# Li-Qingyun/RSCoTr

Measured on AMD Instinct MI355X. Metric: images/sec MTL train step (Swin-T 512^2, bs=2/GPU), higher is better.
Workload: dtype f32 (large products as three fp16 MFMAs on two-plane power-of-two-scaled splits of the fp32 operands, fp32 accumulate: fp32-FMA-class error; six bf16 MFMAs on three-plane splits where an operand has no range word)

## Files before the change

include/rscotr.h:

```cpp
#ifndef RSCOTR_H
#define RSCOTR_H
#include <stdint.h>
#ifdef __cplusplus
extern "C" {
#endif

#define RSCOTR_OK 0
#define RSCOTR_E_SHAPE (-1)
#define RSCOTR_E_ALIGN (-2)
#define RSCOTR_E_ARCH (-3)
#define RSCOTR_E_LAUNCH (-4)
#define RSCOTR_E_ARG (-5)

#define RSCOTR_ABI_VERSION 11
int rscotr_version(void);
const char* rscotr_last_error(void);
int rscotr_device_count(void);

int rscotr_prof_enable(int every_gemm, int every_msda_fwd, int every_msda_bwd, int max_records);
int rscotr_prof_pause(void);
int rscotr_prof_empty(int n, void* stream);
int rscotr_prof_get(int i, int* kind, double* work, float* ms, char* name, int name_len);
int rscotr_prof_disable(void);

int rscotr_msda_fwd(const float* value, const int64_t* spatial_shapes,
                    const int64_t* level_start_index, const float* loc, const float* attn,
                    float* out, int B, int Nk, int Nq, int H, int D, int L, int P, void* stream);
int rscotr_msda_bwd(const float* value, const int64_t* spatial_shapes,
                    const int64_t* level_start_index, const float* loc, const float* attn,
                    const float* grad_out, float* grad_value, float* grad_loc, float* grad_attn,
                    int B, int Nk, int Nq, int H, int D, int L, int P, const int64_t* shapes_host,
                    void* workspace, int64_t workspace_bytes, uint32_t* amax_grad_value,
                    void* stream);
int64_t rscotr_msda_bwd_workspace(int B, int Nk, int Nq, int H, int L, int P);
int64_t rscotr_msda_bwd_tiled_workspace(const int64_t* shapes_host, int B, int Nk, int Nq, int H, int D, int L, int P);
int rscotr_msda_prep_fwd(const float* off, const float* logit, const float* ref, const float* norm, float* loc,
                         float* attn, int B, int Nq, int H, int L, int P, int refdim, int ld_off, int ld_logit,
                         int ref_levels, void* stream);
int rscotr_msda_prep_bwd(const float* grad_loc, const float* grad_attn, const float* attn, const float* ref,
                         const float* norm, float* grad_off, float* grad_logit, int B, int Nq, int H, int L, int P,
                         int refdim, int ld_off, int ld_logit, int ref_levels, uint32_t* amax_out, void* stream);
int rscotr_msda_fused_ok(int Nk, int H, int D, int L, int P);
int rscotr_msda_fwd_prep(const float* value, const int64_t* spatial_shapes, const int64_t* level_start_index,
                         const float* off, const float* logit, int ld_off, int ld_logit, const float* ref,
                         const float* norm, int refdim, int ref_levels, float* loc, float* attn, float* out, int B,
                         int Nk, int Nq, int H, int D, int L, int P, void* stream);

int rscotr_gemm_split_weights(const int64_t* table, int n, int total_blocks, void* stream);
int64_t rscotr_gemm_f32_wplanes_workspace(int M, int N, int K);
int rscotr_gemm_f32_wplanes_ok(int M, int N, int K, int act_is_gelu);
int rscotr_gemm_f32_wplanes(const float* A, const void* planes, int npad, float* C, int M, int N, int K, int lda, int ldc,
                            const float* bias, int act, const float* aux, float* pre, const float* resid, int accumulate,
                            const float* rowscale, int rows_per_scale, float* out2, float* workspace,
                            int64_t workspace_bytes, void* stream);
int rscotr_gemm_set_precision(int prec);
int rscotr_gemm_get_precision(void);
int64_t rscotr_gemm_f32_workspace(int M, int N, int K);
int rscotr_gemm_f32(const float* A, const float* B, float* C, int M, int N, int K, int lda, int ldb,
                    int ldc, int a_kmajor, int b_kmajor, const float* bias, int act, const float* aux,
                    float* pre, const float* resid, int accumulate, float* rowsum, int rowsum_accumulate,
                    const float* rowscale, int rows_per_scale, const float* kscale, int krows_per_scale,
                    float* out2, float* workspace, int64_t workspace_bytes, void* stream);
#define RSCOTR_RANGE_EXP_LO 80
#define RSCOTR_RANGE_PLANES 32
#define RSCOTR_RANGE_STRIDE 16384
int rscotr_gemm_f32_r(const float* A, const float* B, float* C, int M, int N, int K, int lda, int ldb,
                      int ldc, int a_kmajor, int b_kmajor, const float* bias, int act, const float* aux,
                      float* pre, const float* resid, int accumulate, float* rowsum, int rowsum_accumulate,
                      const float* rowscale, int rows_per_scale, const float* kscale, int krows_per_scale,
                      float* out2, float* workspace, int64_t workspace_bytes, const uint32_t* amax_a,
                      const uint32_t* amax_b, uint32_t* amax_out, void* stream);
int rscotr_gemm_set_h3(int on);
int rscotr_gemm_relu_bits_ok(int M, int N, int K, int lda, int ldb, int a_kmajor, int b_kmajor);
int rscotr_gemm_split_weights_h3(const int64_t* table, int n, int total_blocks, void* stream);
int rscotr_gemm_f32_rb(const float* A, const float* B, float* C, int M, int N, int K, int lda, int ldb,
                       int ldc, int a_kmajor, int b_kmajor, const float* bias, int act, const float* aux,
                       float* pre, const float* resid, int accumulate, float* rowsum, int rowsum_accumulate,
                       const float* rowscale, int rows_per_scale, const float* kscale, int krows_per_scale,
                       float* out2, float* workspace, int64_t workspace_bytes, const uint32_t* amax_a,
                       const uint32_t* amax_b, uint32_t* amax_out, const void* b_planes, int b_rpad, void* stream);
int rscotr_ffn_h3_ok(int M, int C, int H);
int rscotr_ffn_h3_splits(int M, int C, int H);
int64_t rscotr_ffn_h3_bits_words(int M, int C, int H);
int rscotr_gemm_split_weights_frag(const int64_t* table, int n, int total_blocks, void* stream);
int rscotr_lin_h3_ok(int M, int N, int K);
int rscotr_lin_h3(const float* X, int M, int N, int K, const void* Wf, const float* bias, const float* resid, float* Y,
                  const float* xscale, const float* yscale, int rows_per, const uint32_t* amax_x, const uint32_t* amax_w,
                  uint32_t* amax_y, void* stream);
int rscotr_lin_h3_ln(const float* X, int M, int N, int K, const float* ln_weight, const float* ln_bias, float ln_eps, float* ln_out,
                     float* ln_mean, float* ln_rstd, const void* Wf, const float* bias, const float* resid, float* Y,
                     const float* yscale, int rows_per, const uint32_t* amax_ln_weight, const uint32_t* amax_ln_bias,
                     const uint32_t* amax_w, uint32_t* amax_ln_out, uint32_t* amax_y, void* stream);
int rscotr_ffn_h3_ln(const float* X, int M, int C, int H, const float* ln_weight, const float* ln_bias, float ln_eps, float* ln_out,
                     float* ln_mean, float* ln_rstd, const void* W1f, const float* b1, const void* W2f, const float* b2, float* Pre,
                     float* Hid, const float* resid, float* Y, const float* yscale, int rows_per, const uint32_t* amax_ln_weight,
                     const uint32_t* amax_ln_bias, const uint32_t* amax_w1, const uint32_t* amax_w2, const uint32_t* amax_b1,
                     uint32_t* amax_ln_out, uint32_t* amax_hid, uint32_t* amax_y, float* workspace, int64_t workspace_bytes,
                     void* stream);
int rscotr_ffn_h3(const float* X, int M, int C, int H, const void* W1f, const float* b1, const void* W2f, const float* b2,
                  int mode, void* bits, float* Pre, float* Hid, const float* resid, float* Y, const float* xscale,
                  const float* yscale, int rows_per, const uint32_t* amax_x, const uint32_t* amax_w1,
                  const uint32_t* amax_w2, const uint32_t* amax_b1, uint32_t* amax_hid, uint32_t* amax_y, float* workspace,
                  int64_t workspace_bytes, void* stream);
int rscotr_gemm_f32_split_route(int M, int N, int K, int lda, int ldb, int a_kmajor, int b_kmajor, int act, int has_pre,
                                int has_rowscale, int has_kscale, int64_t workspace_bytes);
int rscotr_amax_f32(const float* X, int64_t rows, int cols, int ld, uint32_t* slot, void* stream);
int rscotr_amax_group(const int64_t* table, int n, int total_blocks, void* stream);
int rscotr_gemm_f32_dw_slabs(const float* A, const float* B, float* C, int M, int N, int K, int lda, int ldb, int ldc,
                             float* rowsum, const float* kscale, int krows_per_scale, float* slab_region,
                             int64_t slab_bytes, int32_t* splits_out, void* stream);
int rscotr_gemm_f32_dw_slabs_r(const float* A, const float* B, float* C, int M, int N, int K, int lda, int ldb, int ldc,
                               float* rowsum, const float* kscale, int krows_per_scale, float* slab_region,
                               int64_t slab_bytes, int32_t* splits_out, const uint32_t* amax_a, const uint32_t* amax_b,
                               void* stream);
int rscotr_splitk_flush(const int64_t* table, const int32_t* wgmap, int nwg, double bytes, void* stream);
int rscotr_gemm_dw_group(const int64_t* table, int n, int total_wgs, int variant, double flops,
                         const uint32_t* amax_base, void* stream);

int rscotr_gemm_f32_batched(const float* A, const float* B, float* C, int M, int N, int K, int lda, int ldb,
                            int ldc, int a_kmajor, int b_kmajor, int nb0, int nb1, int64_t sA0, int64_t sA1,
                            int64_t sB0, int64_t sB1, int64_t sC0, int64_t sC1, int accumulate, int ksplits,
                            float* workspace, int64_t c_elems, void* stream);
int rscotr_softmax_mask_fwd(float* S, const unsigned char* mask, int mask_mode, int B, int heads, int Lq, int Lk,
                            float scale, void* stream);
int rscotr_softmax_bwd(const float* P, float* dP, int64_t rows, int Lk, float scale, void* stream);
int64_t rscotr_attn_core_workspace(int B, int heads, int Lq, int Lk);
int rscotr_attn_core_fwd(const float* q, const float* k, const float* v, const unsigned char* mask, int mask_mode, float* out,
                         float* lse, int B, int heads, int Lq, int Lk, int hd, int ldq, int ldk, int ldv, int ldo, float scale,
                         void* workspace, int64_t workspace_bytes, void* stream);
int rscotr_attn_core_bwd(const float* q, const float* k, const float* v, const unsigned char* mask, int mask_mode, const float* out,
                         const float* dout, const float* lse, float* dq, float* dk, float* dv, int B, int heads, int Lq, int Lk,
                         int hd, int ldq, int ldk, int ldv, int ldo, int lddq, int lddk, int lddv, float scale, void* workspace,
                         int64_t workspace_bytes, void* stream);
int64_t rscotr_colsum_f32_workspace(int M, int N);
int rscotr_colsum_f32(const float* X, float* out, int M, int N, int ld, int accumulate, float* workspace,
                      int64_t workspace_bytes, void* stream);

int rscotr_layernorm_fwd(const float* x, const float* weight, const float* bias, float* y, float* mean,
                         float* rstd, int M, int C, float eps, uint32_t* amax_out, void* stream);
int rscotr_det_proposals(const float* enc_cls, const float* enc_reg, const float* proposals, int proposals_batched,
                         int64_t* topk_idx, float* topk_score, float* topk_unact, float* topk_anchor, int32_t* inv, int B, int N,
                         int C, int K, void* stream);
int rscotr_det_proposals_bwd(const float* d_score, const float* d_anchor, const float* topk_anchor, const int32_t* inv,
                             float* d_cls, float* d_reg, int B, int N, int C, int K, void* stream);

int rscotr_det_targets(const int32_t* q_for_gt, const int64_t* gt_lab, const float* gt_boxn, int64_t* labels, float* bbox_targets,
                       float* bbox_weights, int S, int B, int Q, int G, int num_classes, void* stream);

int rscotr_layernorm_fwd_sum(const float* x, const float* weight, const float* bias, float* y, float* mean, float* rstd,
                             const float* add, int add_rows, float* y2, int M, int C, float eps, uint32_t* amax_out,
                             void* stream);
int64_t rscotr_layernorm_bwd_workspace(int M, int C);
int rscotr_layernorm_bwd(const float* dy, const float* x, const float* weight, const float* mean,
                         const float* rstd, float* dx, const float* dx_add, float* dweight, float* dbias, int M, int C,
                         float* workspace, int64_t workspace_bytes, uint32_t* amax_out, void* stream);

int rscotr_patch_merge_norm_fwd(const float* x, const float* weight, const float* bias, float* y, float* mean, float* rstd,
                                int B, int H, int W, int Cin, float eps, uint32_t* amax_out, void* stream);
int64_t rscotr_patch_merge_norm_bwd_workspace(int B, int H, int W, int Cin);
int rscotr_patch_merge_norm_bwd(const float* dy, const float* x, const float* weight, const float* mean, const float* rstd,
                                float* dx, float* dweight, float* dbias, int B, int H, int W, int Cin, float* workspace,
                                int64_t workspace_bytes, int fold, uint32_t* amax_out, void* stream);

int rscotr_layernorm_bwd_partials(const float* dy, const float* x, const float* weight, const float* mean,
                                  const float* rstd, float* dx, const float* dx_add, int M, int C, float* part, int64_t part_bytes,
                                  uint32_t* amax_out, void* stream);
int rscotr_layernorm_flush(const int64_t* table, const int32_t* wgmap, int nwg, void* stream);


int rscotr_swin_wattn_fwd(const float* qkv, const float* qkv_bias, const float* bias_table, float* out,
                          int B, int H, int W, int C, int heads, int ws, int shift, uint32_t* amax_out,
                         void* stream);
int64_t rscotr_swin_wattn_bwd_workspace(int B, int H, int W, int C, int heads);
int rscotr_swin_wattn_bwd(const float* qkv, const float* qkv_bias, const float* bias_table, const float* dout,
                          float* dqkv, float* dqkv_bias, float* dbias_table, int B, int H, int W, int C,
                          int heads, int ws, int shift, const float* out, float* workspace,
                          int64_t workspace_bytes, uint32_t* amax_out, void* stream);
int rscotr_swin_wattn_flush(const int64_t* table, int n, int total_heads, void* stream);

int64_t rscotr_groupnorm_tokens_workspace(int B, int L, int C, int G);
int rscotr_groupnorm_tokens_fwd(const float* x, const float* weight, const float* bias, float* y,
                                float* mean_rstd, int B, int L, int C, int G, float eps, float* workspace,
                                int64_t workspace_bytes, void* stream);
int rscotr_groupnorm_tokens_bwd(const float* dy, const float* x, const float* weight, const float* mean_rstd,
                                float* dx, float* dweight, float* dbias, float* proj_ws, int B, int L, int C,
                                int G, int64_t dy_batch_stride, float* workspace, int64_t workspace_bytes, void* stream);
int rscotr_im2col3x3s2_tokens(const float* x, float* col, int B, int H, int W, int C, void* stream);
int rscotr_col2im3x3s2_tokens(const float* dcol, float* dx, int B, int H, int W, int C, void* stream);

int64_t rscotr_upsample_ce_workspace(void);
int rscotr_upsample_ce_fwd(const float* logit, const int64_t* label, float* lse, float* sums, int B, int C,
                           int h, int w, int H, int W, int ignore_index, float* workspace, int64_t workspace_bytes,
                           void* stream);
int rscotr_upsample_ce_bwd(const float* logit, const int64_t* label, const float* lse, const float* grad_scale,
                           float* dlogit, int B, int C, int h, int w, int H, int W, int ignore_index, void* stream);
int64_t rscotr_upsample_ce_w_workspace(void);
int rscotr_upsample_ce_w_fwd(const float* logit, const int64_t* label, const float* class_weight, float* lse, float* nll,
                             float* pix_weight, float* sums, int B, int C, int h, int w, int H, int W, int ignore_index,
                             float* workspace, int64_t workspace_bytes, void* stream);
int rscotr_upsample_ce_ohem(const int64_t* label, const float* class_weight, const float* nll, float* pix_weight,
                            float* sum_out, int64_t npix, int C, int ignore_index, int64_t kept, float nll_thresh,
                            float* workspace, int64_t workspace_bytes, void* stream);
int rscotr_upsample_ce_w_bwd(const float* logit, const int64_t* label, const float* lse, const float* pix_weight,
                             const float* grad_scale, float* dlogit, int B, int C, int h, int w, int H, int W,
                             int ignore_index, void* stream);

int64_t rscotr_upsample_dice_workspace(int B, int C);
int rscotr_upsample_dice_fwd(const float* logit, const int64_t* label, const float* class_weight, float* lse, float* coef,
                             float* loss, int B, int C, int h, int w, int H, int W, int ignore_index, float smooth,
                             float loss_weight, float* workspace, int64_t workspace_bytes, void* stream);
int rscotr_upsample_dice_bwd(const float* logit, const int64_t* label, const float* lse, const float* coef,
                             const float* grad_scale, float* pix_s, float* dlogit, int B, int C, int h, int w, int H, int W,
                             int ignore_index, void* stream);

int64_t rscotr_upsample_tversky_workspace(int B, int C);
int rscotr_upsample_tversky_fwd(const float* logit, const int64_t* label, const float* class_weight, float* lse, float* coef,
                                float* loss, int B, int C, int h, int w, int H, int W, int ignore_index, float alpha, float beta,
                                float smooth, float loss_weight, float* workspace, int64_t workspace_bytes, void* stream);
int rscotr_upsample_tversky_bwd(const float* logit, const int64_t* label, const float* lse, const float* coef,
                                const float* grad_scale, float* pix_s, float* dlogit, int B, int C, int h, int w, int H, int W,
                                int ignore_index, void* stream);

int64_t rscotr_upsample_focal_workspace(void);
int rscotr_upsample_focal_fwd(const float* logit, const int64_t* label, const float* alpha_per_class, const float* class_weight,
                              float* loss, int B, int C, int h, int w, int H, int W, int ignore_index, float gamma, float alpha,
                              float loss_scale, float* workspace, int64_t workspace_bytes, void* stream);
int rscotr_upsample_focal_bwd(const float* logit, const int64_t* label, const float* alpha_per_class, const float* class_weight,
                              const float* grad_scale, float* dlogit, int B, int C, int h, int w, int H, int W, int ignore_index,
                              float gamma, float alpha, void* stream);

int64_t rscotr_upsample_lovasz_workspace(int B, int C, int nslots, int H, int W, int per_image);
int rscotr_upsample_lovasz_sort_tile(void);
int rscotr_upsample_lovasz_sort_workgroup(void);
int rscotr_upsample_lovasz_fwd(const float* logit, const int64_t* label, const int* slots, const float* class_weight, float* lse,
                               float* dplane, int* meta, float* loss, int B, int C, int nslots, int h, int w, int H, int W,
                               int ignore_index, int present, int per_image, int image_mean, float loss_weight, float* workspace,
                               int64_t workspace_bytes, void* stream);
int rscotr_upsample_lovasz_bwd(const float* logit, const int64_t* label, const int* slots, const float* lse, const float* dplane,
                               const int* meta, const float* grad_scale, float* pix_s, float* dlogit, int B, int C, int nslots,
                               int h, int w, int H, int W, int ignore_index, int per_image, void* stream);

int rscotr_sine_embed4(const float* pos, float* out, int64_t rows, void* stream);

int rscotr_level_embed_fwd(const float* x, int64_t x_bstride, const float* cst, int cst_batched, const float* w,
                           float* out, const int* sizes, int L, int B, int N, int C, void* stream);
int rscotr_cdn_queries(const int64_t* gt_lab, const float* gt_boxn, const int64_t* slot_src, const float* slot_valid,
                       const float* slot_neg, const float* u, int uniform, const float* embed, float label_thr,
                       float box_scale, int num_classes, int64_t* kl_out, float* q_label, float* q_bbox, int n_slots, int C,
                       void* stream);
int rscotr_cdn_embed_grad(const float* g, const int64_t* kl, const float* slot_valid, float* dw, int rows, int n_slots,
                          int C, int accumulate, void* stream);
int rscotr_gap_tokens_fwd(const float* x, float* out, int B, int T, int C, void* stream);
int rscotr_gap_tokens_bwd(const float* g, float* dx, int B, int T, int C, void* stream);
int rscotr_soft_ce(const float* score, const float* label, float* loss, float* dscore, int B, int C, float smooth,
                   float avg_factor, void* stream);
int rscotr_sum8(const float* p0, const float* p1, const float* p2, const float* p3, const float* p4, const float* p5,
                const float* p6, const float* p7, int n, float* out, int64_t count, void* stream);
int rscotr_pack4(const float* a, int64_t na, const float* b, int64_t nb, const float* c, int64_t nc, const float* d,
                 int64_t nd, float* out, uint32_t* amax_out, void* stream);
int64_t rscotr_level_embed_bwd_workspace(int L, int C);
int rscotr_level_embed_bwd(const float* g, float* dw, const int* sizes, int L, int B, int N, int C, int accumulate,
                           float* workspace, int* counters, void* stream);

int rscotr_seg_attn_mask(const float* mask_pred, unsigned char* out, int rows, int h, int w, int th, int tw,
                         void* stream);

int64_t rscotr_seg_mix_workspace(void);
int rscotr_seg_mix_fwd(const float* cls, const float* e, const float* mf, float* mix, float* seg, int B, int Q, int K, int D,
                       int P, void* stream);
int rscotr_seg_mix_bwd(const float* g, const float* cls, const float* e, const float* mf, const float* mix, float* dmf,
                       float* de, float* dcls, float* dmix, int B, int Q, int K, int D, int P, float* workspace,
                       int64_t workspace_bytes, void* stream);

int rscotr_refine_box_fwd(const float* delta, const float* ref, float* out, int64_t n, float eps, void* stream);
int rscotr_refine_box_bwd(const float* grad_out, const float* out, const float* ref, float* d_delta, float* d_ref,
                          int64_t n, float eps, void* stream);
int rscotr_match_cost(const float* cls, const float* box, const float* gt_box, const int64_t* gt_lab,
                      const float* factors, float* cost, int S, int B, int Q, int C, int G, float w_cls, float w_l1,
                      float w_iou, float alpha, float gamma, float eps, void* stream);
int rscotr_focal_sum(const float* pred, const int64_t* target, const float* weight, float* sums, float* dpred, int S,
                     int N, int C, float gamma, float alpha, void* stream);
int rscotr_box_loss(const float* pred, const float* target, const float* weight, const float* factors, float* sums,
                    float* d_l1, float* d_giou, int S, int B, int Q, float eps, void* stream);
int rscotr_match_cost_kind(const float* cls, const float* box, const float* gt_box, const int64_t* gt_lab,
                           const float* factors, float* cost, int S, int B, int Q, int C, int G, float w_cls, float w_l1,
                           float w_iou, float alpha, float gamma, float eps, int iou_mode, void* stream);
int rscotr_box_loss_kind(const float* pred, const float* target, const float* weight, const float* factors, float* sums,
                         float* d_l1, float* d_iou, int S, int B, int Q, float eps, int kind, int mode, void* stream);
int rscotr_qfl_sum(const float* pred, const int64_t* target, const float* weight, const float* box, const float* box_target,
                   float* sums, float* dpred, int S, int N, int C, float beta, void* stream);

int rscotr_lsap_f64(const double* cost, int nr, int nc, int64_t* row_ind, int64_t* col_ind);
int rscotr_lsap_dev_f32(const float* cost, const int32_t* gcount, int P, int Q, int ld, int32_t* q_for_gt,
                        void* stream);
int rscotr_lsap_batch_f32(const float* cost, const int64_t* offsets, const int* rows, const int* cols,
                          int n, const int64_t* out_offsets, int64_t* row_ind, int64_t* col_ind);

int rscotr_grad_sumsq(const float* grad, const int32_t* chunk_seg, const int64_t* chunk_off,
                      const int32_t* chunk_len, const float* seg_dyn, int nchunks, float* sumsq,
                      void* stream);
int rscotr_adamw_clip_step(float* param, const float* grad, float* exp_avg, float* exp_avg_sq,
                           const int32_t* chunk_seg, const int64_t* chunk_off, const int32_t* chunk_len,
                           const float* seg_dyn, int nchunks, const float* sumsq, float max_norm,
                           float beta1, float beta2, float eps, void* stream);
int rscotr_adamw_clip_step_r(float* param, const float* grad, float* exp_avg, float* exp_avg_sq,
                             const int32_t* chunk_seg, const int64_t* chunk_off, const int32_t* chunk_len,
                             const float* seg_dyn, int nchunks, const float* sumsq, float max_norm,
                             float beta1, float beta2, float eps, uint32_t* seg_amax, int nseg, uint32_t* chunk_amax,
                             void* stream);
int rscotr_param_amax(const float* param, const int32_t* chunk_seg, const int64_t* chunk_off,
                      const int32_t* chunk_len, int nchunks, uint32_t* seg_amax, int nseg, uint32_t* chunk_amax,
                      void* stream);

int rscotr_comm_available(void);
int rscotr_comm_unique_id(void* id128);
int rscotr_comm_init(const void* id128, int rank, int nranks, void** comm_out);
int rscotr_comm_allreduce_avg(void* comm, float* buf, int64_t count, void* stream);
int rscotr_comm_destroy(void* comm);

int rscotr_img_prep_u8(const uint8_t* src, const int64_t* meta, float* out, int B, int Hout, int Wout,
                       const float* mean3, const float* std3, int to_rgb, void* stream);
int rscotr_seg_label_prep_u8(const uint8_t* src, const int64_t* meta, int64_t* out, int B, int Hout, int Wout,
                             int reduce_zero_label, int pad_val, void* stream);

int rscotr_img_aug_u8(const uint8_t* src, const int64_t* meta, const int32_t* tables, const float* params, float* out,
                      int B, int Hout, int Wout, const float* mean3, const float* std3, int to_rgb, void* stream);
int rscotr_seg_label_aug_u8(const uint8_t* src, const int64_t* meta, const int32_t* tables, int64_t* out, int B, int Hout,
                            int Wout, int reduce_zero_label, int pad_val, void* stream);

int rscotr_img_aug_chain_u8(const uint8_t* src, const int64_t* meta, const int32_t* tables, float* out, int B, int Hout,
                            int Wout, const float* mean3, const float* std3, int to_rgb, void* stream);

int rscotr_img_aug_rot_u8(const uint8_t* src, const int64_t* meta, const int32_t* tables, const float* params,
                          const int32_t* rot, const int32_t* warp, float* out, int B, int Hout, int Wout, const float* mean3,
                          const float* std3, int to_rgb, void* stream);
int rscotr_seg_label_rot_u8(const uint8_t* src, const int64_t* meta, const int32_t* tables, const int32_t* rot,
                            const int32_t* warp, int64_t* out, int B, int Hout, int Wout, int reduce_zero_label, int pad_val,
                            void* stream);

int rscotr_img_frames_u8(const uint8_t* src, const int64_t* meta, const int32_t* tables, uint8_t* frames, int B, int H, int W,
                         void* stream);
int rscotr_randaug_u8(const uint8_t* in, uint8_t* out, const int32_t* meta, const int32_t* warp, const int16_t* wtab,
                      uint32_t* stats, int need_stats, int B, int H, int W, void* stream);

int rscotr_seg_predict_u8(const float* logit, uint8_t* out, int B, int C, int h, int w, int H, int W, int rescale, int hs,
                          int ws, int Ho, int Wo, int flip, void* stream);
int rscotr_seg_areas_u8(const uint8_t* pred, const uint8_t* gt, int64_t* out, int B, int Hp, int Wp, int C, int ignore_index,
                        int reduce_zero_label, void* stream);

int rscotr_seg_predict_tta_u8(const int64_t* views, uint8_t* out, int V, int B, int C, int Ho, int Wo, void* stream);

int rscotr_seg_predict_slide_u8(const float* logit, uint8_t* out, int B, int C, int h, int w, int H, int W, int ch, int cw, int sy,
                                int sx, int rescale, int hs, int ws, int Ho, int Wo, int flip, void* stream);

int rscotr_det_decode_f32(const float* cls, const float* box, const float* meta, float* dets, int64_t* labels, int B, int Q,
                          int C, int K, int rescale, void* stream);
int rscotr_det_match(const float* dets, const int64_t* labels, const int32_t* n_det, const float* gt_boxes,
                     const int64_t* gt_labels, const int64_t* gt_offsets, const double* area_ranges, const double* iou_thrs,
                     int32_t* flags, int32_t* npig, int B, int K, int64_t G, int C, int A, int T, int max_det, void* stream);

#ifdef __cplusplus
}
#endif
#endif
```

rscotr_amd/csrc/common.h:

```cpp
#pragma once
#include <hip/hip_runtime.h>
#include <stdint.h>
#include <stdio.h>
#include <stdarg.h>

#define RSCOTR_OK 0
#define RSCOTR_E_SHAPE (-1)
#define RSCOTR_E_ALIGN (-2)
#define RSCOTR_E_ARCH (-3)
#define RSCOTR_E_LAUNCH (-4)
#define RSCOTR_E_ARG (-5)

namespace rscotr {

char* err_buf();

inline int fail(int code, const char* fmt, ...) {
  va_list ap;
  va_start(ap, fmt);
  vsnprintf(err_buf(), 512, fmt, ap);
  va_end(ap);
  return code;
}

inline int check_launch(const char* what) {
  hipError_t e = hipGetLastError();
  if (e != hipSuccess) return fail(RSCOTR_E_LAUNCH, "%s: %s", what, hipGetErrorString(e));
  return RSCOTR_OK;
}

inline bool aligned16(const void* p) { return (reinterpret_cast<uintptr_t>(p) & 15u) == 0; }

constexpr int kWave = 64;

enum { PROF_GEMM = 0, PROF_MSDA_FWD = 1, PROF_MSDA_BWD = 2, PROF_HBM = 3, PROF_MFMA = 4, PROF_KINDS = 5 };
struct ProfScope {
  int slot;
  hipStream_t stream;
  ProfScope(int kind, double work, hipStream_t s, const char* fmt, ...);
  ~ProfScope();
};

template <int G>
__device__ __forceinline__ float group_sum(float v) {
#pragma unroll
  for (int o = G / 2; o > 0; o >>= 1) v += __shfl_xor(v, o, 64);
  return v;
}

template <int G>
__device__ __forceinline__ float group_max(float v) {
#pragma unroll
  for (int o = G / 2; o > 0; o >>= 1) v = fmaxf(v, __shfl_xor(v, o, 64));
  return v;
}

__device__ __forceinline__ float wave_sum(float v) { return group_sum<64>(v); }
__device__ __forceinline__ float wave_max(float v) { return group_max<64>(v); }

constexpr int kAmaxPlanes = 32;
constexpr int kAmaxStride = 16384;
constexpr int kRangeExpLo = 80;

__device__ __forceinline__ int range_byte(unsigned bits) {
  return min(max((int)((bits >> 23) & 0xffu), kRangeExpLo), kRangeExpLo + 4 * kAmaxPlanes - 1) - kRangeExpLo;
}
__device__ __forceinline__ void range_mark(unsigned* slot, int i) {
  reinterpret_cast<unsigned char*>(slot + (long)(i >> 2) * kAmaxStride)[i & 3] = 1;
}

__device__ __forceinline__ int amax_fold_code(unsigned v, int sub) { return v ? 4 * sub + ((31 - __clz((int)v)) >> 3) + 1 : 0; }
__device__ __forceinline__ unsigned amax_fold_bits(int c) { return c ? (unsigned)(kRangeExpLo + c - 1) << 23 : 0u; }
__device__ __forceinline__ unsigned amax_fold(unsigned v) {
  int c = amax_fold_code(v, (int)(threadIdx.x & (kAmaxPlanes - 1)));
#pragma unroll
  for (int o = kAmaxPlanes / 2; o > 0; o >>= 1) c = max(c, __shfl_xor(c, o, 64));
  return amax_fold_bits(__builtin_amdgcn_readfirstlane(c));
}
__device__ __forceinline__ unsigned amax_fold_lane(unsigned v, int lane) {
  int c = amax_fold_code(v, lane & (kAmaxPlanes - 1));
#pragma unroll
  for (int o = kAmaxPlanes / 2; o > 0; o >>= 1) c = max(c, __builtin_amdgcn_ds_bpermute((lane ^ o) << 2, c));
  return amax_fold_bits(__builtin_amdgcn_readfirstlane(c));
}
__device__ __forceinline__ unsigned amax_read(const unsigned* word) {
  return amax_fold(word[(long)(threadIdx.x & (kAmaxPlanes - 1)) * kAmaxStride]);
}
__device__ __forceinline__ float amax_hi(unsigned folded) { return folded ? __uint_as_float(folded + (1u << 23)) : 0.f; }

__device__ __forceinline__ void amax_commit(unsigned* slot, float amx) {
  if (!slot) return;
#pragma unroll
  for (int o = 32; o > 0; o >>= 1) amx = fmaxf(amx, __shfl_xor(amx, o, 64));
  if ((threadIdx.x & 63) == 0) {
    const unsigned b = __float_as_uint(amx) & 0x7fffffffu;
    if (b) range_mark(slot, range_byte(b));
  }
}

__device__ __forceinline__ float2 msda_location(const float* __restrict__ r, float2 o, const float* __restrict__ norm, int l, int P,
                                                int refdim) {
  float2 out;
  if (refdim == 2) {
    out.x = r[0] + o.x / norm[2 * l];
    out.y = r[1] + o.y / norm[2 * l + 1];
  } else {
    out.x = r[0] + o.x / (float)P * r[2] * 0.5f;
    out.y = r[1] + o.y / (float)P * r[3] * 0.5f;
  }
  return out;
}

__device__ __forceinline__ float amax4(float a, const float4& v) {
  return fmaxf(fmaxf(a, fmaxf(fabsf(v.x), fabsf(v.y))), fmaxf(fabsf(v.z), fabsf(v.w)));
}

}
```

rscotr_amd/csrc/ffn.hip:

```cpp
#include "gemm_common.h"
#include "rscotr.h"
#include <type_traits>

namespace rscotr {

typedef float f32x4_t __attribute__((ext_vector_type(4)));

constexpr int FFN_HC = 128;
constexpr int FFN_LDRB = 160;
constexpr int FFN_DB = 1;

enum { FFN_RELU = 0,
       FFN_RELU_GATE = 1,
       FFN_GELU = 2,
       FFN_GELU_GRAD = 3 };

struct FfnParams {
  const float* X;
  int M, H;
  const uint4* W1f;
  const float* b1;
  const uint4* W2f;
  const float* b2;
  unsigned* bits;
  float* Pre;
  float* Hid;
  const float* resid;
  float* Y;
  const float* xscale;
  const float* yscale;
  int rows_per;
  const unsigned *amax_x, *amax_w1, *amax_w2, *amax_b1;
  unsigned *amax_hid, *amax_y;
  int splits;
  float* slabs;
  const float *ln_g, *ln_b;
  float ln_eps;
  float *ln_out, *ln_mean, *ln_rstd;
  const unsigned *amax_g, *amax_bt;
  unsigned* amax_ln;
  int by_xcd;
  int tpx;
};

template <int C, int NT>
constexpr size_t ffn_lds_bytes() { return (size_t)(C / 32 + 2 * (FFN_HC / 32)) * (16 * NT) * FFN_LDRB; }

__device__ __forceinline__ void store_b128(float4 v, __amdgpu_buffer_rsrc_t r, int voff, int soff) {
  __builtin_amdgcn_raw_buffer_store_b128(__builtin_bit_cast(__attribute__((__vector_size__(4 * sizeof(unsigned)))) unsigned, v), r, voff, soff, 0);
  __builtin_amdgcn_sched_barrier(0);
  asm volatile("s_nop 1");
  __builtin_amdgcn_sched_barrier(0);
}

constexpr int FFN_STAG_MINC = 192;
constexpr int FFN_PHASES = 4;
__device__ __forceinline__ int ffn_phase(int j, int n) {
  const int ph = n < FFN_PHASES ? n : FFN_PHASES;
  return (int)((unsigned)j % (unsigned)ph) * n / ph;
}

__device__ __forceinline__ f32x4_t mfma16(uint4 a, uint4 b, f32x4_t c) {
  return __builtin_amdgcn_mfma_f32_16x16x32_f16(__builtin_bit_cast(f16x8, a), __builtin_bit_cast(f16x8, b), c, 0, 0, 0);
}

constexpr int FFN_SWIN_WAVES = 4;
template <int C, int NT, int MODE, bool LN = false>
__global__ __launch_bounds__(512) __attribute__((amdgpu_waves_per_eu(C == 96 ? FFN_SWIN_WAVES : 2, C == 96 ? FFN_SWIN_WAVES : 2))) void ffn_h3_kernel(FfnParams p) {
  extern __shared__ __attribute__((aligned(16))) unsigned char ffn_lds[];
  constexpr bool GATE = MODE == FFN_RELU_GATE, GELU = MODE == FFN_GELU, GGRAD = MODE == FFN_GELU_GRAD;
  constexpr bool FWD = MODE == FFN_RELU || MODE == FFN_GELU;
  constexpr int BM = 16 * NT, STG = BM * FFN_LDRB;
  constexpr int KS1 = C / 32, HST = FFN_HC / 32;
  constexpr int DA = KS1 % 2 == 0 ? 2 : 1;
  constexpr int TPB = C == 96 ? 2 : C / 64;
  constexpr int NB = C / 16 / TPB;
  constexpr int RING = 4 * DA > 2 * TPB * FFN_DB ? 4 * DA : 2 * TPB * FFN_DB;
  constexpr int SPK = (2 * NT + KS1 - 1) / KS1;
  static_assert(C % 32 == 0 && (C / 16) % TPB == 0 && NB <= 4, "column tiles split evenly over the B wavefronts");
  unsigned char* xs = ffn_lds;
  unsigned char* hs = ffn_lds + KS1 * STG;
  const int tid = threadIdx.x, lane = tid & 63, li = lane & 15, kg = lane >> 4;
  const int wv = __builtin_amdgcn_readfirstlane(tid >> 6);
  const bool role_a = wv < 4;
  const int wr = wv & 3;
  int bx = blockIdx.x, by = blockIdx.y, jx = blockIdx.x >> 3;
  if (p.by_xcd) {
    const int xcd = (int)(blockIdx.x & 7);
    jx = (int)(blockIdx.x >> 3);
    by = xcd % p.splits;
    bx = xcd / p.splits + (8 / p.splits) * jx;
    if (bx * BM >= p.M) return;
  }
  const int m0 = bx * BM;
  const int nch = p.H / FFN_HC;
  const int nloc = nch / p.splits;
  const int cbase = by * nloc;

  const long sub = (long)(lane & (kAmaxPlanes - 1)) * kAmaxStride;
  const unsigned rx = LN ? 0u : p.amax_x[sub], r1 = p.amax_w1[sub], r2 = p.amax_w2[sub], rb = p.amax_b1 ? p.amax_b1[sub] : 0u;
  const unsigned rg = LN ? p.amax_g[sub] : 0u, rbt = (LN && p.amax_bt) ? p.amax_bt[sub] : 0u;

  const int wbytes = p.H * C * 4;
  const __amdgpu_buffer_rsrc_t rW = __builtin_amdgcn_make_buffer_rsrc(const_cast<uint4*>(role_a ? p.W1f : p.W2f), 0, wbytes, 0x00020000);
  const int nks2 = p.H / 32;
  const int vW = lane * 16 + (role_a ? wr * 2 * KS1 * 2048 : wr * TPB * nks2 * 2048);
  auto ld_a = [&](int c, int ks, int it, int pl) {
    return __builtin_bit_cast(uint4, __builtin_amdgcn_raw_buffer_load_b128(rW, vW, c * (8 * KS1 * 2048) + it * (KS1 * 2048) + ks * 2048 + pl * 1024, 0));
  };
  auto ld_b = [&](int t, int it, int pl) {
    return __builtin_bit_cast(uint4, __builtin_amdgcn_raw_buffer_load_b128(rW, vW, it * nks2 * 2048 + t * 2048 + pl * 1024, 0));
  };
  const int c0r = cbase + (C >= FFN_STAG_MINC ? ffn_phase(jx, nloc) : 0);
  uint4 ring[RING];
  if (role_a) {
#pragma unroll
    for (int q = 0; q < 4 * DA; ++q) ring[q] = ld_a(c0r, q >> 2, (q >> 1) & 1, q & 1);
  } else if (wr < NB) {
#pragma unroll
    for (int q = 0; q < 2 * TPB * FFN_DB; ++q) ring[q] = ld_b(c0r * HST + min(q / (2 * TPB), HST - 1), (q >> 1) % TPB, q & 1);
  }

  const int rows_ok = min(BM, p.M - m0);
  const __amdgpu_buffer_rsrc_t rX = __builtin_amdgcn_make_buffer_rsrc(const_cast<float*>(p.X + (long)m0 * C), 0, rows_ok * C * 4, 0x00020000);
  const __amdgpu_buffer_rsrc_t rH = __builtin_amdgcn_make_buffer_rsrc(p.Hid + (long)m0 * p.H, 0, rows_ok * p.H * 4, 0x00020000);
  const __amdgpu_buffer_rsrc_t rP = __builtin_amdgcn_make_buffer_rsrc((GELU || GGRAD) ? p.Pre + (long)m0 * p.H : p.Hid, 0, rows_ok * p.H * 4, 0x00020000);
  float* const ybase = p.splits > 1 ? p.slabs + (long)by * p.M * C : p.Y;
  const __amdgpu_buffer_rsrc_t rY = __builtin_amdgcn_make_buffer_rsrc(ybase + (long)m0 * C, 0, rows_ok * C * 4, 0x00020000);
  const __amdgpu_buffer_rsrc_t rR = __builtin_amdgcn_make_buffer_rsrc(const_cast<float*>(p.resid ? p.resid + (long)m0 * C : p.X), 0, rows_ok * C * 4, 0x00020000);

  const unsigned fx = LN ? 0u : amax_fold(rx);
  const float xbound = LN ? sqrtf((float)C) * amax_hi(amax_fold(rg)) + amax_hi(amax_fold(rbt)) : amax_hi(fx);
  const unsigned ux = LN ? __float_as_uint(xbound) : fx;
  if constexpr (!LN) {
    constexpr int TOT = BM * (C / 4), NV = (TOT + 511) / 512;
    float4 v[NV];
#pragma unroll
    for (int i = 0; i < NV; ++i) v[i] = __builtin_bit_cast(float4, __builtin_amdgcn_raw_buffer_load_b128(rX, (tid + i * 512) * 16, 0, 0));
    const int ex0 = h3_scale_exp(ux);
    const H3Scale hx{__uint_as_float((unsigned)ex0 << 23), __uint_as_float((unsigned)(ex0 + 11) << 23)};
#pragma unroll
    for (int i = 0; i < NV; ++i) {
      const int idx = tid + i * 512;
      if (TOT % 512 == 0 || idx < TOT) {
        const int row = idx / (C / 4), kq = (idx % (C / 4)) * 4;
        if (p.xscale) {
          const float f = p.xscale[min(m0 + row, p.M - 1) / p.rows_per];
          v[i].x *= f; v[i].y *= f; v[i].z *= f; v[i].w *= f;
        }
        unsigned ab[3], cd[3];
        split_pair_h(v[i].x, v[i].y, hx, ab);
        split_pair_h(v[i].z, v[i].w, hx, cd);
        unsigned char* dst = xs + (kq / 32) * STG + row * FFN_LDRB + (kq % 32) * 2;
        *reinterpret_cast<uint2*>(dst) = make_uint2(ab[0], cd[0]);
        *reinterpret_cast<uint2*>(dst + 64) = make_uint2(ab[1], cd[1]);
      }
    }
  } else {
    static_assert(C % 48 == 0 && (C / 12 == 8 || C / 12 == 16 || C / 12 == 32), "LN rows: 8 / 16 / 32 lanes x 3 float4");
    constexpr int G = C / 12, RPP = 512 / G, NP = (BM + RPP - 1) / RPP;
    const int sub = tid % G, rr = tid / G;
    const __amdgpu_buffer_rsrc_t rL = __builtin_amdgcn_make_buffer_rsrc(p.ln_out + (long)m0 * C, 0, (by == 0 ? rows_ok : 0) * C * 4, 0x00020000);
    const int ex0 = h3_scale_exp(ux);
    const H3Scale hx{__uint_as_float((unsigned)ex0 << 23), __uint_as_float((unsigned)(ex0 + 11) << 23)};
    float amx = 0.f;
    if (RPP <= BM || wv < 8 * BM / RPP) {
      float4 gw[3], gb[3];
#pragma unroll
      for (int j = 0; j < 3; ++j) {
        gw[j] = reinterpret_cast<const float4*>(p.ln_g)[sub + j * G];
        gb[j] = p.ln_b ? reinterpret_cast<const float4*>(p.ln_b)[sub + j * G] : make_float4(0.f, 0.f, 0.f, 0.f);
      }
#pragma unroll
      for (int ps = 0; ps < NP; ++ps) {
        const int row = ps * RPP + rr;
        float4 v[3];
        float sm = 0.f;
#pragma unroll
        for (int j = 0; j < 3; ++j) {
          v[j] = __builtin_bit_cast(float4, __builtin_amdgcn_raw_buffer_load_b128(rX, (row * C + 4 * (sub + j * G)) * 4, 0, 0));
          sm += v[j].x + v[j].y + v[j].z + v[j].w;
        }
#pragma unroll
        for (int o = G / 2; o > 0; o >>= 1) sm += __shfl_xor(sm, o, 64);
        const float mu = sm * (1.f / (float)C);
        float q = 0.f;
#pragma unroll
        for (int j = 0; j < 3; ++j) {
          v[j].x -= mu; v[j].y -= mu; v[j].z -= mu; v[j].w -= mu;
          q += v[j].x * v[j].x + v[j].y * v[j].y + v[j].z * v[j].z + v[j].w * v[j].w;
        }
#pragma unroll
        for (int o = G / 2; o > 0; o >>= 1) q += __shfl_xor(q, o, 64);
        const float rs = rsqrtf(q * (1.f / (float)C) + p.ln_eps);
        if (sub == 0 && by == 0 && row < rows_ok) { p.ln_mean[m0 + row] = mu; p.ln_rstd[m0 + row] = rs; }
#pragma unroll
        for (int j = 0; j < 3; ++j) {
          float4 o;
          o.x = v[j].x * rs * gw[j].x + gb[j].x; o.y = v[j].y * rs * gw[j].y + gb[j].y;
          o.z = v[j].z * rs * gw[j].z + gb[j].z; o.w = v[j].w * rs * gw[j].w + gb[j].w;
          if (row >= rows_ok) o = make_float4(0.f, 0.f, 0.f, 0.f);
          const int kq = 4 * (sub + j * G);
          store_b128(o, rL, (row * C + kq) * 4, 0);
          amx = amax4(amx, o);
          unsigned ab[3], cd[3];
          split_pair_h(o.x, o.y, hx, ab);
          split_pair_h(o.z, o.w, hx, cd);
          unsigned char* dst = xs + (kq / 32) * STG + row * FFN_LDRB + (kq % 32) * 2;
          *reinterpret_cast<uint2*>(dst) = make_uint2(ab[0], cd[0]);
          *reinterpret_cast<uint2*>(dst + 64) = make_uint2(ab[1], cd[1]);
        }
      }
    }
    if (by == 0) amax_commit(p.amax_ln, amx);
  }
  const unsigned u1 = amax_fold(r1), u2 = amax_fold(r2), ub = amax_fold(rb);
  const int ex = h3_scale_exp(ux), e1 = h3_scale_exp(u1), e2 = h3_scale_exp(u2);
  const float bound = ((float)C * xbound * amax_hi(u1) + amax_hi(ub)) * (GGRAD ? 1.25f : 1.f);
  const int eh = h3_scale_exp(__float_as_uint(bound));
  const H3Scale hh{__uint_as_float((unsigned)eh << 23), __uint_as_float((unsigned)(eh + 11) << 23)};
  const float invx = __uint_as_float((unsigned)(254 - ex) << 23), inv1 = __uint_as_float((unsigned)(254 - e1) << 23);
  const float invh = __uint_as_float((unsigned)(254 - eh) << 23), inv2 = __uint_as_float((unsigned)(254 - e2) << 23);

  const int fo = li * FFN_LDRB + kg * 16;
  const int c0 = C >= FFN_STAG_MINC ? ffn_phase(jx, nloc) : 0;
  auto chunk_of = [&](int c) {
    if constexpr (C < FFN_STAG_MINC) return cbase + c;
    const int v = c + c0;
    return cbase + (v >= nloc ? v - nloc : v);
  };
  __syncthreads();

  if (role_a) {
    unsigned amxu = 0u;
    const int vH = (li * p.H + wr * 32 + 4 * kg) * 4;
    float4 pv[2][NT];
    float4 bvs[2];
    float4 pres[GGRAD ? 2 : 1][GGRAD ? NT : 1];
    unsigned bits = 0u;
    auto slice = [&](int cl, int it, int n) {
      const int cp = chunk_of(cl);
      float v[4] = {pv[it][n].x, pv[it][n].y, pv[it][n].z, pv[it][n].w};
      const int soff = (n * 16 * p.H + cp * FFN_HC + it * 16) * 4;
      if constexpr (MODE == FFN_RELU) {
        const float t[4] = {v[0] + bvs[it].x, v[1] + bvs[it].y, v[2] + bvs[it].z, v[3] + bvs[it].w};
#pragma unroll
        for (int r = 0; r < 4; ++r) {
          const bool pos = t[r] > 0.f;
          v[r] = pos ? t[r] : 0.f;
          bits |= (unsigned)pos << ((it * NT + n) * 4 + r);
        }
      } else if constexpr (GATE) {
#pragma unroll
        for (int r = 0; r < 4; ++r)
          v[r] = __uint_as_float(__float_as_uint(v[r]) & (unsigned)__builtin_amdgcn_sbfe((int)bits, (it * NT + n) * 4 + r, 1));
      } else if constexpr (GELU) {
        const float4 t = make_float4(v[0] + bvs[it].x, v[1] + bvs[it].y, v[2] + bvs[it].z, v[3] + bvs[it].w);
        store_b128(t, rP, vH, soff);
        v[0] = gelu_f(t.x); v[1] = gelu_f(t.y); v[2] = gelu_f(t.z); v[3] = gelu_f(t.w);
      } else {
        const float4 t = pres[GGRAD ? it : 0][GGRAD ? n : 0];
        v[0] *= gelu_grad_f(t.x); v[1] *= gelu_grad_f(t.y); v[2] *= gelu_grad_f(t.z); v[3] *= gelu_grad_f(t.w);
      }
#pragma unroll
      for (int r = 0; r < 4; ++r) amxu = max(amxu, __float_as_uint(v[r]) & 0x7fffffffu);
      unsigned ab[3], cd[3];
      split_pair_h(v[0], v[1], hh, ab);
      split_pair_h(v[2], v[3], hh, cd);
      unsigned char* dst = hs + (cl & 1) * (HST * STG) + wr * STG + li * FFN_LDRB + kg * 8 + n * 16 * FFN_LDRB + it * 32;
      *reinterpret_cast<uint2*>(dst) = make_uint2(ab[0], cd[0]);
      *reinterpret_cast<uint2*>(dst + 64) = make_uint2(ab[1], cd[1]);
      store_b128(make_float4(v[0], v[1], v[2], v[3]), rH, vH, soff);
    };
    auto pre_epi = [&](int cl) {
      const int cp = chunk_of(cl);
#pragma unroll
      for (int it = 0; it < 2; ++it)
        bvs[it] = (FWD && p.b1) ? *reinterpret_cast<const float4*>(p.b1 + cp * FFN_HC + wr * 32 + it * 16 + 4 * kg) : make_float4(0.f, 0.f, 0.f, 0.f);
      if constexpr (GATE) bits = p.bits[(((long)bx * nch + cp) * 4 + wr) * 64 + lane];
      else bits = 0u;
      if constexpr (GGRAD) {
#pragma unroll
        for (int it = 0; it < 2; ++it)
#pragma unroll
          for (int n = 0; n < NT; ++n)
            pres[it][n] = __builtin_bit_cast(float4, __builtin_amdgcn_raw_buffer_load_b128(rP, vH, (n * 16 * p.H + cp * FFN_HC + it * 16) * 4, 0));
      }
    };
    auto kloop = [&](int c, auto with_epi) {
      constexpr bool EPI = decltype(with_epi)::value;
      f32x4_t ha[2][NT], hb[2][NT];
#pragma unroll
      for (int it = 0; it < 2; ++it)
#pragma unroll
        for (int n = 0; n < NT; ++n) { ha[it][n] = f32x4_t{0.f, 0.f, 0.f, 0.f}; hb[it][n] = f32x4_t{0.f, 0.f, 0.f, 0.f}; }
      const int cw = chunk_of(c), cn = chunk_of(min(c + 1, nloc - 1));
#pragma unroll
      for (int ks = 0; ks < KS1; ++ks) {
        uint4 xh[NT], xl[NT];
#pragma unroll
        for (int n = 0; n < NT; ++n) {
          const unsigned char* q = xs + ks * STG + n * 16 * FFN_LDRB + fo;
          xh[n] = *reinterpret_cast<const uint4*>(q);
          xl[n] = *reinterpret_cast<const uint4*>(q + 64);
        }
#pragma unroll
        for (int it = 0; it < 2; ++it) {
          const int slot = (ks % DA) * 4 + it * 2;
          const uint4 wh = ring[slot], wl = ring[slot + 1];
#pragma unroll
          for (int n = 0; n < NT; ++n) hb[it][n] = mfma16(wh, xl[n], hb[it][n]);
#pragma unroll
          for (int n = 0; n < NT; ++n) hb[it][n] = mfma16(wl, xh[n], hb[it][n]);
#pragma unroll
          for (int n = 0; n < NT; ++n) ha[it][n] = mfma16(wh, xh[n], ha[it][n]);
          if (ks + DA < KS1) { ring[slot] = ld_a(cw, ks + DA, it, 0); ring[slot + 1] = ld_a(cw, ks + DA, it, 1); }
          else { ring[slot] = ld_a(cn, ks + DA - KS1, it, 0); ring[slot + 1] = ld_a(cn, ks + DA - KS1, it, 1); }
        }
        if constexpr (EPI) {
#pragma unroll
          for (int t = ks * SPK; t < (ks + 1) * SPK; ++t)
            if (t < 2 * NT) slice(c - 1, t / NT, t % NT);
        }
        __builtin_amdgcn_sched_barrier(0);
      }
      if constexpr (EPI && MODE == FFN_RELU) p.bits[(((long)bx * nch + chunk_of(c - 1)) * 4 + wr) * 64 + lane] = bits;
      pre_epi(c);
#pragma unroll
      for (int it = 0; it < 2; ++it)
#pragma unroll
        for (int n = 0; n < NT; ++n) {
          pv[it][n].x = fmaf(hb[it][n][0], 0x1p-11f, ha[it][n][0]) * invx * inv1;
          pv[it][n].y = fmaf(hb[it][n][1], 0x1p-11f, ha[it][n][1]) * invx * inv1;
          pv[it][n].z = fmaf(hb[it][n][2], 0x1p-11f, ha[it][n][2]) * invx * inv1;
          pv[it][n].w = fmaf(hb[it][n][3], 0x1p-11f, ha[it][n][3]) * invx * inv1;
        }
    };
    kloop(0, std::false_type{});
    __syncthreads();
#pragma unroll 1
    for (int c = 1; c < nloc; ++c) {
      kloop(c, std::true_type{});
      __syncthreads();
    }
#pragma unroll
    for (int t = 0; t < 2 * NT; ++t) slice(nloc - 1, t / NT, t % NT);
    if constexpr (MODE == FFN_RELU) p.bits[(((long)bx * nch + chunk_of(nloc - 1)) * 4 + wr) * 64 + lane] = bits;
    __syncthreads();
    __syncthreads();
    amax_commit(p.amax_hid, __uint_as_float(amxu));
  } else {
    f32x4_t ya[TPB][NT], yb[TPB][NT];
#pragma unroll
    for (int it = 0; it < TPB; ++it)
#pragma unroll
      for (int n = 0; n < NT; ++n) { ya[it][n] = f32x4_t{0.f, 0.f, 0.f, 0.f}; yb[it][n] = f32x4_t{0.f, 0.f, 0.f, 0.f}; }
    const bool active = wr < NB;
    __syncthreads();
    __syncthreads();
#pragma unroll 1
    for (int c = 0; c < nloc; ++c) {
      const unsigned char* img = hs + (c & 1) * (HST * STG) + fo;
      const int cb = chunk_of(c);
      if (active) {
#pragma unroll 1
        for (int kq = 0; kq < HST / FFN_DB; ++kq)
#pragma unroll
          for (int u = 0; u < FFN_DB; ++u) {
            const int ks = kq * FFN_DB + u;
            uint4 gh[NT], gl[NT];
#pragma unroll
            for (int n = 0; n < NT; ++n) {
              const unsigned char* q = img + ks * STG + n * 16 * FFN_LDRB;
              gh[n] = *reinterpret_cast<const uint4*>(q);
              gl[n] = *reinterpret_cast<const uint4*>(q + 64);
            }
            int tn;
            if constexpr (C < FFN_STAG_MINC) tn = cbase * HST + min(c * HST + ks + FFN_DB, nloc * HST - 1);
            else tn = ks + FFN_DB < HST ? cb * HST + ks + FFN_DB : chunk_of(min(c + 1, nloc - 1)) * HST + (ks + FFN_DB - HST);
#pragma unroll
            for (int it = 0; it < TPB; ++it) {
              const int slot = u * 2 * TPB + it * 2;
              const uint4 wh = ring[slot], wl = ring[slot + 1];
#pragma unroll
              for (int n = 0; n < NT; ++n) yb[it][n] = mfma16(wh, gl[n], yb[it][n]);
#pragma unroll
              for (int n = 0; n < NT; ++n) yb[it][n] = mfma16(wl, gh[n], yb[it][n]);
#pragma unroll
              for (int n = 0; n < NT; ++n) ya[it][n] = mfma16(wh, gh[n], ya[it][n]);
              ring[slot] = ld_b(tn, it, 0);
              ring[slot + 1] = ld_b(tn, it, 1);
            }
          }
      }
      __syncthreads();
    }
    if (active) {
      const int vY = (li * C + wr * TPB * 16 + 4 * kg) * 4;
      float amy = 0.f;
#pragma unroll
      for (int it = 0; it < TPB; ++it) {
        float4 bv = make_float4(0.f, 0.f, 0.f, 0.f);
        if (p.b2) bv = *reinterpret_cast<const float4*>(p.b2 + wr * TPB * 16 + it * 16 + 4 * kg);
        float4 e[NT];
        float ysc[NT];
#pragma unroll
        for (int n = 0; n < NT; ++n) {
          e[n] = p.resid ? __builtin_bit_cast(float4, __builtin_amdgcn_raw_buffer_load_b128(rR, vY, (n * 16 * C + it * 16) * 4, 0)) : make_float4(0.f, 0.f, 0.f, 0.f);
          ysc[n] = p.yscale ? p.yscale[min(m0 + n * 16 + li, p.M - 1) / p.rows_per] : 1.f;
        }
#pragma unroll
        for (int n = 0; n < NT; ++n) {
          float4 v;
          v.x = fmaf(fmaf(yb[it][n][0], 0x1p-11f, ya[it][n][0]) * invh * inv2 + bv.x, ysc[n], e[n].x);
          v.y = fmaf(fmaf(yb[it][n][1], 0x1p-11f, ya[it][n][1]) * invh * inv2 + bv.y, ysc[n], e[n].y);
          v.z = fmaf(fmaf(yb[it][n][2], 0x1p-11f, ya[it][n][2]) * invh * inv2 + bv.z, ysc[n], e[n].z);
          v.w = fmaf(fmaf(yb[it][n][3], 0x1p-11f, ya[it][n][3]) * invh * inv2 + bv.w, ysc[n], e[n].w);
          store_b128(v, rY, vY, (n * 16 * C + it * 16) * 4);
          amy = amax4(amy, v);
        }
      }
      amax_commit(p.amax_y, amy);
    }
  }
}

struct LinParams {
  const float* X;
  int M, N;
  const uint4* Wf;
  const float* bias;
  const float* resid;
  float* Y;
  const float* xscale;
  const float* yscale;
  int rows_per;
  const unsigned *amax_x, *amax_w;
  unsigned* amax_y;
  int col_groups;
  const float *ln_g, *ln_b;
  float ln_eps;
  float *ln_out, *ln_mean, *ln_rstd;
  const unsigned *amax_g, *amax_bt;
  unsigned* amax_ln;
};

template <int C, bool LN, int NT = 2>
__global__ __launch_bounds__(512) void lin_h3_kernel(LinParams p) {
  extern __shared__ __attribute__((aligned(16))) unsigned char ffn_lds[];
  constexpr int BM = 16 * NT, STG = BM * FFN_LDRB, KS1 = C / 32;
  constexpr int DA = KS1 % 2 == 0 ? 2 : KS1 % 3 == 0 ? 3 : 1;
  static_assert(C % 32 == 0 && KS1 % DA == 0, "reduction in whole 32-k steps");
  unsigned char* xs = ffn_lds;
  const int tid = threadIdx.x, lane = tid & 63, li = lane & 15, kg = lane >> 4;
  const int wv = __builtin_amdgcn_readfirstlane(tid >> 6);
  const int m0 = blockIdx.x * BM;
  const long sub = (long)(lane & (kAmaxPlanes - 1)) * kAmaxStride;
  const unsigned rx = LN ? 0u : p.amax_x[sub], rw = p.amax_w[sub];
  const unsigned rg = LN ? p.amax_g[sub] : 0u, rbt = (LN && p.amax_bt) ? p.amax_bt[sub] : 0u;
  const __amdgpu_buffer_rsrc_t rW = __builtin_amdgcn_make_buffer_rsrc(const_cast<uint4*>(p.Wf), 0, p.N * C * 4, 0x00020000);
  auto ld_w = [&](int col0, int ks, int it, int pl) {
    return __builtin_bit_cast(uint4, __builtin_amdgcn_raw_buffer_load_b128(rW, lane * 16, ((col0 >> 4) + it) * (KS1 * 2048) + ks * 2048 + pl * 1024, 0));
  };
  const int c_first = (int)blockIdx.y * 256 + wv * 32;
  const int c_step = 256 * (int)gridDim.y;
  uint4 ring[4 * DA];
  if (c_first < p.N) {
#pragma unroll
    for (int q = 0; q < 4 * DA; ++q) ring[q] = ld_w(c_first, q >> 2, (q >> 1) & 1, q & 1);
  }
  const int rows_ok = min(BM, p.M - m0);
  const __amdgpu_buffer_rsrc_t rX = __builtin_amdgcn_make_buffer_rsrc(const_cast<float*>(p.X + (long)m0 * C), 0, rows_ok * C * 4, 0x00020000);
  const __amdgpu_buffer_rsrc_t rY = __builtin_amdgcn_make_buffer_rsrc(p.Y + (long)m0 * p.N, 0, rows_ok * p.N * 4, 0x00020000);
  const __amdgpu_buffer_rsrc_t rR = __builtin_amdgcn_make_buffer_rsrc(const_cast<float*>(p.resid ? p.resid + (long)m0 * p.N : p.X), 0, rows_ok * p.N * 4, 0x00020000);
  const unsigned fx = LN ? 0u : amax_fold(rx);
  const float xbound = LN ? sqrtf((float)C) * amax_hi(amax_fold(rg)) + amax_hi(amax_fold(rbt)) : amax_hi(fx);
  const unsigned ux = LN ? __float_as_uint(xbound) : fx;
  const int ex = h3_scale_exp(ux);
  const H3Scale hx{__uint_as_float((unsigned)ex << 23), __uint_as_float((unsigned)(ex + 11) << 23)};
  if constexpr (!LN) {
    constexpr int TOT = BM * (C / 4), NV = (TOT + 511) / 512;
    float4 v[NV];
#pragma unroll
    for (int i = 0; i < NV; ++i) v[i] = __builtin_bit_cast(float4, __builtin_amdgcn_raw_buffer_load_b128(rX, (tid + i * 512) * 16, 0, 0));
#pragma unroll
    for (int i = 0; i < NV; ++i) {
      const int idx = tid + i * 512;
      if (TOT % 512 == 0 || idx < TOT) {
        const int row = idx / (C / 4), kq = (idx % (C / 4)) * 4;
        if (p.xscale) {
          const float f = p.xscale[min(m0 + row, p.M - 1) / p.rows_per];
          v[i].x *= f; v[i].y *= f; v[i].z *= f; v[i].w *= f;
        }
        unsigned ab[3], cd[3];
        split_pair_h(v[i].x, v[i].y, hx, ab);
        split_pair_h(v[i].z, v[i].w, hx, cd);
        unsigned char* dst = xs + (kq / 32) * STG + row * FFN_LDRB + (kq % 32) * 2;
        *reinterpret_cast<uint2*>(dst) = make_uint2(ab[0], cd[0]);
        *reinterpret_cast<uint2*>(dst + 64) = make_uint2(ab[1], cd[1]);
      }
    }
  } else {
    static_assert(!LN || (C % 48 == 0 && (C / 12 == 8 || C / 12 == 16 || C / 12 == 32)), "LN rows: 8 / 16 / 32 lanes x 3 float4");
    constexpr int G = C / 12, RPP = 512 / G, NP = (BM + RPP - 1) / RPP;
    const int sb = tid % G, rr = tid / G;
    const bool own = blockIdx.y == 0;
    const __amdgpu_buffer_rsrc_t rL = __builtin_amdgcn_make_buffer_rsrc(p.ln_out + (long)m0 * C, 0, (own ? rows_ok : 0) * C * 4, 0x00020000);
    float amx = 0.f;
    if (RPP <= BM || wv < 8 * BM / RPP) {
      float4 gw[3], gb[3];
#pragma unroll
      for (int j = 0; j < 3; ++j) {
        gw[j] = reinterpret_cast<const float4*>(p.ln_g)[sb + j * G];
        gb[j] = p.ln_b ? reinterpret_cast<const float4*>(p.ln_b)[sb + j * G] : make_float4(0.f, 0.f, 0.f, 0.f);
      }
#pragma unroll
      for (int ps = 0; ps < NP; ++ps) {
        const int row = ps * RPP + rr;
        float4 v[3];
        float sm = 0.f;
#pragma unroll
        for (int j = 0; j < 3; ++j) {
          v[j] = __builtin_bit_cast(float4, __builtin_amdgcn_raw_buffer_load_b128(rX, (row * C + 4 * (sb + j * G)) * 4, 0, 0));
          sm += v[j].x + v[j].y + v[j].z + v[j].w;
        }
#pragma unroll
        for (int o = G / 2; o > 0; o >>= 1) sm += __shfl_xor(sm, o, 64);
        const float mu = sm * (1.f / (float)C);
        float q = 0.f;
#pragma unroll
        for (int j = 0; j < 3; ++j) {
          v[j].x -= mu; v[j].y -= mu; v[j].z -= mu; v[j].w -= mu;
          q += v[j].x * v[j].x + v[j].y * v[j].y + v[j].z * v[j].z + v[j].w * v[j].w;
        }
#pragma unroll
        for (int o = G / 2; o > 0; o >>= 1) q += __shfl_xor(q, o, 64);
        const float rs = rsqrtf(q * (1.f / (float)C) + p.ln_eps);
        if (sb == 0 && own && row < rows_ok) { p.ln_mean[m0 + row] = mu; p.ln_rstd[m0 + row] = rs; }
#pragma unroll
        for (int j = 0; j < 3; ++j) {
          float4 o;
          o.x = v[j].x * rs * gw[j].x + gb[j].x; o.y = v[j].y * rs * gw[j].y + gb[j].y;
          o.z = v[j].z * rs * gw[j].z + gb[j].z; o.w = v[j].w * rs * gw[j].w + gb[j].w;
          if (row >= rows_ok) o = make_float4(0.f, 0.f, 0.f, 0.f);
          const int kq = 4 * (sb + j * G);
          store_b128(o, rL, (row * C + kq) * 4, 0);
          amx = amax4(amx, o);
          unsigned ab[3], cd[3];
          split_pair_h(o.x, o.y, hx, ab);
          split_pair_h(o.z, o.w, hx, cd);
          unsigned char* dst = xs + (kq / 32) * STG + row * FFN_LDRB + (kq % 32) * 2;
          *reinterpret_cast<uint2*>(dst) = make_uint2(ab[0], cd[0]);
          *reinterpret_cast<uint2*>(dst + 64) = make_uint2(ab[1], cd[1]);
        }
      }
    }
    if (own) amax_commit(p.amax_ln, amx);
  }
  const int ew = h3_scale_exp(amax_fold(rw));
  const float inv = __uint_as_float((unsigned)(254 - ex) << 23) * __uint_as_float((unsigned)(254 - ew) << 23);
  const int fo = li * FFN_LDRB + kg * 16;
  __syncthreads();

  float amy = 0.f;
#pragma unroll 1
  for (int col0 = c_first; col0 < p.N; col0 += c_step) {
    f32x4_t ha[2][NT], hb[2][NT];
#pragma unroll
    for (int it = 0; it < 2; ++it)
#pragma unroll
      for (int n = 0; n < NT; ++n) { ha[it][n] = f32x4_t{0.f, 0.f, 0.f, 0.f}; hb[it][n] = f32x4_t{0.f, 0.f, 0.f, 0.f}; }
    const int cnext = col0 + c_step < p.N ? col0 + c_step : col0;
#pragma unroll
    for (int ks = 0; ks < KS1; ++ks) {
      uint4 xh[NT], xl[NT];
#pragma unroll
      for (int n = 0; n < NT; ++n) {
        const unsigned char* q = xs + ks * STG + n * 16 * FFN_LDRB + fo;
        xh[n] = *reinterpret_cast<const uint4*>(q);
        xl[n] = *reinterpret_cast<const uint4*>(q + 64);
      }
#pragma unroll
      for (int it = 0; it < 2; ++it) {
        const int slot = (ks % DA) * 4 + it * 2;
        const uint4 wh = ring[slot], wl = ring[slot + 1];
#pragma unroll
        for (int n = 0; n < NT; ++n) hb[it][n] = mfma16(wh, xl[n], hb[it][n]);
#pragma unroll
        for (int n = 0; n < NT; ++n) hb[it][n] = mfma16(wl, xh[n], hb[it][n]);
#pragma unroll
        for (int n = 0; n < NT; ++n) ha[it][n] = mfma16(wh, xh[n], ha[it][n]);
        if (ks + DA < KS1) { ring[slot] = ld_w(col0, ks + DA, it, 0); ring[slot + 1] = ld_w(col0, ks + DA, it, 1); }
        else { ring[slot] = ld_w(cnext, ks + DA - KS1, it, 0); ring[slot + 1] = ld_w(cnext, ks + DA - KS1, it, 1); }
      }
      __builtin_amdgcn_sched_barrier(0);
    }
    const int vY = (li * p.N + col0 + 4 * kg) * 4;
#pragma unroll
    for (int it = 0; it < 2; ++it) {
      float4 bv = make_float4(0.f, 0.f, 0.f, 0.f);
      if (p.bias) bv = *reinterpret_cast<const float4*>(p.bias + col0 + it * 16 + 4 * kg);
      float4 e[NT];
      float ysc[NT];
#pragma unroll
      for (int n = 0; n < NT; ++n) {
        e[n] = p.resid ? __builtin_bit_cast(float4, __builtin_amdgcn_raw_buffer_load_b128(rR, vY, (n * 16 * p.N + it * 16) * 4, 0)) : make_float4(0.f, 0.f, 0.f, 0.f);
        ysc[n] = p.yscale ? p.yscale[min(m0 + n * 16 + li, p.M - 1) / p.rows_per] : 1.f;
      }
#pragma unroll
      for (int n = 0; n < NT; ++n) {
        float4 v;
        v.x = fmaf(fmaf(hb[it][n][0], 0x1p-11f, ha[it][n][0]) * inv + bv.x, ysc[n], e[n].x);
        v.y = fmaf(fmaf(hb[it][n][1], 0x1p-11f, ha[it][n][1]) * inv + bv.y, ysc[n], e[n].y);
        v.z = fmaf(fmaf(hb[it][n][2], 0x1p-11f, ha[it][n][2]) * inv + bv.z, ysc[n], e[n].z);
        v.w = fmaf(fmaf(hb[it][n][3], 0x1p-11f, ha[it][n][3]) * inv + bv.w, ysc[n], e[n].w);
        store_b128(v, rY, vY, (n * 16 * p.N + it * 16) * 4);
        amy = amax4(amy, v);
      }
    }
  }
  amax_commit(p.amax_y, amy);
}



__global__ __launch_bounds__(256) void split_weights_frag_kernel(const int64_t* __restrict__ table, int n_entries) {
  int e = 0;
  while (e + 1 < n_entries && (long)table[(long)(e + 1) * 9 + 6] <= (long)blockIdx.x) ++e;
  const int64_t* t = table + (long)e * 9;
  const float* W = reinterpret_cast<const float*>(t[0]);
  uint4* planes = reinterpret_cast<uint4*>(t[1]);
  const int wrows = (int)t[2], wcols = (int)t[3], ldw = (int)t[4], tr = (int)t[7];
  const int rows = tr ? wcols : wrows, red = tr ? wrows : wcols;
  const int se = h3_scale_exp(amax_read(reinterpret_cast<const unsigned*>(t[8])));
  const H3Scale hs{__uint_as_float((unsigned)se << 23), __uint_as_float((unsigned)(se + 11) << 23)};
  const long idx = ((long)blockIdx.x - t[6]) * 256 + threadIdx.x;
  const int nks = red / 32;
  const int lane = (int)(idx & 63);
  const long rest = idx >> 6;
  const int ks = (int)(rest % nks), nt = (int)(rest / nks);
  if (nt >= rows / 16) return;
  const int n = nt * 16 + (lane & 15), k0 = ks * 32 + 8 * (lane >> 4);
  float v[8];
  if (!tr) {
    const float4* src = reinterpret_cast<const float4*>(W + (long)n * ldw + k0);
    const float4 a = src[0], b = src[1];
    v[0] = a.x; v[1] = a.y; v[2] = a.z; v[3] = a.w; v[4] = b.x; v[5] = b.y; v[6] = b.z; v[7] = b.w;
  } else {
#pragma unroll
    for (int j = 0; j < 8; ++j) v[j] = W[(long)(k0 + j) * ldw + n];
  }
  unsigned h[4], l[4];
#pragma unroll
  for (int q = 0; q < 4; ++q) {
    unsigned o[3];
    split_pair_h(v[2 * q], v[2 * q + 1], hs, o);
    h[q] = o[0]; l[q] = o[1];
  }
  uint4* dst = planes + ((long)nt * nks + ks) * 128 + lane;
  dst[0] = make_uint4(h[0], h[1], h[2], h[3]);
  dst[64] = make_uint4(l[0], l[1], l[2], l[3]);
}

}

using namespace rscotr;

extern "C" int rscotr_gemm_split_weights_frag(const int64_t* table, int n, int total_blocks, void* stream) {
  if (!table || n <= 0 || total_blocks <= 0) return fail(RSCOTR_E_ARG, "split_weights_frag: empty table");
  hipLaunchKernelGGL(split_weights_frag_kernel, dim3((unsigned)total_blocks), dim3(256), 0, static_cast<hipStream_t>(stream), table, n);
  return check_launch("split_weights_frag");
}

static int ffn_rows(int M, int C) {
  if (C != 256) return 32;
  const long c48 = ((long)((M + 47) / 48) + 255) / 256 * 48, c32 = ((long)((M + 31) / 32) + 255) / 256 * 32;
  return c32 < c48 ? 32 : 48;
}

extern "C" int rscotr_ffn_h3_splits(int M, int C, int H) {
  if (H < FFN_HC || H % FFN_HC) return 1;
  const int bm = ffn_rows(M, C), tiles = (M + bm - 1) / bm, nch = H / FFN_HC;
  if (tiles >= 200) return 1;
  for (int d = 2; d <= nch / 2; ++d)
    if (nch % d == 0 && tiles * d >= 200) return d;
  return 1;
}

extern "C" int rscotr_ffn_h3_ok(int M, int C, int H) {
  return ((C == 384 || C == 256 || C == 192 || C == 128 || C == 96) && H >= FFN_HC && H % FFN_HC == 0 && M >= 1) ? 1 : 0;
}

extern "C" int64_t rscotr_ffn_h3_bits_words(int M, int C, int H) {
  const int bm = ffn_rows(M, C);
  return (int64_t)((M + bm - 1) / bm) * (H / FFN_HC) * 256;
}

template <int C, int NT, int MODE, bool LN = false>
static void ffn_launch1(const FfnParams& p, hipStream_t s) {
  constexpr size_t lds = ffn_lds_bytes<C, NT>();
  static bool attr_set = [] {
    (void)hipFuncSetAttribute(reinterpret_cast<const void*>(ffn_h3_kernel<C, NT, MODE, LN>), hipFuncAttributeMaxDynamicSharedMemorySize, (int)lds);
    return true;
  }();
  (void)attr_set;
  const unsigned tiles = (unsigned)((p.M + 16 * NT - 1) / (16 * NT));
  const dim3 grid = p.by_xcd ? dim3(8u * (unsigned)p.tpx) : dim3(tiles, (unsigned)p.splits);
  hipLaunchKernelGGL((ffn_h3_kernel<C, NT, MODE, LN>), grid, dim3(512), lds, s, p);
}

template <int C, int NT>
static void ffn_launch(const FfnParams& p, int mode, hipStream_t s) {
  switch (mode) {
    case FFN_RELU: ffn_launch1<C, NT, FFN_RELU>(p, s); break;
    case FFN_RELU_GATE: ffn_launch1<C, NT, FFN_RELU_GATE>(p, s); break;
    case FFN_GELU: ffn_launch1<C, NT, FFN_GELU>(p, s); break;
    default: ffn_launch1<C, NT, FFN_GELU_GRAD>(p, s); break;
  }
}

struct FfnNorm {
  const float *g, *b;
  float eps;
  float *out, *mean, *rstd;
  const uint32_t *amax_g, *amax_b;
  uint32_t* amax_out;
};

static int ffn_h3_run(const float* X, int M, int C, int H, const void* W1f, const float* b1, const void* W2f, const float* b2,
                      int mode, void* bits, float* Pre, float* Hid, const float* resid, float* Y, const float* xscale,
                      const float* yscale, int rows_per, const uint32_t* amax_x, const uint32_t* amax_w1,
                      const uint32_t* amax_w2, const uint32_t* amax_b1, uint32_t* amax_hid, uint32_t* amax_y, float* workspace,
                      int64_t workspace_bytes, const FfnNorm& ln, void* stream) {
  if (!rscotr_ffn_h3_ok(M, C, H)) return fail(RSCOTR_E_SHAPE, "ffn_h3: M=%d C=%d H=%d (C in {96, 128, 192, 256, 384}, H %% 128 == 0)", M, C, H);
  const int splits = rscotr_ffn_h3_splits(M, C, H);
  if (splits > 1 && (!workspace || workspace_bytes < (int64_t)splits * M * C * 4 || ((uintptr_t)workspace & 15)))
    return fail(RSCOTR_E_ARG, "ffn_h3: M=%d C=%d H=%d runs as %d partial sums: workspace of %lld bytes (16-byte aligned), got %lld", M, C, H,
                splits, (long long)splits * M * C * 4, (long long)workspace_bytes);
  if (mode < 0 || mode > 3) return fail(RSCOTR_E_ARG, "ffn_h3: mode %d", mode);
  if (!X || !W1f || !W2f || !Hid || !Y || (!amax_x && !ln.g) || !amax_w1 || !amax_w2) return fail(RSCOTR_E_ARG, "ffn_h3: null argument");
  if (ln.g) {
    if (mode != FFN_GELU || !(C == 96 || C == 192 || C == 384))
      return fail(RSCOTR_E_SHAPE, "ffn_h3_ln: the norm prologue exists for mode 2 (GELU forward) at C in {96, 192, 384} (mode %d, C=%d)", mode, C);
    if (!ln.out || !ln.mean || !ln.rstd || !ln.amax_g || xscale) return fail(RSCOTR_E_ARG, "ffn_h3_ln: null argument (or a row scale on X)");
    if (((uintptr_t)ln.g | (uintptr_t)ln.b | (uintptr_t)ln.out) & 15) return fail(RSCOTR_E_ALIGN, "ffn_h3_ln: operands must be 16-byte aligned");
  }
  if (mode <= FFN_RELU_GATE ? !bits : !Pre) return fail(RSCOTR_E_ARG, "ffn_h3: mode %d needs %s", mode, mode <= FFN_RELU_GATE ? "bits" : "Pre");
  if ((xscale || yscale) && rows_per <= 0) return fail(RSCOTR_E_ARG, "ffn_h3: rows_per with a row scale");
  if (((uintptr_t)X | (uintptr_t)W1f | (uintptr_t)W2f | (uintptr_t)Hid | (uintptr_t)Y | (uintptr_t)resid | (uintptr_t)b1 | (uintptr_t)b2 |
       (uintptr_t)Pre) & 15)
    return fail(RSCOTR_E_ALIGN, "ffn_h3: operands must be 16-byte aligned");
  if ((long)M * H * 4 >= (1l << 32)) return fail(RSCOTR_E_SHAPE, "ffn_h3: M * H too large for 32-bit buffer offsets");
  const bool fwd = mode == FFN_RELU || mode == FFN_GELU;
  FfnParams p{};
  p.X = X; p.M = M; p.H = H;
  p.W1f = static_cast<const uint4*>(W1f); p.b1 = fwd ? b1 : nullptr;
  p.W2f = static_cast<const uint4*>(W2f); p.b2 = b2;
  p.bits = static_cast<unsigned*>(bits); p.Pre = Pre; p.Hid = Hid; p.resid = resid; p.Y = Y;
  p.xscale = xscale; p.yscale = yscale; p.rows_per = rows_per > 0 ? rows_per : 1;
  p.amax_x = amax_x; p.amax_w1 = amax_w1; p.amax_w2 = amax_w2; p.amax_b1 = fwd ? amax_b1 : nullptr;
  p.amax_hid = amax_hid; p.amax_y = amax_y;
  p.splits = splits; p.slabs = workspace;
  p.ln_g = ln.g; p.ln_b = ln.b; p.ln_eps = ln.eps; p.ln_out = ln.out; p.ln_mean = ln.mean; p.ln_rstd = ln.rstd;
  p.amax_g = ln.amax_g; p.amax_bt = ln.amax_b; p.amax_ln = ln.amax_out;
  if (splits > 1 && 8 % splits == 0) {
    const int bm0 = ffn_rows(M, C), tiles = (M + bm0 - 1) / bm0, per = 8 / splits;
    p.by_xcd = 1; p.tpx = (tiles + per - 1) / per;
  }
  if (splits > 1) { p.b2 = nullptr; p.resid = nullptr; p.yscale = nullptr; p.amax_y = nullptr; }
  hipStream_t s = static_cast<hipStream_t>(stream);
  const int bm = ffn_rows(M, C);
  {
    ProfScope prof(PROF_GEMM, 4.0 * M * (double)C * H, s, "rscotr::ffn_h3_kernel<%d, %d, %d>", C, bm / 16, mode);
    if (ln.g) {
      if (C == 384) ffn_launch1<384, 2, FFN_GELU, true>(p, s);
      else if (C == 192) ffn_launch1<192, 2, FFN_GELU, true>(p, s);
      else ffn_launch1<96, 2, FFN_GELU, true>(p, s);
    } else if (C == 384) ffn_launch<384, 2>(p, mode, s);
    else if (C == 256) { if (bm == 32) ffn_launch<256, 2>(p, mode, s); else ffn_launch<256, 3>(p, mode, s); }
    else if (C == 192) ffn_launch<192, 2>(p, mode, s);
    else if (C == 128) ffn_launch<128, 2>(p, mode, s);
    else ffn_launch<96, 2>(p, mode, s);
  }
  if (int rc = check_launch("ffn_h3")) return rc;
  if (splits > 1) {
    GemmParams q{};
    q.C = Y; q.M = M; q.N = C; q.ldc = C; q.vecC = 1;
    q.bias = b2; q.resid = resid; q.rowscale = yscale; q.rows_per = p.rows_per;
    q.slabs = workspace; q.splits = splits; q.amax_out = amax_y;
    splitk_reduce_launch(q, workspace, s);
    return check_launch("ffn_h3 combine");
  }
  return 0;
}


extern "C" int rscotr_ffn_h3(const float* X, int M, int C, int H, const void* W1f, const float* b1, const void* W2f, const float* b2,
                             int mode, void* bits, float* Pre, float* Hid, const float* resid, float* Y, const float* xscale,
                             const float* yscale, int rows_per, const uint32_t* amax_x, const uint32_t* amax_w1,
                             const uint32_t* amax_w2, const uint32_t* amax_b1, uint32_t* amax_hid, uint32_t* amax_y, float* workspace,
                             int64_t workspace_bytes, void* stream) {
  return ffn_h3_run(X, M, C, H, W1f, b1, W2f, b2, mode, bits, Pre, Hid, resid, Y, xscale, yscale, rows_per, amax_x, amax_w1, amax_w2, amax_b1,
                    amax_hid, amax_y, workspace, workspace_bytes, FfnNorm{}, stream);
}

extern "C" int rscotr_ffn_h3_ln(const float* X, int M, int C, int H, const float* ln_weight, const float* ln_bias, float ln_eps,
                                float* ln_out, float* ln_mean, float* ln_rstd, const void* W1f, const float* b1, const void* W2f,
                                const float* b2, float* Pre, float* Hid, const float* resid, float* Y, const float* yscale, int rows_per,
                                const uint32_t* amax_ln_weight, const uint32_t* amax_ln_bias, const uint32_t* amax_w1,
                                const uint32_t* amax_w2, const uint32_t* amax_b1, uint32_t* amax_ln_out, uint32_t* amax_hid,
                                uint32_t* amax_y, float* workspace, int64_t workspace_bytes, void* stream) {
  if (!ln_weight) return fail(RSCOTR_E_ARG, "ffn_h3_ln: null LayerNorm weight");
  const FfnNorm ln{ln_weight, ln_bias, ln_eps, ln_out, ln_mean, ln_rstd, amax_ln_weight, amax_ln_bias, amax_ln_out};
  return ffn_h3_run(X, M, C, H, W1f, b1, W2f, b2, FFN_GELU, nullptr, Pre, Hid, resid, Y, nullptr, yscale, rows_per, nullptr, amax_w1, amax_w2,
                    amax_b1, amax_hid, amax_y, workspace, workspace_bytes, ln, stream);
}

template <int C, bool LN, int NT = 2>
static void lin_launch(const LinParams& p, hipStream_t s) {
  constexpr size_t lds = (size_t)(C / 32) * (16 * NT) * FFN_LDRB;
  static bool attr_set = [] {
    (void)hipFuncSetAttribute(reinterpret_cast<const void*>(lin_h3_kernel<C, LN, NT>), hipFuncAttributeMaxDynamicSharedMemorySize, (int)lds);
    return true;
  }();
  (void)attr_set;
  hipLaunchKernelGGL((lin_h3_kernel<C, LN, NT>), dim3((unsigned)((p.M + 16 * NT - 1) / (16 * NT)), (unsigned)p.col_groups), dim3(512), lds, s, p);
}

extern "C" int rscotr_lin_h3_ok(int M, int N, int K) {
  const bool k_ok = K == 96 || K == 128 || K == 192 || K == 256 || K == 288 || K == 384 || K == 576 || K == 768 || K == 1152;
  return (k_ok && N >= 32 && N % 32 == 0 && M >= 1 && (long)M * N * 4 < (1l << 32) && (long)M * K * 4 < (1l << 32)) ? 1 : 0;
}

static int lin_h3_run(const float* X, int M, int N, int K, const void* Wf, const float* bias, const float* resid, float* Y,
                      const float* xscale, const float* yscale, int rows_per, const uint32_t* amax_x, const uint32_t* amax_w,
                      uint32_t* amax_y, const FfnNorm& ln, void* stream) {
  if (!rscotr_lin_h3_ok(M, N, K)) return fail(RSCOTR_E_SHAPE, "lin_h3: M=%d N=%d K=%d (K in {96, 128, 192, 256, 288, 384, 576, 768, 1152}, N %% 32 == 0)", M, N, K);
  if (!X || !Wf || !Y || (!amax_x && !ln.g) || !amax_w) return fail(RSCOTR_E_ARG, "lin_h3: null argument");
  if ((xscale || yscale) && rows_per <= 0) return fail(RSCOTR_E_ARG, "lin_h3: rows_per with a row scale");
  if (((uintptr_t)X | (uintptr_t)Wf | (uintptr_t)Y | (uintptr_t)resid | (uintptr_t)bias) & 15)
    return fail(RSCOTR_E_ALIGN, "lin_h3: operands must be 16-byte aligned");
  if (ln.g) {
    if (!(K == 96 || K == 192 || K == 384)) return fail(RSCOTR_E_SHAPE, "lin_h3_ln: the norm prologue exists at K in {96, 192, 384} (K=%d)", K);
    if (!ln.out || !ln.mean || !ln.rstd || !ln.amax_g || xscale) return fail(RSCOTR_E_ARG, "lin_h3_ln: null argument (or a row scale on X)");
    if (((uintptr_t)ln.g | (uintptr_t)ln.b | (uintptr_t)ln.out) & 15) return fail(RSCOTR_E_ALIGN, "lin_h3_ln: operands must be 16-byte aligned");
  }
  LinParams p{};
  p.X = X; p.M = M; p.N = N; p.Wf = static_cast<const uint4*>(Wf); p.bias = bias; p.resid = resid; p.Y = Y;
  p.xscale = xscale; p.yscale = yscale; p.rows_per = rows_per > 0 ? rows_per : 1;
  p.amax_x = amax_x; p.amax_w = amax_w; p.amax_y = amax_y;
  p.ln_g = ln.g; p.ln_b = ln.b; p.ln_eps = ln.eps; p.ln_out = ln.out; p.ln_mean = ln.mean; p.ln_rstd = ln.rstd;
  p.amax_g = ln.amax_g; p.amax_bt = ln.amax_b; p.amax_ln = ln.amax_out;
  p.col_groups = (M + 31) / 32 >= 200 ? 1 : (N + 255) / 256;
  if (K == 1152 && M >= 8192) return fail(RSCOTR_E_SHAPE, "lin_h3: K = 1152 is a few-row width (M=%d)", M);
  hipStream_t s = static_cast<hipStream_t>(stream);
  ProfScope prof(PROF_GEMM, 2.0 * M * (double)N * K, s, "rscotr::lin_h3_kernel<%d, %s>", K, ln.g ? "true" : "false");
  if (ln.g) {
    if (K == 96) lin_launch<96, true>(p, s);
    else if (K == 192) lin_launch<192, true>(p, s);
    else lin_launch<384, true>(p, s);
  } else switch (K) {
    case 96: lin_launch<96, false>(p, s); break;
    case 128: lin_launch<128, false>(p, s); break;
    case 192: lin_launch<192, false>(p, s); break;
    case 256: lin_launch<256, false>(p, s); break;
    case 288: lin_launch<288, false>(p, s); break;
    case 384: lin_launch<384, false>(p, s); break;
    case 576: lin_launch<576, false>(p, s); break;
    case 768: lin_launch<768, false>(p, s); break;
    default: lin_launch<1152, false, 1>(p, s); break;
  }
  return check_launch("lin_h3");
}

extern "C" int rscotr_lin_h3(const float* X, int M, int N, int K, const void* Wf, const float* bias, const float* resid, float* Y,
                             const float* xscale, const float* yscale, int rows_per, const uint32_t* amax_x, const uint32_t* amax_w,
                             uint32_t* amax_y, void* stream) {
  return lin_h3_run(X, M, N, K, Wf, bias, resid, Y, xscale, yscale, rows_per, amax_x, amax_w, amax_y, FfnNorm{}, stream);
}

extern "C" int rscotr_lin_h3_ln(const float* X, int M, int N, int K, const float* ln_weight, const float* ln_bias, float ln_eps,
                                float* ln_out, float* ln_mean, float* ln_rstd, const void* Wf, const float* bias, const float* resid,
                                float* Y, const float* yscale, int rows_per, const uint32_t* amax_ln_weight, const uint32_t* amax_ln_bias,
                                const uint32_t* amax_w, uint32_t* amax_ln_out, uint32_t* amax_y, void* stream) {
  if (!ln_weight) return fail(RSCOTR_E_ARG, "lin_h3_ln: null LayerNorm weight");
  const FfnNorm ln{ln_weight, ln_bias, ln_eps, ln_out, ln_mean, ln_rstd, amax_ln_weight, amax_ln_bias, amax_ln_out};
  return lin_h3_run(X, M, N, K, Wf, bias, resid, Y, nullptr, yscale, rows_per, nullptr, amax_w, amax_y, ln, stream);
}
```

rscotr_amd/csrc/gemm_planes.hip:

```cpp
#include "gemm_plan.h"

namespace rscotr {
constexpr int WPL_LDR = 56;

struct WplRegs {
  float4 a;
  uint4 b[3];
  __device__ __forceinline__ void load(const float* a_src, const unsigned short* b_src, long a_off, long b_off, bool b_active) {
    a = *reinterpret_cast<const float4*>(a_src + a_off);
    if (b_active) {
      const uint4* s = reinterpret_cast<const uint4*>(b_src + b_off);
      b[0] = s[0]; b[1] = s[1]; b[2] = s[2];
    }
  }
  __device__ __forceinline__ void store(unsigned* a_s, unsigned* b_s, int tid, bool b_active) const {
    __bf16 x[3], y[3], z[3], w[3];
    split_planes<3>(a.x, x); split_planes<3>(a.y, y); split_planes<3>(a.z, z); split_planes<3>(a.w, w);
    unsigned* dst = a_s + ((tid >> 2) * WPL_LDR + (tid & 3) * 4) / 2;
#pragma unroll
    for (int p = 0; p < 3; ++p) *reinterpret_cast<uint2*>(dst + p * 8) = make_uint2(pack_bf16(x[p], y[p]), pack_bf16(z[p], w[p]));
    if (b_active) {
      uint4* d4 = reinterpret_cast<uint4*>(b_s + ((tid >> 1) * WPL_LDR + (tid & 1) * 24) / 2);
      d4[0] = b[0]; d4[1] = b[1]; d4[2] = b[2];
    }
  }
};

template <int BN> constexpr size_t wplanes_lds_bytes() { return 2 * (size_t)(128 + BN) * WPL_LDR * 2; }

template <int BN>
__global__ __launch_bounds__(512) __attribute__((amdgpu_waves_per_eu(2, 2))) void gemm_wplanes_kernel(
    GemmParams p, const unsigned short* __restrict__ planes, int npad) {
  constexpr int BM = 128, DEPTH = 3;
  constexpr int WNW = BN / 64, WMW = 8 / WNW, MT = BM / WMW / 32, NT = 2;
  constexpr int A_WORDS = BM * WPL_LDR / 2, B_WORDS = BN * WPL_LDR / 2;
  extern __shared__ __attribute__((aligned(16))) unsigned wpl_lds[];
  unsigned* sA[2] = {wpl_lds, wpl_lds + A_WORDS};
  unsigned* sB[2] = {wpl_lds + 2 * A_WORDS, wpl_lds + 2 * A_WORDS + B_WORDS};
  const int tid = threadIdx.x, lane = tid & 63, wave = tid >> 6;
  const int wm = wave / WNW, wn = wave % WNW;
  const int tiles_n = (p.N + BN - 1) / BN;
  const int idx = xcd_swizzle(blockIdx.x, gridDim.x);
  const int split = idx / p.tiles, tile = idx - split * p.tiles;
  const int m0 = (tile / tiles_n) * BM, n0 = (tile % tiles_n) * BN;
  const int nk_all = p.K / 16;
  const int kt0 = (int)((long)split * nk_all / p.splits), kt1 = (int)((long)(split + 1) * nk_all / p.splits);
  const int nk = kt1 - kt0;

  f32x16 acc[MT][NT];
#pragma unroll
  for (int i = 0; i < MT; ++i)
#pragma unroll
    for (int j = 0; j < NT; ++j)
#pragma unroll
      for (int r = 0; r < 16; ++r) acc[i][j][r] = 0.f;

  WplRegs sets[DEPTH];
  const float* a_src = p.A + (long)min(m0 + (tid >> 2), p.M - 1) * p.lda + (tid & 3) * 4;
  const bool b_active = BN == 256 || tid < 256;
  const unsigned short* b_src = planes + ((long)n0 + (tid >> 1)) * 48 + (tid & 1) * 24;
  const long b_step = (long)npad * 48;
  const int fr = lane & 31, g = lane >> 5;
  auto mma = [&](const unsigned* a_s, const unsigned* b_s) {
    bf16x8 af[MT][3], bf[NT][3];
#pragma unroll
    for (int i = 0; i < MT; ++i) {
      const unsigned* q = a_s + ((wm * (BM / WMW) + i * 32 + fr) * WPL_LDR + 8 * g) / 2;
#pragma unroll
      for (int pl = 0; pl < 3; ++pl) af[i][pl] = __builtin_bit_cast(bf16x8, *reinterpret_cast<const uint4*>(q + pl * 8));
    }
#pragma unroll
    for (int j = 0; j < NT; ++j) {
      const unsigned* q = b_s + ((wn * 64 + j * 32 + fr) * WPL_LDR + 8 * g) / 2;
#pragma unroll
      for (int pl = 0; pl < 3; ++pl) bf[j][pl] = __builtin_bit_cast(bf16x8, *reinterpret_cast<const uint4*>(q + pl * 8));
    }
#pragma unroll
    for (int i = 0; i < MT; ++i)
#pragma unroll
      for (int j = 0; j < NT; ++j) {
        acc[i][j] = __builtin_amdgcn_mfma_f32_32x32x16_bf16(af[i][2], bf[j][0], acc[i][j], 0, 0, 0);
        acc[i][j] = __builtin_amdgcn_mfma_f32_32x32x16_bf16(af[i][0], bf[j][2], acc[i][j], 0, 0, 0);
        acc[i][j] = __builtin_amdgcn_mfma_f32_32x32x16_bf16(af[i][1], bf[j][1], acc[i][j], 0, 0, 0);
        acc[i][j] = __builtin_amdgcn_mfma_f32_32x32x16_bf16(af[i][1], bf[j][0], acc[i][j], 0, 0, 0);
        acc[i][j] = __builtin_amdgcn_mfma_f32_32x32x16_bf16(af[i][0], bf[j][1], acc[i][j], 0, 0, 0);
        acc[i][j] = __builtin_amdgcn_mfma_f32_32x32x16_bf16(af[i][0], bf[j][0], acc[i][j], 0, 0, 0);
      }
  };
  constexpr int U = 2 * DEPTH;
  constexpr int NMFMA = MT * NT * 6;
#pragma unroll
  for (int d = 0; d < DEPTH; ++d) {
    const int kt = kt0 + min(d, nk - 1);
    sets[d].load(a_src, b_src, (long)kt * 16, kt * b_step, b_active);
  }
  sets[0].store(sA[0], sB[0], tid, b_active);
  __syncthreads();
  for (int t0 = 0; t0 < nk; t0 += U) {
#pragma unroll
    for (int s = 0; s < U; ++s) {
      const int t = t0 + s;
      if (t < nk) {
        {
          const int kt = kt0 + min(t + DEPTH, nk - 1);
          sets[s % DEPTH].load(a_src, b_src, (long)kt * 16, kt * b_step, b_active);
        }
        mma(sA[s & 1], sB[s & 1]);
        sets[(s + 1) % DEPTH].store(sA[(s + 1) & 1], sB[(s + 1) & 1], tid, b_active);
#pragma unroll
        for (int i = 0; i < NMFMA; ++i) {
          __builtin_amdgcn_sched_group_barrier(0x008, 1, 0);
          __builtin_amdgcn_sched_group_barrier(0x002, 2, 0);
          __builtin_amdgcn_sched_group_barrier(0x200, 1, 0);
        }
        __syncthreads();
      }
    }
  }

  if (p.splits > 1) {
    float* slab = p.slabs + (long)split * p.M * p.N;
#pragma unroll
    for (int i = 0; i < MT; ++i)
#pragma unroll
      for (int j = 0; j < NT; ++j) {
        const int n = n0 + wn * 64 + j * 32 + fr;
        if (n >= p.N) continue;
#pragma unroll
        for (int r = 0; r < 16; ++r) {
          const int m = m0 + wm * (BM / WMW) + i * 32 + (r & 3) + 8 * (r >> 2) + 4 * g;
          if (m < p.M) slab[(long)m * p.N + n] = acc[i][j][r];
        }
      }
    return;
  }
  float amx = 0.f;
#pragma unroll
  for (int i = 0; i < MT; ++i)
#pragma unroll
    for (int j = 0; j < NT; ++j) {
      const int n = n0 + wn * 64 + j * 32 + fr;
      if (n >= p.N) continue;
      const float bv = p.bias ? p.bias[n] : 0.f;
      const int mb = m0 + wm * (BM / WMW) + i * 32 + 4 * g;
#pragma unroll
      for (int g4 = 0; g4 < 4; ++g4) {
        float v[4];
#pragma unroll
        for (int u = 0; u < 4; ++u) v[u] = acc[i][j][4 * g4 + u] + bv;
        epilogue_rows4<true>(p, v, mb + 8 * g4, n, amx);
        __builtin_amdgcn_sched_barrier(0);
      }
    }
}

__global__ __launch_bounds__(256) void split_weights_kernel(const int64_t* __restrict__ table, int n_entries) {
  int e = 0;
  while (e + 1 < n_entries && (long)table[(long)(e + 1) * 8 + 6] <= (long)blockIdx.x) ++e;
  const int64_t* t = table + (long)e * 8;
  const float* W = reinterpret_cast<const float*>(t[0]);
  unsigned short* planes = reinterpret_cast<unsigned short*>(t[1]);
  const int N = (int)t[2], K = (int)t[3], ldw = (int)t[4], npad = (int)t[5], tr = (int)t[7];
  const int rows = tr ? K : N, red = tr ? N : K;
  const long idx = ((long)blockIdx.x - t[6]) * 256 + threadIdx.x;
  const int nkt = red / 16;
  const int row = tr ? (int)(idx % npad) : (int)(idx / nkt);
  const int kt = tr ? (int)(idx / npad) : (int)(idx % nkt);
  if (kt >= nkt || row >= npad) return;
  float v[16];
  if (row >= rows) {
#pragma unroll
    for (int i = 0; i < 16; ++i) v[i] = 0.f;
  } else if (!tr) {
    const float4* src = reinterpret_cast<const float4*>(W + (long)row * ldw + kt * 16);
#pragma unroll
    for (int q = 0; q < 4; ++q) { const float4 x = src[q]; v[4 * q] = x.x; v[4 * q + 1] = x.y; v[4 * q + 2] = x.z; v[4 * q + 3] = x.w; }
  } else {
#pragma unroll
    for (int i = 0; i < 16; ++i) v[i] = W[(long)(kt * 16 + i) * ldw + row];
  }
  unsigned out[3][8];
#pragma unroll
  for (int q = 0; q < 8; ++q) {
    __bf16 a[3], b[3];
    split_planes<3>(v[2 * q], a);
    split_planes<3>(v[2 * q + 1], b);
#pragma unroll
    for (int pl = 0; pl < 3; ++pl) out[pl][q] = pack_bf16(a[pl], b[pl]);
  }
  uint4* dst = reinterpret_cast<uint4*>(planes + ((long)kt * npad + row) * 48);
#pragma unroll
  for (int pl = 0; pl < 3; ++pl) {
    dst[pl * 2] = make_uint4(out[pl][0], out[pl][1], out[pl][2], out[pl][3]);
    dst[pl * 2 + 1] = make_uint4(out[pl][4], out[pl][5], out[pl][6], out[pl][7]);
  }
}

__global__ __launch_bounds__(256) void split_weights_h3_kernel(const int64_t* __restrict__ table, int n_entries) {
  int e = 0;
  while (e + 1 < n_entries && (long)table[(long)(e + 1) * 9 + 6] <= (long)blockIdx.x) ++e;
  const int64_t* t = table + (long)e * 9;
  const float* W = reinterpret_cast<const float*>(t[0]);
  uint4* planes = reinterpret_cast<uint4*>(t[1]);
  const int wrows = (int)t[2], wcols = (int)t[3], ldw = (int)t[4], rpad = (int)t[5], tr = (int)t[7];
  const int rows = tr ? wcols : wrows, red = tr ? wrows : wcols;
  const int se = h3_scale_exp(amax_read(reinterpret_cast<const unsigned*>(t[8])));
  const H3Scale hs{__uint_as_float((unsigned)se << 23), __uint_as_float((unsigned)(se + 11) << 23)};
  const long idx = ((long)blockIdx.x - t[6]) * 256 + threadIdx.x;
  const int nkt = red / 32;
  const int kt = (int)(idx / rpad), row = (int)(idx % rpad);
  if (kt >= nkt) return;
  float v[32];
  if (row >= rows) {
#pragma unroll
    for (int i = 0; i < 32; ++i) v[i] = 0.f;
  } else if (!tr) {
    const float4* src = reinterpret_cast<const float4*>(W + (long)row * ldw + kt * 32);
#pragma unroll
    for (int q = 0; q < 8; ++q) { const float4 x = src[q]; v[4 * q] = x.x; v[4 * q + 1] = x.y; v[4 * q + 2] = x.z; v[4 * q + 3] = x.w; }
  } else {
#pragma unroll
    for (int i = 0; i < 32; ++i) v[i] = W[(long)(kt * 32 + i) * ldw + row];
  }
  unsigned h[16], l[16];
#pragma unroll
  for (int q = 0; q < 16; ++q) {
    unsigned o[3];
    split_pair_h(v[2 * q], v[2 * q + 1], hs, o);
    h[q] = o[0]; l[q] = o[1];
  }
  uint4* dst = planes + ((long)kt * rpad + row) * 8;
#pragma unroll
  for (int q = 0; q < 4; ++q) {
    dst[q] = make_uint4(h[4 * q], h[4 * q + 1], h[4 * q + 2], h[4 * q + 3]);
    dst[4 + q] = make_uint4(l[4 * q], l[4 * q + 1], l[4 * q + 2], l[4 * q + 3]);
  }
}

void launch_wplanes(const GemmParams& p, const GemmPlan& pl, const unsigned short* planes, int npad, hipStream_t s) {
  static const bool attr_set = [] {
    hipFuncSetAttribute(reinterpret_cast<const void*>(gemm_wplanes_kernel<256>), hipFuncAttributeMaxDynamicSharedMemorySize,
                        (int)wplanes_lds_bytes<256>());
    hipFuncSetAttribute(reinterpret_cast<const void*>(gemm_wplanes_kernel<128>), hipFuncAttributeMaxDynamicSharedMemorySize,
                        (int)wplanes_lds_bytes<128>());
    return true;
  }();
  (void)attr_set;
  if (pl.bn == 256) gemm_wplanes_kernel<256><<<dim3(pl.nwg), 512, wplanes_lds_bytes<256>(), s>>>(p, planes, npad);
  else gemm_wplanes_kernel<128><<<dim3(pl.nwg), 512, wplanes_lds_bytes<128>(), s>>>(p, planes, npad);
}
}
using namespace rscotr;

extern "C" int rscotr_gemm_split_weights(const int64_t* table, int n, int total_blocks, void* stream) {
  if (n < 0 || total_blocks < 0) return fail(RSCOTR_E_SHAPE, "rscotr_gemm_split_weights: negative count");
  if (n == 0 || total_blocks == 0) return RSCOTR_OK;
  if (!table) return fail(RSCOTR_E_ARG, "rscotr_gemm_split_weights: null table");
  split_weights_kernel<<<dim3((unsigned)total_blocks), 256, 0, (hipStream_t)stream>>>(table, n);
  return check_launch("rscotr_gemm_split_weights");
}

extern "C" int rscotr_gemm_split_weights_h3(const int64_t* table, int n, int total_blocks, void* stream) {
  if (n < 0 || total_blocks < 0) return fail(RSCOTR_E_SHAPE, "rscotr_gemm_split_weights_h3: negative count");
  if (n == 0 || total_blocks == 0) return RSCOTR_OK;
  if (!table) return fail(RSCOTR_E_ARG, "rscotr_gemm_split_weights_h3: null table");
  split_weights_h3_kernel<<<dim3((unsigned)total_blocks), 256, 0, (hipStream_t)stream>>>(table, n);
  return check_launch("rscotr_gemm_split_weights_h3");
}
```

rscotr_amd/csrc/neck.hip:

```cpp
#include "common.h"

namespace rscotr {

template <int MODE>
__global__ __launch_bounds__(256) void gn_stats_kernel(const float* __restrict__ x, const float* __restrict__ dy,
                                                       const float* __restrict__ gamma,
                                                       const float* __restrict__ mean_rstd, float* __restrict__ part,
                                                       int L, int C, int G, int tokens_per_block, long dy_bstride = 0) {
  const int LT = C >> 2;
  const int TPW = kWave / LT;
  const int gs4 = (C / G) >> 2;
  const int lane = threadIdx.x & 63, wave = threadIdx.x >> 6;
  const int sub = lane % LT, slot = lane / LT;
  const int b = blockIdx.y;
  const int t0 = blockIdx.x * tokens_per_block, t1 = min(L, t0 + tokens_per_block);
  const int g = sub / gs4;
  float4 gm = make_float4(1.f, 1.f, 1.f, 1.f);
  float mu = 0.f, rs = 0.f;
  if (MODE == 1) {
    if (gamma) gm = reinterpret_cast<const float4*>(gamma)[sub];
    mu = mean_rstd[((long)b * G + g) * 2];
    rs = mean_rstd[((long)b * G + g) * 2 + 1];
  }
  float s1 = 0.f, s2 = 0.f;
  float4 ag = make_float4(0.f, 0.f, 0.f, 0.f), ab = make_float4(0.f, 0.f, 0.f, 0.f);
  for (int t = t0 + wave * TPW + slot; t < t1; t += 4 * TPW) {
    const long off = ((long)b * L + t) * C;
    const float4 xv = reinterpret_cast<const float4*>(x + off)[sub];
    if (MODE == 0) {
      s1 += xv.x + xv.y + xv.z + xv.w;
      s2 += xv.x * xv.x + xv.y * xv.y + xv.z * xv.z + xv.w * xv.w;
    } else {
      const float4 d = reinterpret_cast<const float4*>(dy + (long)b * dy_bstride + (long)t * C)[sub];
      const float4 xh = make_float4((xv.x - mu) * rs, (xv.y - mu) * rs, (xv.z - mu) * rs, (xv.w - mu) * rs);
      s1 += gm.x * d.x + gm.y * d.y + gm.z * d.z + gm.w * d.w;
      s2 += gm.x * d.x * xh.x + gm.y * d.y * xh.y + gm.z * d.z * xh.z + gm.w * d.w * xh.w;
      ag.x += d.x * xh.x; ag.y += d.y * xh.y; ag.z += d.z * xh.z; ag.w += d.w * xh.w;
      ab.x += d.x; ab.y += d.y; ab.z += d.z; ab.w += d.w;
    }
  }
  for (int o = 1; o < gs4; o <<= 1) {
    s1 += __shfl_xor(s1, o, 64);
    s2 += __shfl_xor(s2, o, 64);
  }
  for (int o = LT; o < kWave; o <<= 1) {
    s1 += __shfl_xor(s1, o, 64);
    s2 += __shfl_xor(s2, o, 64);
    if (MODE == 1) {
      ag.x += __shfl_xor(ag.x, o, 64); ag.y += __shfl_xor(ag.y, o, 64);
      ag.z += __shfl_xor(ag.z, o, 64); ag.w += __shfl_xor(ag.w, o, 64);
      ab.x += __shfl_xor(ab.x, o, 64); ab.y += __shfl_xor(ab.y, o, 64);
      ab.z += __shfl_xor(ab.z, o, 64); ab.w += __shfl_xor(ab.w, o, 64);
    }
  }
  __shared__ float red[4][64][10];
  if (slot == 0) {
    float* r = red[wave][sub];
    r[0] = s1; r[1] = s2;
    r[2] = ag.x; r[3] = ag.y; r[4] = ag.z; r[5] = ag.w;
    r[6] = ab.x; r[7] = ab.y; r[8] = ab.z; r[9] = ab.w;
  }
  __syncthreads();
  if (wave == 0 && slot == 0) {
    float v[10];
#pragma unroll
    for (int k = 0; k < 10; ++k) v[k] = red[0][sub][k] + red[1][sub][k] + red[2][sub][k] + red[3][sub][k];
    float* row = part + ((long)b * gridDim.x + blockIdx.x) * (2 * G + 2 * C);
    if (sub % gs4 == 0) {
      row[2 * g] = v[0];
      row[2 * g + 1] = v[1];
    }
    if (MODE == 1) {
      for (int k = 0; k < 4; ++k) row[2 * G + sub * 4 + k] = v[2 + k];
      for (int k = 0; k < 4; ++k) row[2 * G + C + sub * 4 + k] = v[6 + k];
    }
  }
}

__global__ void gn_finalize_kernel(const float* __restrict__ part, float* __restrict__ mean_rstd, int B, int G, int C,
                                   int chunks, float inv_count, float eps) {
  const int i = blockIdx.x * blockDim.x + threadIdx.x;
  if (i >= B * G) return;
  const int b = i / G, g = i - b * G;
  float s1 = 0.f, s2 = 0.f;
#pragma unroll 8
  for (int c = 0; c < chunks; ++c) {
    const float* row = part + ((long)b * chunks + c) * (2 * G + 2 * C);
    s1 += row[2 * g];
    s2 += row[2 * g + 1];
  }
  const float mu = s1 * inv_count;
  const float var = fmaxf(s2 * inv_count - mu * mu, 0.f);
  mean_rstd[2 * i] = mu;
  mean_rstd[2 * i + 1] = rsqrtf(var + eps);
}

__global__ void gn_finalize_bwd_kernel(const float* __restrict__ part, float* __restrict__ proj, float* __restrict__ dgamma,
                                       float* __restrict__ dbeta, int B, int G, int C, int chunks) {
  const int i = blockIdx.x * blockDim.x + threadIdx.x;
  if (i < B * G) {
    const int b = i / G, g = i - b * G;
    float s1 = 0.f, s2 = 0.f;
#pragma unroll 8
    for (int c = 0; c < chunks; ++c) {
      const float* row = part + ((long)b * chunks + c) * (2 * G + 2 * C);
      s1 += row[2 * g];
      s2 += row[2 * g + 1];
    }
    proj[2 * i] = s1;
    proj[2 * i + 1] = s2;
  }
  if (i < 2 * C) {
    float* dst = i < C ? dgamma : dbeta;
    if (dst) {
      float s = 0.f;
#pragma unroll 8
      for (int r = 0; r < B * chunks; ++r) s += part[(long)r * (2 * G + 2 * C) + 2 * G + i];
      dst[i < C ? i : i - C] += s;
    }
  }
}

template <int MODE>
__global__ __launch_bounds__(256) void gn_apply_kernel(const float* __restrict__ x, const float* __restrict__ dy,
                                                       const float* __restrict__ gamma, const float* __restrict__ beta,
                                                       const float* __restrict__ mean_rstd,
                                                       const float* __restrict__ proj, float* __restrict__ out, int L,
                                                       int C, int G, float inv_count, long dy_bstride4 = 0) {
  const int C4 = C >> 2, gs4 = (C / G) >> 2;
  const long total = (long)gridDim.y * L * C4;
  for (long i = (long)blockIdx.x * 256 + threadIdx.x; i < (long)L * C4; i += (long)gridDim.x * 256) {
    const int b = blockIdx.y;
    const int c4 = (int)(i % C4);
    const int g = c4 / gs4;
    const long off = (long)b * L * C4 + i;
    const float mu = mean_rstd[((long)b * G + g) * 2], rs = mean_rstd[((long)b * G + g) * 2 + 1];
    const float4 xv = reinterpret_cast<const float4*>(x)[off];
    const float4 gm = gamma ? reinterpret_cast<const float4*>(gamma)[c4] : make_float4(1.f, 1.f, 1.f, 1.f);
    float4 o;
    if (MODE == 0) {
      const float4 bt = beta ? reinterpret_cast<const float4*>(beta)[c4] : make_float4(0.f, 0.f, 0.f, 0.f);
      o.x = (xv.x - mu) * rs * gm.x + bt.x; o.y = (xv.y - mu) * rs * gm.y + bt.y;
      o.z = (xv.z - mu) * rs * gm.z + bt.z; o.w = (xv.w - mu) * rs * gm.w + bt.w;
    } else {
      const float4 d = reinterpret_cast<const float4*>(dy)[(long)b * dy_bstride4 + i];
      const float p1 = proj[((long)b * G + g) * 2] * inv_count, p2 = proj[((long)b * G + g) * 2 + 1] * inv_count;
      o.x = rs * (gm.x * d.x - p1 - (xv.x - mu) * rs * p2); o.y = rs * (gm.y * d.y - p1 - (xv.y - mu) * rs * p2);
      o.z = rs * (gm.z * d.z - p1 - (xv.z - mu) * rs * p2); o.w = rs * (gm.w * d.w - p1 - (xv.w - mu) * rs * p2);
    }
    reinterpret_cast<float4*>(out)[off] = o;
  }
  (void)total;
}

__global__ __launch_bounds__(256) void im2col3x3s2_kernel(const float* __restrict__ x, float* __restrict__ col, int B,
                                                          int H, int W, int C, int Ho, int Wo) {
  const long total = (long)B * Ho * Wo * C * 9;
  for (long i = (long)blockIdx.x * 256 + threadIdx.x; i < total; i += (long)gridDim.x * 256) {
    const int k = (int)(i % 9);
    long r = i / 9;
    const int c = (int)(r % C);
    r /= C;
    const int ox = (int)(r % Wo), oy = (int)((r / Wo) % Ho), b = (int)(r / ((long)Wo * Ho));
    const int y = 2 * oy - 1 + k / 3, xx = 2 * ox - 1 + k % 3;
    col[i] = (y >= 0 && y < H && xx >= 0 && xx < W) ? x[(((long)b * H + y) * W + xx) * C + c] : 0.f;
  }
}

__global__ __launch_bounds__(256) void col2im3x3s2_kernel(const float* __restrict__ dcol, float* __restrict__ dx, int B,
                                                          int H, int W, int C, int Ho, int Wo) {
  const long total = (long)B * H * W * C;
  for (long i = (long)blockIdx.x * 256 + threadIdx.x; i < total; i += (long)gridDim.x * 256) {
    const int c = (int)(i % C);
    long r = i / C;
    const int xx = (int)(r % W), y = (int)((r / W) % H), b = (int)(r / ((long)W * H));
    float acc = 0.f;
    for (int ky = 0; ky < 3; ++ky) {
      const int ty = y + 1 - ky;
      if (ty < 0 || (ty & 1)) continue;
      const int oy = ty >> 1;
      if (oy >= Ho) continue;
      for (int kx = 0; kx < 3; ++kx) {
        const int tx = xx + 1 - kx;
        if (tx < 0 || (tx & 1)) continue;
        const int ox = tx >> 1;
        if (ox >= Wo) continue;
        acc += dcol[((((long)b * Ho + oy) * Wo + ox) * C + c) * 9 + ky * 3 + kx];
      }
    }
    dx[i] = acc;
  }
}

static int gn_check(const char* fn, int B, int L, int C, int G) {
  if (B < 0 || L < 0 || C <= 0 || G <= 0 || C % G != 0)
    return fail(RSCOTR_E_SHAPE, "%s: bad shape B=%d L=%d C=%d G=%d", fn, B, L, C, G);
  const int lt = C / 4, gs = C / G;
  if (C % 4 != 0 || (lt != 16 && lt != 32 && lt != 64) || gs % 4 != 0 || ((gs / 4) & (gs / 4 - 1)) != 0)
    return fail(RSCOTR_E_SHAPE, "%s: C=%d must be 64, 128 or 256 with a power-of-two multiple of 4 channels per group", fn, C);
  return RSCOTR_OK;
}

static dim3 gn_stats_grid(int B, int L, int* tpb) {
  int chunks = std::max(1, std::min((L + 31) / 32, 128));
  *tpb = (L + chunks - 1) / chunks;
  chunks = (L + *tpb - 1) / *tpb;
  return dim3(chunks, B);
}

}

using namespace rscotr;

extern "C" int64_t rscotr_groupnorm_tokens_workspace(int B, int L, int C, int G) {
  if (B <= 0 || L <= 0 || C <= 0 || G <= 0) return 0;
  int tpb;
  const dim3 grid = gn_stats_grid(B, L, &tpb);
  return (int64_t)B * grid.x * (2 * G + 2 * C) * 4;
}

extern "C" int rscotr_groupnorm_tokens_fwd(const float* x, const float* weight, const float* bias, float* y,
                                           float* mean_rstd, int B, int L, int C, int G, float eps, float* workspace,
                                           int64_t workspace_bytes, void* stream) {
  if (int e = gn_check("rscotr_groupnorm_tokens_fwd", B, L, C, G)) return e;
  if (B == 0 || L == 0) return RSCOTR_OK;
  if (!x || !y || !mean_rstd) return fail(RSCOTR_E_ARG, "rscotr_groupnorm_tokens_fwd: null pointer");
  if (!aligned16(x) || !aligned16(y) || (weight && !aligned16(weight)) || (bias && !aligned16(bias)))
    return fail(RSCOTR_E_ALIGN, "rscotr_groupnorm_tokens_fwd: pointers must be 16-byte aligned");
  if (!workspace || workspace_bytes < rscotr_groupnorm_tokens_workspace(B, L, C, G))
    return fail(RSCOTR_E_ARG, "rscotr_groupnorm_tokens_fwd: workspace of rscotr_groupnorm_tokens_workspace() bytes required");
  hipStream_t s = (hipStream_t)stream;
  int tpb;
  const dim3 grid = gn_stats_grid(B, L, &tpb);
  gn_stats_kernel<0><<<grid, 256, 0, s>>>(x, nullptr, nullptr, nullptr, workspace, L, C, G, tpb);
  const float inv = 1.f / ((float)L * (float)(C / G));
  gn_finalize_kernel<<<(B * G + 255) / 256, 256, 0, s>>>(workspace, mean_rstd, B, G, C, (int)grid.x, inv, eps);
  const int ax = (int)std::min<long>(((long)L * (C / 4) + 255) / 256, 1024);
  gn_apply_kernel<0><<<dim3(ax, B), 256, 0, s>>>(x, nullptr, weight, bias, mean_rstd, nullptr, y, L, C, G, inv);
  return check_launch("rscotr_groupnorm_tokens_fwd");
}

extern "C" int rscotr_groupnorm_tokens_bwd(const float* dy, const float* x, const float* weight,
                                           const float* mean_rstd, float* dx, float* dweight, float* dbias,
                                           float* proj_ws, int B, int L, int C, int G, int64_t dy_batch_stride,
                                           float* workspace, int64_t workspace_bytes, void* stream) {
  if (int e = gn_check("rscotr_groupnorm_tokens_bwd", B, L, C, G)) return e;
  if (B == 0 || L == 0) return RSCOTR_OK;
  if (dy_batch_stride < (int64_t)L * C || (dy_batch_stride & 3))
    return fail(RSCOTR_E_SHAPE, "rscotr_groupnorm_tokens_bwd: dy batch stride %lld must be >= L * C and a multiple of 4",
                (long long)dy_batch_stride);
  if (!dy || !x || !mean_rstd || !dx || !proj_ws) return fail(RSCOTR_E_ARG, "rscotr_groupnorm_tokens_bwd: null pointer");
  if (!aligned16(dy) || !aligned16(x) || !aligned16(dx) || (weight && !aligned16(weight)))
    return fail(RSCOTR_E_ALIGN, "rscotr_groupnorm_tokens_bwd: pointers must be 16-byte aligned");
  if (!workspace || workspace_bytes < rscotr_groupnorm_tokens_workspace(B, L, C, G))
    return fail(RSCOTR_E_ARG, "rscotr_groupnorm_tokens_bwd: workspace of rscotr_groupnorm_tokens_workspace() bytes required");
  hipStream_t s = (hipStream_t)stream;
  int tpb;
  const dim3 grid = gn_stats_grid(B, L, &tpb);
  gn_stats_kernel<1><<<grid, 256, 0, s>>>(x, dy, weight, mean_rstd, workspace, L, C, G, tpb, (long)dy_batch_stride);
  gn_finalize_bwd_kernel<<<(std::max(B * G, 2 * C) + 255) / 256, 256, 0, s>>>(workspace, proj_ws, dweight, dbias, B, G, C,
                                                                              (int)grid.x);
  const float inv = 1.f / ((float)L * (float)(C / G));
  const int ax = (int)std::min<long>(((long)L * (C / 4) + 255) / 256, 1024);
  gn_apply_kernel<1><<<dim3(ax, B), 256, 0, s>>>(x, dy, weight, nullptr, mean_rstd, proj_ws, dx, L, C, G, inv,
                                                 (long)(dy_batch_stride / 4));
  return check_launch("rscotr_groupnorm_tokens_bwd");
}

extern "C" int rscotr_im2col3x3s2_tokens(const float* x, float* col, int B, int H, int W, int C, void* stream) {
  if (B < 0 || H <= 0 || W <= 0 || C <= 0) return fail(RSCOTR_E_SHAPE, "rscotr_im2col3x3s2_tokens: bad shape");
  if (B == 0) return RSCOTR_OK;
  if (!x || !col) return fail(RSCOTR_E_ARG, "rscotr_im2col3x3s2_tokens: null pointer");
  const int Ho = (H + 1) / 2, Wo = (W + 1) / 2;
  const long total = (long)B * Ho * Wo * C * 9;
  im2col3x3s2_kernel<<<(int)std::min<long>((total + 255) / 256, 4096), 256, 0, (hipStream_t)stream>>>(x, col, B, H, W, C,
                                                                                                 Ho, Wo);
  return check_launch("rscotr_im2col3x3s2_tokens");
}

extern "C" int rscotr_col2im3x3s2_tokens(const float* dcol, float* dx, int B, int H, int W, int C, void* stream) {
  if (B < 0 || H <= 0 || W <= 0 || C <= 0) return fail(RSCOTR_E_SHAPE, "rscotr_col2im3x3s2_tokens: bad shape");
  if (B == 0) return RSCOTR_OK;
  if (!dcol || !dx) return fail(RSCOTR_E_ARG, "rscotr_col2im3x3s2_tokens: null pointer");
  const int Ho = (H + 1) / 2, Wo = (W + 1) / 2;
  const long total = (long)B * H * W * C;
  col2im3x3s2_kernel<<<(int)std::min<long>((total + 255) / 256, 4096), 256, 0, (hipStream_t)stream>>>(dcol, dx, B, H, W, C,
                                                                                                 Ho, Wo);
  return check_launch("rscotr_col2im3x3s2_tokens");
}
```

rscotr_amd/csrc/optim.hip:

```cpp
#include "common.h"

namespace rscotr {

constexpr int SEG_STRIDE = 8;

constexpr int SUMSQ_PARTS = 1024;
__global__ __launch_bounds__(256) void grad_sumsq_kernel(
    const float* __restrict__ grad, const int32_t* __restrict__ chunk_seg,
    const int64_t* __restrict__ chunk_off, const int32_t* __restrict__ chunk_len,
    const float* __restrict__ seg_dyn, float* __restrict__ sumsq, int nchunks) {
  float acc = 0.f;
  for (int c = blockIdx.x; c < nchunks; c += gridDim.x) {
    const int seg = chunk_seg[c];
    if (seg_dyn[seg * SEG_STRIDE + 4] == 0.f) continue;
    const float4* g = reinterpret_cast<const float4*>(grad + chunk_off[c]);
    const int n4 = chunk_len[c] >> 2;
    for (int i = threadIdx.x; i < n4; i += 256) {
      const float4 v = g[i];
      acc += v.x * v.x + v.y * v.y + v.z * v.z + v.w * v.w;
    }
  }
  acc = wave_sum(acc);
  __shared__ float part[4];
  if ((threadIdx.x & 63) == 0) part[threadIdx.x >> 6] = acc;
  __syncthreads();
  if (threadIdx.x == 0) sumsq[1 + blockIdx.x] = part[0] + part[1] + part[2] + part[3];
}

__global__ __launch_bounds__(256) void grad_sumsq_final_kernel(float* __restrict__ sumsq, int nparts) {
  float acc = 0.f;
  for (int i = threadIdx.x; i < nparts; i += 256) acc += sumsq[1 + i];
  acc = wave_sum(acc);
  __shared__ float part[4];
  if ((threadIdx.x & 63) == 0) part[threadIdx.x >> 6] = acc;
  __syncthreads();
  if (threadIdx.x == 0) sumsq[0] = part[0] + part[1] + part[2] + part[3];
}

__global__ __launch_bounds__(256) void seg_amax_reduce_kernel(const int32_t* __restrict__ chunk_seg, const unsigned* __restrict__ chunk_amax,
                                                              const float* __restrict__ seg_dyn, unsigned* __restrict__ seg_amax,
                                                              int nseg, int nchunks) {
  const int sgm = blockIdx.x * 4 + (threadIdx.x >> 6), lane = threadIdx.x & 63;
  if (sgm >= nseg || (seg_dyn && seg_dyn[sgm * SEG_STRIDE + 4] == 0.f)) return;
  int lo0 = 0, hi0 = nchunks, lo1 = 0, hi1 = nchunks;
  while (lo0 < hi0 || lo1 < hi1) {
    const int m0 = (lo0 + hi0) >> 1, m1 = (lo1 + hi1) >> 1;
    const int v0 = lo0 < hi0 ? chunk_seg[m0] : 0, v1 = lo1 < hi1 ? chunk_seg[m1] : 0;
    if (lo0 < hi0) { if (v0 < sgm) lo0 = m0 + 1; else hi0 = m0; }
    if (lo1 < hi1) { if (v1 < sgm + 1) lo1 = m1 + 1; else hi1 = m1; }
  }
  const int c0 = lo0, c1 = lo1;
  unsigned m = 0u;
  for (int c = c0 + lane; c < c1; c += 64) {
    const uint4 v = reinterpret_cast<const uint4*>(chunk_amax)[c];
    m = max(max(m, max(v.x, v.y)), max(v.z, v.w));
  }
#pragma unroll
  for (int o = 32; o > 0; o >>= 1) m = max(m, (unsigned)__shfl_xor((int)m, o, 64));
  if (lane < kAmaxPlanes) {
    const int i = m ? range_byte(m) : -1;
    seg_amax[sgm + (long)lane * kAmaxStride] = (i >= 0 && (i >> 2) == lane) ? (1u << (8 * (i & 3))) : 0u;
  }
}

__device__ __forceinline__ void chunk_amax_store(unsigned* __restrict__ chunk_amax, int c, float amx) {
  amx = wave_max(amx);
  if ((threadIdx.x & 63) == 0) chunk_amax[4 * c + (threadIdx.x >> 6)] = __float_as_uint(amx);
}

__global__ __launch_bounds__(256) void param_amax_kernel(const float* __restrict__ param, const int32_t* __restrict__ chunk_seg,
                                                         const int64_t* __restrict__ chunk_off,
                                                         const int32_t* __restrict__ chunk_len, unsigned* __restrict__ chunk_amax) {
  const int c = blockIdx.x;
  const float4* p4 = reinterpret_cast<const float4*>(param + chunk_off[c]);
  const int n4 = chunk_len[c] >> 2;
  float amx = 0.f;
  for (int i = threadIdx.x; i < n4; i += 256) {
    const float4 p = p4[i];
    amx = fmaxf(fmaxf(amx, fmaxf(fabsf(p.x), fabsf(p.y))), fmaxf(fabsf(p.z), fabsf(p.w)));
  }
  chunk_amax_store(chunk_amax, c, amx);
}

__global__ __launch_bounds__(256) void adamw_clip_kernel(
    float* __restrict__ param, const float* __restrict__ grad, float* __restrict__ exp_avg,
    float* __restrict__ exp_avg_sq, const int32_t* __restrict__ chunk_seg,
    const int64_t* __restrict__ chunk_off, const int32_t* __restrict__ chunk_len,
    const float* __restrict__ seg_dyn, const float* __restrict__ sumsq, float max_norm, float beta1,
    float beta2, float eps, unsigned* __restrict__ chunk_amax) {
  const int c = blockIdx.x;
  const float* d = seg_dyn + chunk_seg[c] * SEG_STRIDE;
  if (d[4] == 0.f) return;
  const float lr = d[0], wd = d[1], inv_bc1 = d[2], inv_sqrt_bc2 = d[3];
  float coef = 1.f;
  if (max_norm > 0.f) {
    coef = fminf(max_norm / (sqrtf(*sumsq) + 1e-6f), 1.f);
  }
  const int64_t off = chunk_off[c];
  float4* p4 = reinterpret_cast<float4*>(param + off);
  const float4* g4 = reinterpret_cast<const float4*>(grad + off);
  float4* m4 = reinterpret_cast<float4*>(exp_avg + off);
  float4* v4 = reinterpret_cast<float4*>(exp_avg_sq + off);
  const int n4 = chunk_len[c] >> 2;
  const float decay = 1.f - lr * wd;
  const float step_size = lr * inv_bc1;
  const float omb1 = 1.f - beta1, omb2 = 1.f - beta2;
  float amx = 0.f;
#define RSCOTR_ADAMW_1(X)                                   \
  {                                                         \
    const float gg = g.X * coef;                            \
    p.X *= decay;                                           \
    m.X = m.X * beta1 + omb1 * gg;                          \
    v.X = v.X * beta2 + omb2 * gg * gg;                     \
    const float denom = sqrtf(v.X) * inv_sqrt_bc2 + eps;    \
    p.X -= step_size * (m.X / denom);                       \
  }
  auto step4 = [&](int i, float4 p, const float4& g, float4 m, float4 v) {
    RSCOTR_ADAMW_1(x) RSCOTR_ADAMW_1(y) RSCOTR_ADAMW_1(z) RSCOTR_ADAMW_1(w)
    p4[i] = p;
    m4[i] = m;
    v4[i] = v;
    amx = fmaxf(fmaxf(amx, fmaxf(fabsf(p.x), fabsf(p.y))), fmaxf(fabsf(p.z), fabsf(p.w)));
  };
  int i = threadIdx.x;
  for (; i + 256 < n4; i += 512) {
    const int j = i + 256;
    const float4 p0 = p4[i], g0 = g4[i], m0 = m4[i], v0 = v4[i];
    const float4 p1 = p4[j], g1 = g4[j], m1 = m4[j], v1 = v4[j];
    asm volatile("" ::: "memory");
    step4(i, p0, g0, m0, v0);
    step4(j, p1, g1, m1, v1);
  }
  if (i < n4) step4(i, p4[i], g4[i], m4[i], v4[i]);
#undef RSCOTR_ADAMW_1
  if (chunk_amax) chunk_amax_store(chunk_amax, c, amx);
}

}

using namespace rscotr;

extern "C" int rscotr_grad_sumsq(const float* grad, const int32_t* chunk_seg, const int64_t* chunk_off,
                                 const int32_t* chunk_len, const float* seg_dyn, int nchunks,
                                 float* sumsq, void* stream) {
  if (nchunks < 0) return fail(RSCOTR_E_SHAPE, "rscotr_grad_sumsq: negative chunk count");
  if (nchunks == 0) return RSCOTR_OK;
  if (!grad || !chunk_seg || !chunk_off || !chunk_len || !seg_dyn || !sumsq)
    return fail(RSCOTR_E_ARG, "rscotr_grad_sumsq: null pointer");
  if (!aligned16(grad)) return fail(RSCOTR_E_ALIGN, "rscotr_grad_sumsq: grad must be 16-byte aligned");
  const int nparts = nchunks < SUMSQ_PARTS ? nchunks : SUMSQ_PARTS;
  grad_sumsq_kernel<<<dim3(nparts), dim3(256), 0, (hipStream_t)stream>>>(
      grad, chunk_seg, chunk_off, chunk_len, seg_dyn, sumsq, nchunks);
  grad_sumsq_final_kernel<<<1, 256, 0, (hipStream_t)stream>>>(sumsq, nparts);
  return check_launch("rscotr_grad_sumsq");
}

extern "C" int rscotr_adamw_clip_step_r(float* param, const float* grad, float* exp_avg, float* exp_avg_sq,
                                        const int32_t* chunk_seg, const int64_t* chunk_off,
                                        const int32_t* chunk_len, const float* seg_dyn, int nchunks,
                                        const float* sumsq, float max_norm, float beta1, float beta2,
                                        float eps, uint32_t* seg_amax, int nseg, uint32_t* chunk_amax, void* stream);

extern "C" int rscotr_adamw_clip_step(float* param, const float* grad, float* exp_avg, float* exp_avg_sq,
                                      const int32_t* chunk_seg, const int64_t* chunk_off,
                                      const int32_t* chunk_len, const float* seg_dyn, int nchunks,
                                      const float* sumsq, float max_norm, float beta1, float beta2,
                                      float eps, void* stream) {
  return rscotr_adamw_clip_step_r(param, grad, exp_avg, exp_avg_sq, chunk_seg, chunk_off, chunk_len, seg_dyn, nchunks, sumsq,
                                  max_norm, beta1, beta2, eps, nullptr, 0, nullptr, stream);
}

extern "C" int rscotr_param_amax(const float* param, const int32_t* chunk_seg, const int64_t* chunk_off,
                                 const int32_t* chunk_len, int nchunks, uint32_t* seg_amax, int nseg, uint32_t* chunk_amax,
                                 void* stream) {
  if (nchunks < 0 || nseg < 0) return fail(RSCOTR_E_SHAPE, "rscotr_param_amax: negative count");
  if (nchunks == 0 || nseg == 0) return RSCOTR_OK;
  if (!param || !chunk_seg || !chunk_off || !chunk_len || !seg_amax || !chunk_amax) return fail(RSCOTR_E_ARG, "rscotr_param_amax: null pointer");
  if (!aligned16(chunk_amax)) return fail(RSCOTR_E_ALIGN, "rscotr_param_amax: chunk_amax must be 16-byte aligned");
  param_amax_kernel<<<dim3(nchunks), dim3(256), 0, (hipStream_t)stream>>>(param, chunk_seg, chunk_off, chunk_len, chunk_amax);
  seg_amax_reduce_kernel<<<dim3((nseg + 3) / 4), dim3(256), 0, (hipStream_t)stream>>>(chunk_seg, chunk_amax, nullptr, seg_amax, nseg, nchunks);
  return check_launch("rscotr_param_amax");
}

extern "C" int rscotr_adamw_clip_step_r(float* param, const float* grad, float* exp_avg, float* exp_avg_sq,
                                        const int32_t* chunk_seg, const int64_t* chunk_off,
                                        const int32_t* chunk_len, const float* seg_dyn, int nchunks,
                                        const float* sumsq, float max_norm, float beta1, float beta2,
                                        float eps, uint32_t* seg_amax, int nseg, uint32_t* chunk_amax, void* stream) {
  if (nchunks < 0) return fail(RSCOTR_E_SHAPE, "rscotr_adamw_clip_step: negative chunk count");
  if (nchunks == 0) return RSCOTR_OK;
  if (!param || !grad || !exp_avg || !exp_avg_sq || !chunk_seg || !chunk_off || !chunk_len || !seg_dyn)
    return fail(RSCOTR_E_ARG, "rscotr_adamw_clip_step: null pointer");
  if (max_norm > 0.f && !sumsq) return fail(RSCOTR_E_ARG, "rscotr_adamw_clip_step: sumsq required when clipping");
  if (!aligned16(param) || !aligned16(grad) || !aligned16(exp_avg) || !aligned16(exp_avg_sq))
    return fail(RSCOTR_E_ALIGN, "rscotr_adamw_clip_step: arenas must be 16-byte aligned");
  const bool ranges = seg_amax && nseg > 0;
  if (ranges && !chunk_amax) return fail(RSCOTR_E_ARG, "rscotr_adamw_clip_step_r: chunk_amax (4 * nchunks words) required with seg_amax");
  if (ranges && !aligned16(chunk_amax)) return fail(RSCOTR_E_ALIGN, "rscotr_adamw_clip_step_r: chunk_amax must be 16-byte aligned");
  ProfScope prof(PROF_HBM, 0.0, (hipStream_t)stream, "rscotr::adamw_clip_kernel");
  adamw_clip_kernel<<<dim3(nchunks), dim3(256), 0, (hipStream_t)stream>>>(
      param, grad, exp_avg, exp_avg_sq, chunk_seg, chunk_off, chunk_len, seg_dyn, sumsq, max_norm, beta1,
      beta2, eps, ranges ? chunk_amax : nullptr);
  if (ranges)
    seg_amax_reduce_kernel<<<dim3((nseg + 3) / 4), dim3(256), 0, (hipStream_t)stream>>>(chunk_seg, chunk_amax, seg_dyn, seg_amax, nseg, nchunks);
  return check_launch("rscotr_adamw_clip_step");
}
```

rscotr_amd/csrc/ranges.hip:

```cpp
#include "common.h"
#include <algorithm>
namespace rscotr {
__device__ __forceinline__ unsigned amax_scan(const float* __restrict__ X, long rows, int cols, int ld, bool vec, long tid, long nth) {
  unsigned m = 0u;
  if (vec) {
    const int c4 = cols >> 2;
    const long n4 = rows * c4;
    for (long i = tid; i < n4; i += nth) {
      const long r = i / c4;
      const int c = (int)(i - r * c4) << 2;
      const uint4 v = *reinterpret_cast<const uint4*>(X + r * ld + c);
      m = max(max(m, v.x & 0x7fffffffu), max(max(v.y & 0x7fffffffu, v.z & 0x7fffffffu), v.w & 0x7fffffffu));
    }
  } else {
    const long n = rows * cols;
    for (long i = tid; i < n; i += nth) {
      const long r = i / cols;
      m = max(m, __float_as_uint(X[r * ld + (i - r * cols)]) & 0x7fffffffu);
    }
  }
  return m;
}

__device__ __forceinline__ void amax_mark(unsigned m, unsigned* sm, unsigned* __restrict__ slot) {
#pragma unroll
  for (int o = 32; o > 0; o >>= 1) m = max(m, (unsigned)__shfl_xor((int)m, o, 64));
  if ((threadIdx.x & 63) == 0) sm[threadIdx.x >> 6] = m;
  __syncthreads();
  if (threadIdx.x == 0) {
    m = max(max(sm[0], sm[1]), max(sm[2], sm[3]));
    if (m) range_mark(slot, range_byte(m));
  }
}

__global__ __launch_bounds__(256) void amax_kernel(const float* __restrict__ X, long rows, int cols, int ld, int vec,
                                                   unsigned* __restrict__ slot) {
  __shared__ unsigned sm[4];
  amax_mark(amax_scan(X, rows, cols, ld, vec, (long)blockIdx.x * 256 + threadIdx.x, (long)gridDim.x * 256), sm, slot);
}

__global__ __launch_bounds__(256) void amax_group_kernel(const int64_t* __restrict__ table, int n) {
  __shared__ unsigned sm[4];
  int lo = 0, hi = n - 1;
  while (lo < hi) {
    const int mid = (lo + hi + 1) >> 1;
    if ((int)table[(long)mid * 6 + 5] <= (int)blockIdx.x) lo = mid; else hi = mid - 1;
  }
  const int64_t* t = table + (long)lo * 6;
  const float* X = reinterpret_cast<const float*>(t[0]);
  const long rows = t[1];
  const int cols = (int)t[2], ld = (int)t[3];
  unsigned* slot = reinterpret_cast<unsigned*>(t[4]);
  const int first = (int)t[5], nb = (lo + 1 < n ? (int)table[(long)(lo + 1) * 6 + 5] : (int)gridDim.x) - first;
  const long tid = (long)(blockIdx.x - first) * 256 + threadIdx.x, nth = (long)nb * 256;
  amax_mark(amax_scan(X, rows, cols, ld, ((t[0] & 15) == 0) && cols % 4 == 0 && ld % 4 == 0, tid, nth), sm, slot);
}
}

extern "C" int rscotr_amax_group(const int64_t* table, int n, int total_blocks, void* stream) {
  if (n < 0 || total_blocks < 0) return rscotr::fail(RSCOTR_E_SHAPE, "rscotr_amax_group: negative count");
  if (n == 0 || total_blocks == 0) return RSCOTR_OK;
  if (!table) return rscotr::fail(RSCOTR_E_ARG, "rscotr_amax_group: null table");
  rscotr::amax_group_kernel<<<dim3((unsigned)total_blocks), 256, 0, (hipStream_t)stream>>>(table, n);
  return rscotr::check_launch("rscotr_amax_group");
}

extern "C" int rscotr_amax_f32(const float* X, int64_t rows, int cols, int ld, uint32_t* slot, void* stream) {
  if (rows < 0 || cols < 0 || ld < cols) return rscotr::fail(RSCOTR_E_SHAPE, "rscotr_amax_f32: bad shape");
  if (rows == 0 || cols == 0) return RSCOTR_OK;
  if (!X || !slot) return rscotr::fail(RSCOTR_E_ARG, "rscotr_amax_f32: null pointer");
  const int vec = rscotr::aligned16(X) && cols % 4 == 0 && ld % 4 == 0;
  const long n = rows * (long)cols;
  const unsigned grid = (unsigned)std::max<long>(1, std::min<long>(256, (n + 8191) / 8192));
  rscotr::amax_kernel<<<dim3(grid), 256, 0, (hipStream_t)stream>>>(X, rows, cols, ld, vec, slot);
  return rscotr::check_launch("rscotr_amax_f32");
}
```

rscotr_amd/ops/deform.py:

```python
import torch
from torch.autograd import Function

from .core import _WS, _Prof, _chk, _f32c, _ptr, _stream, lib
from .matmul import RANGE_OUT, _linear_param_grad, gemm
from .ranges import RANGES
from .state import STATE


_MSDA_HOST_SHAPES = {}


def msda_register_shapes(spatial_shapes, shapes):
    import weakref
    import numpy as np
    _MSDA_HOST_SHAPES[spatial_shapes.data_ptr()] = (
        weakref.ref(spatial_shapes), spatial_shapes._version,
        np.ascontiguousarray(np.asarray(shapes, dtype=np.int64).reshape(-1, 2)))
    if len(_MSDA_HOST_SHAPES) > 256:
        for k in [k for k, e in _MSDA_HOST_SHAPES.items() if e[0]() is None]:
            del _MSDA_HOST_SHAPES[k]


def _msda_host_shapes(spatial_shapes):
    e = _MSDA_HOST_SHAPES.get(spatial_shapes.data_ptr())
    if e is not None:
        owner = e[0]()
        if (owner is not None and owner._version == e[1] and spatial_shapes._version == e[1]
                and owner.shape == spatial_shapes.shape):
            return e[2]
    if torch.cuda.is_current_stream_capturing():
        raise RuntimeError('rscotr_msda_bwd (tiled): the level shapes of this spatial_shapes tensor are not known on the host; '
                           'register them (ops.msda_register_shapes) before the iteration is captured')
    import numpy as np
    return np.ascontiguousarray(spatial_shapes.detach().cpu().numpy().astype(np.int64).reshape(-1, 2))


def _msda_fwd_raw(value, spatial_shapes, level_start_index, loc, attn):
    B, Nk, H, D = value.shape
    _, Nq, _, L, P, _ = loc.shape
    out = torch.empty((B, Nq, H * D), dtype=torch.float32, device=value.device)
    nbytes = 4 * B * (Nk * H * D + Nq * H * L * P * 3 + Nq * H * D)
    with _Prof('msda_fwd', nbytes):
        lib.call('rscotr_msda_fwd', value.data_ptr(), spatial_shapes.data_ptr(),
                 level_start_index.data_ptr(), loc.data_ptr(), attn.data_ptr(), out.data_ptr(),
                 B, Nk, Nq, H, D, L, P, _stream())
    return out


def _msda_bwd_raw(value, spatial_shapes, level_start_index, loc, attn, grad_out):
    B, Nk, H, D = value.shape
    _, Nq, _, L, P, _ = loc.shape
    hs, hs_ptr, nws = None, 0, 0
    if STATE.msda_bwd != 'scatter':
        nws = lib.rscotr_msda_bwd_workspace(B, Nk, Nq, H, L, P)
        if STATE.msda_bwd == 'tiled':
            hs = _msda_host_shapes(spatial_shapes)
            hs_ptr = hs.ctypes.data
            nws = max(nws, lib.rscotr_msda_bwd_tiled_workspace(hs_ptr, B, Nk, Nq, H, D, L, P))
    ws = _WS.get(nws, value.device) if nws else None
    grad_value = torch.zeros_like(value) if ws is None else torch.empty_like(value)
    grad_loc = torch.empty_like(loc)
    grad_attn = torch.empty_like(attn)
    nbytes = 4 * B * (3 * Nk * H * D + Nq * H * L * P * 3 + Nq * H * D + Nq * H * L * P * 3)
    slot = RANGES.out_slot(value.device)
    with _Prof('msda_bwd', nbytes):
        lib.call('rscotr_msda_bwd', value.data_ptr(), spatial_shapes.data_ptr(),
                 level_start_index.data_ptr(), loc.data_ptr(), attn.data_ptr(), grad_out.data_ptr(),
                 grad_value.data_ptr(), grad_loc.data_ptr(), grad_attn.data_ptr(),
                 B, Nk, Nq, H, D, L, P, hs_ptr, 0 if ws is None else ws.data_ptr(), nws, slot, _stream())
    return RANGES.tag(grad_value, slot), grad_loc, grad_attn


class _MSDA(Function):
    @staticmethod
    def forward(ctx, value, spatial_shapes, level_start_index, loc, attn):
        value, loc, attn = _f32c(value), _f32c(loc), _f32c(attn)
        spatial_shapes = spatial_shapes.contiguous()
        level_start_index = level_start_index.contiguous()
        _chk(value, spatial_shapes, level_start_index, loc, attn)
        assert spatial_shapes.dtype == torch.int64 and level_start_index.dtype == torch.int64
        out = _msda_fwd_raw(value, spatial_shapes, level_start_index, loc, attn)
        ctx.save_for_backward(value, spatial_shapes, level_start_index, loc, attn)
        return out

    @staticmethod
    def backward(ctx, grad_out):
        value, spatial_shapes, level_start_index, loc, attn = ctx.saved_tensors
        grad_value, grad_loc, grad_attn = _msda_bwd_raw(value, spatial_shapes, level_start_index, loc, attn, _f32c(grad_out))
        return grad_value, None, None, grad_loc, grad_attn


def msda(value, spatial_shapes, level_start_index, loc, attn):
    return _MSDA.apply(value, spatial_shapes, level_start_index, loc, attn)


def _msda_fused_ok(Nk, H, D, L, P):
    return bool(lib.rscotr_msda_fused_ok(Nk, H, D, L, P))


def _msda_fwd_prep_raw(value, spatial_shapes, level_start_index, off, logit, ref, norm, L, P, ld_off, ld_logit):
    B, Nk, H, D = value.shape
    Nq = ref.shape[1]
    loc = torch.empty((B, Nq, H, L, P, 2), dtype=torch.float32, device=value.device)
    attn = torch.empty((B, Nq, H, L, P), dtype=torch.float32, device=value.device)
    out = torch.empty((B, Nq, H * D), dtype=torch.float32, device=value.device)
    nbytes = 4 * B * (Nk * H * D + Nq * H * L * P * 6 + Nq * H * D)
    with _Prof('msda_fwd', nbytes):
        lib.call('rscotr_msda_fwd_prep', value.data_ptr(), spatial_shapes.data_ptr(), level_start_index.data_ptr(),
                 off.data_ptr(), logit.data_ptr(), ld_off, ld_logit, ref.data_ptr(), _ptr(norm), ref.shape[-1], ref.shape[-2],
                 loc.data_ptr(), attn.data_ptr(), out.data_ptr(), B, Nk, Nq, H, D, L, P, _stream())
    return loc, attn, out


def _msda_prep_fwd_raw(off, logit, ref, norm, B, Nq, H, L, P, ld_off=None, ld_logit=None):
    refdim = ref.shape[-1]
    loc = torch.empty((B, Nq, H, L, P, 2), dtype=torch.float32, device=off.device)
    attn = torch.empty((B, Nq, H, L, P), dtype=torch.float32, device=off.device)
    lib.call('rscotr_msda_prep_fwd', off.data_ptr(), logit.data_ptr(), ref.data_ptr(), _ptr(norm), loc.data_ptr(),
             attn.data_ptr(), B, Nq, H, L, P, refdim, ld_off or H * L * P * 2, ld_logit or H * L * P, ref.shape[-2], _stream())
    return loc, attn


def _msda_prep_bwd_raw(gloc, gattn, attn, ref, norm, B, Nq, H, L, P, packed=False):
    n = H * L * P
    if packed:
        both = torch.empty((B * Nq, 3 * n), dtype=torch.float32, device=attn.device)
        goff, glogit, ldo, ldl = both, both[:, 2 * n:], 3 * n, 3 * n
    else:
        goff = torch.empty((B, Nq, H, L * P * 2), dtype=torch.float32, device=attn.device)
        glogit = torch.empty((B, Nq, H, L * P), dtype=torch.float32, device=attn.device)
        ldo, ldl = 2 * n, n
    slot = RANGES.out_slot(attn.device)
    lib.call('rscotr_msda_prep_bwd', gloc.data_ptr(), gattn.data_ptr(), attn.data_ptr(), ref.data_ptr(), _ptr(norm),
             goff.data_ptr(), glogit.data_ptr(), B, Nq, H, L, P, ref.shape[-1], ldo, ldl, ref.shape[-2], slot, _stream())
    return (RANGES.tag(both, slot), None) if packed else (RANGES.tag(goff, slot), RANGES.tag(glogit, slot))


class _MSDAPrep(Function):
    @staticmethod
    def forward(ctx, off, logit, ref, norm, L, P):
        off, logit, ref = _f32c(off), _f32c(logit), _f32c(ref.detach())
        _chk(off, logit, ref, norm)
        B, Nq, H = logit.shape[:3]
        loc, attn = _msda_prep_fwd_raw(off, logit, ref, norm, B, Nq, H, L, P)
        ctx.save_for_backward(attn, ref, norm)
        ctx.geom = (B, Nq, H, L, P)
        return loc, attn

    @staticmethod
    def backward(ctx, gloc, gattn):
        attn, ref, norm = ctx.saved_tensors
        goff, glogit = _msda_prep_bwd_raw(_f32c(gloc), _f32c(gattn), attn, ref, norm, *ctx.geom)
        return goff, glogit, None, None, None, None


def msda_prep(off, logit, reference_points, offset_norm, L, P):
    assert not reference_points.requires_grad, 'reference points are detached on this path'
    B, Nq, H = logit.shape[:3]
    return _MSDAPrep.apply(off.view(B, Nq, H, L * P * 2), logit, reference_points, offset_norm, L, P)




class _MSDAAttn(Function):

    @staticmethod
    def forward(ctx, x, q_pos, value_in, identity, kpm, ref, spatial_shapes, lsi, norm, heads, L, P,
                w_off, b_off, w_aw, b_aw, w_v, b_v, w_o, b_o, q_sum=None):
        B, Nq, C = x.shape
        H, D = heads, C // heads
        M = B * Nq
        x2 = RANGES.carry(x, _f32c(x).reshape(M, C))
        q2 = x2 if q_pos is None else (_f32c(torch.add(x, q_pos)).reshape(M, C) if q_sum is None else
                                       RANGES.carry(q_sum, _f32c(q_sum).reshape(M, C)))
        v_is_x = value_in is None or value_in is x
        id_is_x = identity is x
        val2 = x2 if v_is_x else RANGES.carry(value_in, _f32c(value_in).reshape(-1, C))
        if kpm is not None:
            val2 = val2.masked_fill(kpm.reshape(-1, 1), 0.0)
        Mk = val2.shape[0]
        Nk = Mk // B
        ws = [w if w.is_contiguous() else w.contiguous() for w in (w_off, w_aw, w_v, w_o)]
        ref = _f32c(ref.detach())
        spatial_shapes, lsi = spatial_shapes.contiguous(), lsi.contiguous()
        _chk(x2, q2, val2, ref, spatial_shapes, lsi, norm)
        v = gemm(val2, ws[2], Mk, C, C, C, C, 0, 0, bias=b_v)
        if kpm is not None:
            v.view(B, Nk, C).masked_fill_(kpm[..., None], 0.0)
        n_off, n_aw = H * L * P * 2, H * L * P
        packed = b_off is not None and b_aw is not None and n_off % 4 == 0 and C % 4 == 0
        if packed:
            n3 = n_off + n_aw
            wb = torch.empty(n3 * C + n3, dtype=torch.float32, device=x2.device)
            wslot = RANGES.out_slot(x2.device)
            lib.call('rscotr_pack4', ws[0].data_ptr(), n_off * C, ws[1].data_ptr(), n_aw * C, b_off.data_ptr(), n_off,
                     b_aw.data_ptr(), n_aw, wb.data_ptr(), wslot, _stream())
            w_cat = RANGES.tag(wb[:n3 * C].view(n3, C), wslot)
            both = gemm(q2, w_cat, M, n3, C, C, C, 0, 0, bias=wb[n3 * C:], range_out=RANGE_OUT.want(False))
            off, logit, ldo, ldl = both, both.view(-1)[n_off:], n3, n3
        else:
            w_cat = None
            off = gemm(q2, ws[0], M, n_off, C, C, C, 0, 0, bias=b_off)
            logit = gemm(q2, ws[1], M, n_aw, C, C, C, 0, 0, bias=b_aw)
            ldo, ldl = n_off, n_aw
        if _msda_fused_ok(Nk, H, D, L, P):
            loc, attn, out = _msda_fwd_prep_raw(v.view(B, Nk, H, D), spatial_shapes, lsi, off, logit, ref, norm, L, P, ldo, ldl)
        else:
            loc, attn = _msda_prep_fwd_raw(off, logit, ref, norm, B, Nq, H, L, P, ld_off=ldo, ld_logit=ldl)
            out = _msda_fwd_raw(v.view(B, Nk, H, D), spatial_shapes, lsi, loc, attn)
        id2 = x2 if id_is_x else (None if identity is None else _f32c(identity).reshape(M, C))
        y = gemm(RANGES.carry(v, out.view(M, C)), ws[3], M, C, C, C, C, 0, 0, bias=b_o, resid=id2, range_out=RANGE_OUT.want(id2 is None))
        ctx.save_for_backward(q2, val2, v, loc, attn, ref, norm, out, spatial_shapes, lsi, *ws)
        ctx.slots = (RANGES.saved(q2), RANGES.saved(val2))
        ctx.kpm = kpm
        ctx.w_cat = w_cat
        ctx.params = (w_off, b_off, w_aw, b_aw, w_v, b_v, w_o, b_o)
        ctx.geom = (B, Nq, Nk, C, H, D, L, P)
        ctx.flags = (v_is_x, id_is_x, q_pos is not None, identity is not None)
        ctx.shapes = (x.shape, None if q_pos is None else q_pos.shape, None if value_in is None else value_in.shape,
                      None if identity is None else identity.shape)
        return RANGES.carry(y, y.view(B, Nq, C))

    @staticmethod
    def backward(ctx, dy):
        q2, val2, v, loc, attn, ref, norm, out, spatial_shapes, lsi, w_off, w_aw, w_v, w_o = ctx.saved_tensors
        p_off, pb_off, p_aw, pb_aw, p_v, pb_v, p_o, pb_o = ctx.params
        B, Nq, Nk, C, H, D, L, P = ctx.geom
        v_is_x, id_is_x, has_pos, has_id = ctx.flags
        need = ctx.needs_input_grad
        M, Mk = B * Nq, B * Nk
        n_off, n_aw = H * L * P * 2, H * L * P
        g = RANGES.carry(dy, _f32c(dy).reshape(M, C))
        RANGES.restore(q2, ctx.slots[0])
        RANGES.restore(val2, ctx.slots[1])
        sinks = []
        gw_o, gb_o, s1, s2 = _linear_param_grad(g, out.view(M, C), C, C, M, p_o, pb_o, 0, need[18], pb_o is not None and need[19])
        sinks += [s1, s2]
        d_out = gemm(g, w_o, M, C, C, C, C, 0, 1, range_out=RANGE_OUT.want(False))
        gv, gloc, gattn = _msda_bwd_raw(v.view(B, Nk, H, D), spatial_shapes, lsi, loc, attn, d_out.view(B, Nq, C))
        w_cat = ctx.w_cat
        packed = w_cat is not None
        n3 = n_off + n_aw
        goff, glogit = _msda_prep_bwd_raw(gloc, gattn, attn, ref, norm, B, Nq, H, L, P, packed=packed)
        gv = RANGES.carry(gv, gv.view(Mk, C))
        if packed:
            both = goff
            goff, glogit, ldg = both.view(-1), both.view(-1)[n_off:], n3
            RANGES.carry(both, goff)
            RANGES.carry(both, glogit)
        else:
            goff, glogit, ldg = goff.view(M, n_off), glogit.view(M, n_aw), None
        if ctx.kpm is not None:
            gv.view(B, Nk, C).masked_fill_(ctx.kpm[..., None], 0.0)
        gw_off, gb_off, s1, s2 = _linear_param_grad(goff, q2, n_off, C, M, p_off, pb_off, 0, need[12], pb_off is not None and need[13], lda=ldg)
        sinks += [s1, s2]
        gw_aw, gb_aw, s1, s2 = _linear_param_grad(glogit, q2, n_aw, C, M, p_aw, pb_aw, 0, need[14], pb_aw is not None and need[15], lda=ldg)
        sinks += [s1, s2]
        gw_v, gb_v, s1, s2 = _linear_param_grad(gv, val2, C, C, Mk, p_v, pb_v, 0, need[16], pb_v is not None and need[17])
        sinks += [s1, s2]
        for sk_ in sinks:
            if sk_ is not None:
                STATE.grad_sink.grad_written(sk_[0])
        gin = lambda *a_, **k_: gemm(*a_, range_out=RANGE_OUT.want(False), **k_)
        want_pos = has_pos and need[1]
        want_x = need[0]
        want_val = (not v_is_x) and need[2]
        d_x = d_pos = d_val = None
        merge_id = id_is_x and want_x
        if want_x or want_pos:
            two = want_pos and want_x and (merge_id or v_is_x)
            res = g if (merge_id and (two or not want_pos)) else None
            if two:
                d_x = torch.empty((M, C), dtype=torch.float32, device=g.device)
            if packed:
                pure = gin(both, w_cat, M, C, n3, n3, C, 0, 1, out2=d_x if two else None, resid=res)
            else:
                pure = gin(goff, w_off, M, C, n_off, n_off, C, 0, 1)
                gin(glogit, w_aw, M, C, n_aw, n_aw, C, 0, 1, out=pure, accumulate=True, out2=d_x if two else None, resid=res)
            if two:
                d_pos = pure
            else:
                d_x = pure if want_x else None
                d_pos = pure if want_pos else None
            if v_is_x and want_x:
                gin(gv, w_v, Mk, C, C, C, C, 0, 1, out=d_x, accumulate=True)
        elif v_is_x and want_x:
            d_x = gin(gv, w_v, Mk, C, C, C, C, 0, 1, resid=g if merge_id else None)
        if want_val:
            d_val = gin(gv, w_v, Mk, C, C, C, C, 0, 1).view(ctx.shapes[2])
        d_id = g.view(ctx.shapes[3]) if (has_id and not merge_id and need[3]) else None
        if id_is_x and not merge_id:
            d_id = None
        return (None if d_x is None else RANGES.carry(d_x, d_x.view(ctx.shapes[0])),
                None if d_pos is None else RANGES.carry(d_pos, d_pos.view(ctx.shapes[1])),
                d_val, d_id, None, None, None, None, None, None, None, None,
                gw_off, gb_off, gw_aw, gb_aw, gw_v, gb_v, gw_o, gb_o, None)


def msda_attention(x, q_pos, value, identity, key_padding_mask, reference_points, spatial_shapes, level_start_index,
                   offset_norm, heads, L, P, w_off, b_off, w_aw, b_aw, w_v, b_v, w_o, b_o, q_sum=None):
    assert not reference_points.requires_grad, 'reference points are detached on this path'
    if reference_points.shape[-1] not in (2, 4):
        raise ValueError(f'Last dim of reference_points must be 2 or 4, got {reference_points.shape[-1]}')
    if q_pos is not None and q_pos.shape != x.shape:
        q_pos = q_pos.expand_as(x)
    if q_sum is not None:
        assert q_pos is not None and q_sum.shape == x.shape
        q_sum = RANGES.carry(q_sum, q_sum.detach())
    return _MSDAAttn.apply(x, q_pos, value, identity, key_padding_mask, reference_points, spatial_shapes,
                           level_start_index, offset_norm, heads, L, P, w_off, b_off, w_aw, b_aw, w_v, b_v, w_o, b_o, q_sum)
```

rscotr_amd/ops/norm.py:

```python
import torch
from torch.autograd import Function

from .core import _WS, _Prof, _chk, _f32c, _ptr, _sink, _stream, lib
from .deferred import DEFER, LnPart
from .ranges import RANGES
from .state import STATE

LN_EPS = 1e-5


class LazyNorm:

    def __init__(self, x2, w, b, eps, y, stats, slot):
        self.x2, self.w, self.b, self.eps, self.y, self.stats, self.slot = x2, w, b, eps, y, stats, slot
        self.done = False

    def run(self):
        if not self.done:
            M, C = self.x2.shape
            with _Prof('layernorm_fwd', 8 * M * C):
                lib.call('rscotr_layernorm_fwd', self.x2.data_ptr(), _ptr(self.w), _ptr(self.b), self.y.data_ptr(),
                         self.stats[0].data_ptr(), self.stats[1].data_ptr(), M, C, float(self.eps), self.slot, _stream())
            self.done = True


def materialize(t):
    lz = getattr(t, '_lazy_ln', None)
    if lz is not None:
        lz.run()
    return t


class _LayerNorm(Function):
    @staticmethod
    def forward(ctx, x, w, b, eps, lazy=False):
        C = x.shape[-1]
        x2 = _f32c(x).reshape(-1, C)
        M = x2.shape[0]
        _chk(x2, w, b)
        y = torch.empty_like(x2)
        stats = torch.empty((2, M), dtype=torch.float32, device=x2.device)
        slot = RANGES.out_slot(x2.device)
        lz = LazyNorm(x2, w, b, eps, y, stats, slot)
        if not lazy:
            lz.run()
        ctx.save_for_backward(x2, w, stats)
        ctx.has_b = b is not None
        ctx.bias = b
        out = RANGES.tag(y.view(x.shape), slot)
        if lazy:
            out._lazy_ln = lz
        return out

    @staticmethod
    def backward(ctx, dy, dres=None):
        return _LayerNorm._backward(ctx, dy, dres)

    @staticmethod
    def _backward(ctx, dy, dres):
        x2, w, stats = ctx.saved_tensors
        merge = getattr(ctx, 'merge', None)
        if merge is None:
            M, C = x2.shape
        else:
            M, C = stats.shape[1], 4 * merge[3]
            assert dres is None
        g = _f32c(dy).reshape(M, C)
        r = None if dres is None else _f32c(dres).reshape(M, C)
        dx = torch.empty_like(x2) if ctx.needs_input_grad[0] else None
        slot = RANGES.out_slot(x2.device) if dx is not None else 0
        skw, skb = _sink(w), _sink(ctx.bias)
        direct = skw is not None and (skb is not None or not ctx.has_b)
        dwb = None if direct else torch.zeros((2, C), dtype=torch.float32, device=x2.device)
        dw_ptr = skw[1].data_ptr() if direct else dwb[0].data_ptr()
        db_ptr = (skb[1].data_ptr() if ctx.has_b else 0) if direct else dwb[1].data_ptr()
        nws = lib.rscotr_layernorm_bwd_workspace(M, C) if merge is None else lib.rscotr_patch_merge_norm_bwd_workspace(*merge)
        dx_shape = dy.shape if merge is None else x2.shape
        defer = direct and DEFER.enabled and STATE.side is None and STATE.profile is None
        if merge is not None:
            ws_ptr = DEFER.reserve(nws, x2.device) if defer else _WS.get(nws, x2.device).data_ptr()
            lib.call('rscotr_patch_merge_norm_bwd', g.data_ptr(), x2.data_ptr(), _ptr(w), stats[0].data_ptr(),
                     stats[1].data_ptr(), _ptr(dx), dw_ptr, db_ptr, *merge, ws_ptr, nws, 0 if defer else 1, slot, _stream())
            if defer:
                DEFER.ln_entries.append(LnPart(ws_ptr, dw_ptr, db_ptr, nws // (8 * C), C))
        elif defer:
            part = DEFER.reserve(nws, x2.device)
            lib.call('rscotr_layernorm_bwd_partials', g.data_ptr(), x2.data_ptr(), _ptr(w), stats[0].data_ptr(),
                     stats[1].data_ptr(), _ptr(dx), _ptr(r), M, C, part, nws, slot, _stream())
            DEFER.ln_entries.append(LnPart(part, dw_ptr, db_ptr, nws // (8 * C), C))
        else:
            ws = _WS.get(nws, x2.device)
            with _Prof('layernorm_bwd', 12 * M * C):
                lib.call('rscotr_layernorm_bwd', g.data_ptr(), x2.data_ptr(), _ptr(w), stats[0].data_ptr(),
                         stats[1].data_ptr(), _ptr(dx), _ptr(r), dw_ptr, db_ptr, M, C, ws.data_ptr(), nws, slot, _stream())
        if defer:
            STATE.grad_sink.grad_written(skw[0])
            if ctx.has_b:
                STATE.grad_sink.grad_written(skb[0])
            return (None if dx is None else RANGES.tag(dx.view(dx_shape), slot)), None, None, None
        dxv = None if dx is None else RANGES.tag(dx.view(dx_shape), slot)
        if direct:
            STATE.grad_sink.grad_written(skw[0])
            if ctx.has_b:
                STATE.grad_sink.grad_written(skb[0])
            return dxv, None, None, None
        return dxv, dwb[0] if w is not None else None, dwb[1] if ctx.has_b else None, None


class _LayerNormFork(Function):

    @staticmethod
    def forward(ctx, x, w, b, eps, lazy=False):
        ctx.set_materialize_grads(False)
        return _LayerNorm.forward(ctx, x, w, b, eps, lazy), x

    @staticmethod
    def backward(ctx, dy, dres):
        if dy is None:
            return dres, None, None, None, None
        return _LayerNorm._backward(ctx, dy, dres) + (None,)


class _LayerNormSum(Function):

    @staticmethod
    def forward(ctx, x, w, b, eps, add):
        C = x.shape[-1]
        x2 = _f32c(x).reshape(-1, C)
        M = x2.shape[0]
        if add.dim() == 3 and add.shape[0] > 1 and add.stride(0) == 0:
            a2 = _f32c(add[0])
        else:
            a2 = _f32c(add).reshape(-1, C)
        rows = a2.shape[0]
        assert M % rows == 0 and a2.shape[-1] == C, (tuple(x.shape), tuple(add.shape))
        _chk(x2, w, b, a2)
        y, y2 = torch.empty_like(x2), torch.empty_like(x2)
        stats = torch.empty((2, M), dtype=torch.float32, device=x2.device)
        with _Prof('layernorm_fwd', 16 * M * C):
            slot = RANGES.out_slot(x2.device)
            lib.call('rscotr_layernorm_fwd_sum', x2.data_ptr(), _ptr(w), _ptr(b), y.data_ptr(), stats[0].data_ptr(),
                     stats[1].data_ptr(), a2.data_ptr(), rows, y2.data_ptr(), M, C, float(eps), slot, _stream())
        ctx.save_for_backward(x2, w, stats)
        ctx.has_b = b is not None
        ctx.bias = b
        y, y2 = RANGES.tag(y.view(x.shape), slot), RANGES.tag(y2.view(x.shape), slot)
        ctx.mark_non_differentiable(y2)
        ctx.set_materialize_grads(False)
        ctx.out_shape = tuple(x.shape)
        return y, y2

    @staticmethod
    def backward(ctx, dy, _):
        if dy is None:
            dy = torch.zeros(ctx.out_shape, dtype=torch.float32, device=ctx.saved_tensors[0].device)
        return _LayerNorm._backward(ctx, dy, None) + (None,)


class _PatchMergeNorm(Function):

    @staticmethod
    def forward(ctx, x, w, b, eps, H, W):
        B, L, Cin = x.shape
        assert L == H * W
        x3 = _f32c(x)
        Ho, Wo = (H + 1) // 2, (W + 1) // 2
        M, C = B * Ho * Wo, 4 * Cin
        _chk(x3, w, b)
        y = torch.empty((B, Ho * Wo, C), dtype=torch.float32, device=x3.device)
        stats = torch.empty((2, M), dtype=torch.float32, device=x3.device)
        with _Prof('layernorm_fwd', 8 * M * C):
            slot = RANGES.out_slot(x3.device)
            lib.call('rscotr_patch_merge_norm_fwd', x3.data_ptr(), _ptr(w), _ptr(b), y.data_ptr(), stats[0].data_ptr(),
                     stats[1].data_ptr(), B, H, W, Cin, float(eps), slot, _stream())
        ctx.save_for_backward(x3, w, stats)
        ctx.has_b, ctx.bias, ctx.merge = b is not None, b, (B, H, W, Cin)
        return RANGES.tag(y, slot)

    @staticmethod
    def backward(ctx, dy):
        return _LayerNorm._backward(ctx, dy, None) + (None, None)


def layer_norm(x, w, b, eps=LN_EPS):
    return _LayerNorm.apply(x, w, b, eps)


def patch_merge_norm(x, hw, w, b, eps=LN_EPS):
    H, W = hw
    return _PatchMergeNorm.apply(x, w, b, eps, int(H), int(W)), ((H + 1) // 2, (W + 1) // 2)


def layer_norm_sum(x, w, b, add, eps=LN_EPS):
    return _LayerNormSum.apply(x, w, b, eps, add.detach())


def layer_norm_fork(x, w, b, eps=LN_EPS, lazy=False):
    return _LayerNormFork.apply(x, w, b, eps, bool(lazy))


class _GroupNormTokens(Function):
    @staticmethod
    def forward(ctx, x, w, b, groups, eps):
        x = _f32c(x)
        _chk(x, w, b)
        B, L, C = x.shape
        y = torch.empty_like(x)
        stats = torch.empty((B, groups, 2), dtype=torch.float32, device=x.device)
        nws = lib.rscotr_groupnorm_tokens_workspace(B, L, C, groups)
        lib.call('rscotr_groupnorm_tokens_fwd', x.data_ptr(), _ptr(w), _ptr(b), y.data_ptr(), stats.data_ptr(),
                 B, L, C, groups, float(eps), _WS.get(nws, x.device).data_ptr(), nws, _stream())
        ctx.save_for_backward(x, w, stats)
        ctx.groups, ctx.has_b, ctx.bias = groups, b is not None, b
        return y

    @staticmethod
    def backward(ctx, dy):
        x, w, stats = ctx.saved_tensors
        B, L, C = x.shape
        if not (dy.dtype == torch.float32 and dy.dim() == 3 and dy.stride(2) == 1 and dy.stride(1) == C
                and dy.stride(0) >= L * C and dy.stride(0) % 4 == 0 and dy.data_ptr() % 16 == 0):
            dy = _f32c(dy)
            if dy.data_ptr() % 16:
                dy = dy.clone()
        dx = torch.empty_like(x)
        skw, skb = _sink(w), _sink(ctx.bias)
        direct = w is not None and skw is not None and (skb is not None or not ctx.has_b)
        dwb = None if direct else torch.zeros((2, C), dtype=torch.float32, device=x.device)
        dw_ptr = skw[1].data_ptr() if direct else dwb[0].data_ptr()
        db_ptr = (skb[1].data_ptr() if ctx.has_b else 0) if direct else dwb[1].data_ptr()
        proj = torch.empty((B, ctx.groups, 2), dtype=torch.float32, device=x.device)
        nws = lib.rscotr_groupnorm_tokens_workspace(B, L, C, ctx.groups)
        lib.call('rscotr_groupnorm_tokens_bwd', dy.data_ptr(), x.data_ptr(), _ptr(w), stats.data_ptr(), dx.data_ptr(),
                 dw_ptr, db_ptr, proj.data_ptr(), B, L, C, ctx.groups, dy.stride(0),
                 _WS.get(nws, x.device).data_ptr(), nws, _stream())
        if direct:
            STATE.grad_sink.grad_written(skw[0])
            if ctx.has_b:
                STATE.grad_sink.grad_written(skb[0])
            return dx, None, None, None, None
        return dx, dwb[0] if w is not None else None, dwb[1] if ctx.has_b else None, None, None


def group_norm_tokens(x, groups, w, b, eps=1e-5):
    return _GroupNormTokens.apply(x, w, b, groups, eps)
```

Baseline: 213.6.

## Fold small finalize kernels into consumers and add ranged elementwise add

Drops the separate group-norm finalize kernels. Each apply block now re-reduces the per-chunk partial sums into shared memory, and extra blocks fold the dgamma/dbeta sums. The grad-norm final reduction moves into the AdamW kernel, so every chunk block recomputes the total and block 0 writes it back. Weight-split kernels replace their linear table scan with a binary search, and the query+pos add becomes a fused add-plus-amax kernel so no separate range scan is needed. This removes several tiny launches and one tensor allocation, at the cost of redundant reductions repeated in every block.

```diff
diff --git a/include/rscotr.h b/include/rscotr.h
--- a/include/rscotr.h
+++ b/include/rscotr.h
@@ -105,6 +105,7 @@
 int rscotr_gemm_f32_split_route(int M, int N, int K, int lda, int ldb, int a_kmajor, int b_kmajor, int act, int has_pre,
                                 int has_rowscale, int has_kscale, int64_t workspace_bytes);
 int rscotr_amax_f32(const float* X, int64_t rows, int cols, int ld, uint32_t* slot, void* stream);
+int rscotr_add_range_f32(const float* a, const float* b, float* out, int64_t rows, int cols, uint32_t* slot, void* stream);
 int rscotr_amax_group(const int64_t* table, int n, int total_blocks, void* stream);
 int rscotr_gemm_f32_dw_slabs(const float* A, const float* B, float* C, int M, int N, int K, int lda, int ldb, int ldc,
                              float* rowsum, const float* kscale, int krows_per_scale, float* slab_region,
@@ -301,11 +302,11 @@
                       void* stream);
 int rscotr_adamw_clip_step(float* param, const float* grad, float* exp_avg, float* exp_avg_sq,
                            const int32_t* chunk_seg, const int64_t* chunk_off, const int32_t* chunk_len,
-                           const float* seg_dyn, int nchunks, const float* sumsq, float max_norm,
+                           const float* seg_dyn, int nchunks, float* sumsq, float max_norm,
                            float beta1, float beta2, float eps, void* stream);
 int rscotr_adamw_clip_step_r(float* param, const float* grad, float* exp_avg, float* exp_avg_sq,
                              const int32_t* chunk_seg, const int64_t* chunk_off, const int32_t* chunk_len,
-                             const float* seg_dyn, int nchunks, const float* sumsq, float max_norm,
+                             const float* seg_dyn, int nchunks, float* sumsq, float max_norm,
                              float beta1, float beta2, float eps, uint32_t* seg_amax, int nseg, uint32_t* chunk_amax,
                              void* stream);
 int rscotr_param_amax(const float* param, const int32_t* chunk_seg, const int64_t* chunk_off,
diff --git a/rscotr_amd/csrc/common.h b/rscotr_amd/csrc/common.h
--- a/rscotr_amd/csrc/common.h
+++ b/rscotr_amd/csrc/common.h
@@ -111,6 +111,15 @@
   return out;
 }
 
+__device__ __forceinline__ int table_row_of(const int64_t* __restrict__ table, int n, int stride, int col, long wg) {
+  int lo = 0, hi = n - 1;
+  while (lo < hi) {
+    const int mid = (lo + hi + 1) >> 1;
+    if ((long)table[(long)mid * stride + col] <= wg) lo = mid; else hi = mid - 1;
+  }
+  return lo;
+}
+
 __device__ __forceinline__ float amax4(float a, const float4& v) {
   return fmaxf(fmaxf(a, fmaxf(fabsf(v.x), fabsf(v.y))), fmaxf(fabsf(v.z), fabsf(v.w)));
 }
diff --git a/rscotr_amd/csrc/ffn.hip b/rscotr_amd/csrc/ffn.hip
--- a/rscotr_amd/csrc/ffn.hip
+++ b/rscotr_amd/csrc/ffn.hip
@@ -625,9 +625,7 @@
 
 
 __global__ __launch_bounds__(256) void split_weights_frag_kernel(const int64_t* __restrict__ table, int n_entries) {
-  int e = 0;
-  while (e + 1 < n_entries && (long)table[(long)(e + 1) * 9 + 6] <= (long)blockIdx.x) ++e;
-  const int64_t* t = table + (long)e * 9;
+  const int64_t* t = table + (long)table_row_of(table, n_entries, 9, 6, (long)blockIdx.x) * 9;
   const float* W = reinterpret_cast<const float*>(t[0]);
   uint4* planes = reinterpret_cast<uint4*>(t[1]);
   const int wrows = (int)t[2], wcols = (int)t[3], ldw = (int)t[4], tr = (int)t[7];
diff --git a/rscotr_amd/csrc/gemm_planes.hip b/rscotr_amd/csrc/gemm_planes.hip
--- a/rscotr_amd/csrc/gemm_planes.hip
+++ b/rscotr_amd/csrc/gemm_planes.hip
@@ -155,9 +155,7 @@
 }
 
 __global__ __launch_bounds__(256) void split_weights_kernel(const int64_t* __restrict__ table, int n_entries) {
-  int e = 0;
-  while (e + 1 < n_entries && (long)table[(long)(e + 1) * 8 + 6] <= (long)blockIdx.x) ++e;
-  const int64_t* t = table + (long)e * 8;
+  const int64_t* t = table + (long)table_row_of(table, n_entries, 8, 6, (long)blockIdx.x) * 8;
   const float* W = reinterpret_cast<const float*>(t[0]);
   unsigned short* planes = reinterpret_cast<unsigned short*>(t[1]);
   const int N = (int)t[2], K = (int)t[3], ldw = (int)t[4], npad = (int)t[5], tr = (int)t[7];
@@ -197,9 +195,7 @@
 }
 
 __global__ __launch_bounds__(256) void split_weights_h3_kernel(const int64_t* __restrict__ table, int n_entries) {
-  int e = 0;
-  while (e + 1 < n_entries && (long)table[(long)(e + 1) * 9 + 6] <= (long)blockIdx.x) ++e;
-  const int64_t* t = table + (long)e * 9;
+  const int64_t* t = table + (long)table_row_of(table, n_entries, 9, 6, (long)blockIdx.x) * 9;
   const float* W = reinterpret_cast<const float*>(t[0]);
   uint4* planes = reinterpret_cast<uint4*>(t[1]);
   const int wrows = (int)t[2], wcols = (int)t[3], ldw = (int)t[4], rpad = (int)t[5], tr = (int)t[7];
diff --git a/rscotr_amd/csrc/neck.hip b/rscotr_amd/csrc/neck.hip
--- a/rscotr_amd/csrc/neck.hip
+++ b/rscotr_amd/csrc/neck.hip
@@ -77,64 +77,75 @@
   }
 }
 
-__global__ void gn_finalize_kernel(const float* __restrict__ part, float* __restrict__ mean_rstd, int B, int G, int C,
-                                   int chunks, float inv_count, float eps) {
-  const int i = blockIdx.x * blockDim.x + threadIdx.x;
-  if (i >= B * G) return;
-  const int b = i / G, g = i - b * G;
-  float s1 = 0.f, s2 = 0.f;
+
+__device__ __forceinline__ void gn_fold_sums(const float* __restrict__ part, int b, int g, int G, int C, int chunks, float& s1,
+                                             float& s2) {
+  s1 = 0.f;
+  s2 = 0.f;
 #pragma unroll 8
   for (int c = 0; c < chunks; ++c) {
     const float* row = part + ((long)b * chunks + c) * (2 * G + 2 * C);
     s1 += row[2 * g];
     s2 += row[2 * g + 1];
   }
-  const float mu = s1 * inv_count;
-  const float var = fmaxf(s2 * inv_count - mu * mu, 0.f);
-  mean_rstd[2 * i] = mu;
-  mean_rstd[2 * i + 1] = rsqrtf(var + eps);
-}
-
-__global__ void gn_finalize_bwd_kernel(const float* __restrict__ part, float* __restrict__ proj, float* __restrict__ dgamma,
-                                       float* __restrict__ dbeta, int B, int G, int C, int chunks) {
-  const int i = blockIdx.x * blockDim.x + threadIdx.x;
-  if (i < B * G) {
-    const int b = i / G, g = i - b * G;
-    float s1 = 0.f, s2 = 0.f;
+}
+
+__device__ __forceinline__ void gn_fold_stats(const float* __restrict__ part, int b, int g, int G, int C, int chunks,
+                                              float inv_count, float eps, float& mu, float& rs) {
+  float s1, s2;
+  gn_fold_sums(part, b, g, G, C, chunks, s1, s2);
+  mu = s1 * inv_count;
+  const float var = fmaxf(fmaf(-mu, mu, s2 * inv_count), 0.f);
+  rs = rsqrtf(var + eps);
+}
+
+__device__ __forceinline__ void gn_fold_params(const float* __restrict__ part, float* __restrict__ dgamma,
+                                               float* __restrict__ dbeta, int i, int rows, int G, int C) {
+  if (i >= 2 * C) return;
+  float* dst = i < C ? dgamma : dbeta;
+  if (!dst) return;
+  float s = 0.f;
 #pragma unroll 8
-    for (int c = 0; c < chunks; ++c) {
-      const float* row = part + ((long)b * chunks + c) * (2 * G + 2 * C);
-      s1 += row[2 * g];
-      s2 += row[2 * g + 1];
-    }
-    proj[2 * i] = s1;
-    proj[2 * i + 1] = s2;
-  }
-  if (i < 2 * C) {
-    float* dst = i < C ? dgamma : dbeta;
-    if (dst) {
-      float s = 0.f;
-#pragma unroll 8
-      for (int r = 0; r < B * chunks; ++r) s += part[(long)r * (2 * G + 2 * C) + 2 * G + i];
-      dst[i < C ? i : i - C] += s;
-    }
-  }
+  for (int r = 0; r < rows; ++r) s += part[(long)r * (2 * G + 2 * C) + 2 * G + i];
+  dst[i < C ? i : i - C] += s;
 }
 
 template <int MODE>
 __global__ __launch_bounds__(256) void gn_apply_kernel(const float* __restrict__ x, const float* __restrict__ dy,
                                                        const float* __restrict__ gamma, const float* __restrict__ beta,
-                                                       const float* __restrict__ mean_rstd,
-                                                       const float* __restrict__ proj, float* __restrict__ out, int L,
-                                                       int C, int G, float inv_count, long dy_bstride4 = 0) {
+                                                       const float* __restrict__ part, const float* __restrict__ mean_rstd,
+                                                       float* __restrict__ stats_out, float* __restrict__ dgamma,
+                                                       float* __restrict__ dbeta, float* __restrict__ out, int L, int C, int G,
+                                                       int chunks, int ax, float inv_count, float eps, long dy_bstride4 = 0) {
   const int C4 = C >> 2, gs4 = (C / G) >> 2;
-  const long total = (long)gridDim.y * L * C4;
-  for (long i = (long)blockIdx.x * 256 + threadIdx.x; i < (long)L * C4; i += (long)gridDim.x * 256) {
-    const int b = blockIdx.y;
+  const int b = blockIdx.y;
+  if (MODE == 1 && (int)blockIdx.x >= ax) {
+    if (b == 0) gn_fold_params(part, dgamma, dbeta, ((int)blockIdx.x - ax) * 256 + (int)threadIdx.x, (int)gridDim.y * chunks, G, C);
+    return;
+  }
+  __shared__ float folded[64][2];
+  if ((int)threadIdx.x < G) {
+    const int g = threadIdx.x;
+    float u, v;
+    if (MODE == 0) {
+      gn_fold_stats(part, b, g, G, C, chunks, inv_count, eps, u, v);
+      if (blockIdx.x == 0) {
+        stats_out[((long)b * G + g) * 2] = u;
+        stats_out[((long)b * G + g) * 2 + 1] = v;
+      }
+    } else {
+      gn_fold_sums(part, b, g, G, C, chunks, u, v);
+    }
+    folded[g][0] = u;
+    folded[g][1] = v;
+  }
+  __syncthreads();
+  for (long i = (long)blockIdx.x * 256 + threadIdx.x; i < (long)L * C4; i += (long)ax * 256) {
     const int c4 = (int)(i % C4);
     const int g = c4 / gs4;
     const long off = (long)b * L * C4 + i;
-    const float mu = mean_rstd[((long)b * G + g) * 2], rs = mean_rstd[((long)b * G + g) * 2 + 1];
+    const float mu = MODE == 0 ? folded[g][0] : mean_rstd[((long)b * G + g) * 2];
+    const float rs = MODE == 0 ? folded[g][1] : mean_rstd[((long)b * G + g) * 2 + 1];
     const float4 xv = reinterpret_cast<const float4*>(x)[off];
     const float4 gm = gamma ? reinterpret_cast<const float4*>(gamma)[c4] : make_float4(1.f, 1.f, 1.f, 1.f);
     float4 o;
@@ -144,13 +155,12 @@
       o.z = (xv.z - mu) * rs * gm.z + bt.z; o.w = (xv.w - mu) * rs * gm.w + bt.w;
     } else {
       const float4 d = reinterpret_cast<const float4*>(dy)[(long)b * dy_bstride4 + i];
-      const float p1 = proj[((long)b * G + g) * 2] * inv_count, p2 = proj[((long)b * G + g) * 2 + 1] * inv_count;
+      const float p1 = folded[g][0] * inv_count, p2 = folded[g][1] * inv_count;
       o.x = rs * (gm.x * d.x - p1 - (xv.x - mu) * rs * p2); o.y = rs * (gm.y * d.y - p1 - (xv.y - mu) * rs * p2);
       o.z = rs * (gm.z * d.z - p1 - (xv.z - mu) * rs * p2); o.w = rs * (gm.w * d.w - p1 - (xv.w - mu) * rs * p2);
     }
     reinterpret_cast<float4*>(out)[off] = o;
   }
-  (void)total;
 }
 
 __global__ __launch_bounds__(256) void im2col3x3s2_kernel(const float* __restrict__ x, float* __restrict__ col, int B,
@@ -234,9 +244,9 @@
   const dim3 grid = gn_stats_grid(B, L, &tpb);
   gn_stats_kernel<0><<<grid, 256, 0, s>>>(x, nullptr, nullptr, nullptr, workspace, L, C, G, tpb);
   const float inv = 1.f / ((float)L * (float)(C / G));
-  gn_finalize_kernel<<<(B * G + 255) / 256, 256, 0, s>>>(workspace, mean_rstd, B, G, C, (int)grid.x, inv, eps);
   const int ax = (int)std::min<long>(((long)L * (C / 4) + 255) / 256, 1024);
-  gn_apply_kernel<0><<<dim3(ax, B), 256, 0, s>>>(x, nullptr, weight, bias, mean_rstd, nullptr, y, L, C, G, inv);
+  gn_apply_kernel<0><<<dim3(ax, B), 256, 0, s>>>(x, nullptr, weight, bias, workspace, nullptr, mean_rstd, nullptr, nullptr, y, L, C,
+                                                 G, (int)grid.x, ax, inv, eps);
   return check_launch("rscotr_groupnorm_tokens_fwd");
 }
 
@@ -249,7 +259,8 @@
   if (dy_batch_stride < (int64_t)L * C || (dy_batch_stride & 3))
     return fail(RSCOTR_E_SHAPE, "rscotr_groupnorm_tokens_bwd: dy batch stride %lld must be >= L * C and a multiple of 4",
                 (long long)dy_batch_stride);
-  if (!dy || !x || !mean_rstd || !dx || !proj_ws) return fail(RSCOTR_E_ARG, "rscotr_groupnorm_tokens_bwd: null pointer");
+  (void)proj_ws;
+  if (!dy || !x || !mean_rstd || !dx) return fail(RSCOTR_E_ARG, "rscotr_groupnorm_tokens_bwd: null pointer");
   if (!aligned16(dy) || !aligned16(x) || !aligned16(dx) || (weight && !aligned16(weight)))
     return fail(RSCOTR_E_ALIGN, "rscotr_groupnorm_tokens_bwd: pointers must be 16-byte aligned");
   if (!workspace || workspace_bytes < rscotr_groupnorm_tokens_workspace(B, L, C, G))
@@ -258,12 +269,11 @@
   int tpb;
   const dim3 grid = gn_stats_grid(B, L, &tpb);
   gn_stats_kernel<1><<<grid, 256, 0, s>>>(x, dy, weight, mean_rstd, workspace, L, C, G, tpb, (long)dy_batch_stride);
-  gn_finalize_bwd_kernel<<<(std::max(B * G, 2 * C) + 255) / 256, 256, 0, s>>>(workspace, proj_ws, dweight, dbias, B, G, C,
-                                                                              (int)grid.x);
   const float inv = 1.f / ((float)L * (float)(C / G));
   const int ax = (int)std::min<long>(((long)L * (C / 4) + 255) / 256, 1024);
-  gn_apply_kernel<1><<<dim3(ax, B), 256, 0, s>>>(x, dy, weight, nullptr, mean_rstd, proj_ws, dx, L, C, G, inv,
-                                                 (long)(dy_batch_stride / 4));
+  const int nfin = (dweight || dbias) ? (2 * C + 255) / 256 : 0;
+  gn_apply_kernel<1><<<dim3(ax + nfin, B), 256, 0, s>>>(x, dy, weight, nullptr, workspace, mean_rstd, nullptr, dweight, dbias, dx, L,
+                                                        C, G, (int)grid.x, ax, inv, 0.f, (long)(dy_batch_stride / 4));
   return check_launch("rscotr_groupnorm_tokens_bwd");
 }
 
diff --git a/rscotr_amd/csrc/optim.hip b/rscotr_amd/csrc/optim.hip
--- a/rscotr_amd/csrc/optim.hip
+++ b/rscotr_amd/csrc/optim.hip
@@ -27,14 +27,13 @@
   if (threadIdx.x == 0) sumsq[1 + blockIdx.x] = part[0] + part[1] + part[2] + part[3];
 }
 
-__global__ __launch_bounds__(256) void grad_sumsq_final_kernel(float* __restrict__ sumsq, int nparts) {
+__device__ __forceinline__ float sumsq_fold(const float* __restrict__ sumsq, int nparts, float (&part)[4]) {
   float acc = 0.f;
   for (int i = threadIdx.x; i < nparts; i += 256) acc += sumsq[1 + i];
   acc = wave_sum(acc);
-  __shared__ float part[4];
   if ((threadIdx.x & 63) == 0) part[threadIdx.x >> 6] = acc;
   __syncthreads();
-  if (threadIdx.x == 0) sumsq[0] = part[0] + part[1] + part[2] + part[3];
+  return part[0] + part[1] + part[2] + part[3];
 }
 
 __global__ __launch_bounds__(256) void seg_amax_reduce_kernel(const int32_t* __restrict__ chunk_seg, const unsigned* __restrict__ chunk_amax,
@@ -86,16 +85,21 @@
     float* __restrict__ param, const float* __restrict__ grad, float* __restrict__ exp_avg,
     float* __restrict__ exp_avg_sq, const int32_t* __restrict__ chunk_seg,
     const int64_t* __restrict__ chunk_off, const int32_t* __restrict__ chunk_len,
-    const float* __restrict__ seg_dyn, const float* __restrict__ sumsq, float max_norm, float beta1,
+    const float* __restrict__ seg_dyn, float* __restrict__ sumsq, int nparts, float max_norm, float beta1,
     float beta2, float eps, unsigned* __restrict__ chunk_amax) {
   const int c = blockIdx.x;
   const float* d = seg_dyn + chunk_seg[c] * SEG_STRIDE;
-  if (d[4] == 0.f) return;
-  const float lr = d[0], wd = d[1], inv_bc1 = d[2], inv_sqrt_bc2 = d[3];
+  const bool live = d[4] != 0.f;
+  if (!live && c != 0) return;
   float coef = 1.f;
   if (max_norm > 0.f) {
-    coef = fminf(max_norm / (sqrtf(*sumsq) + 1e-6f), 1.f);
-  }
+    __shared__ float part[4];
+    const float total = sumsq_fold(sumsq, nparts, part);
+    if (c == 0 && threadIdx.x == 0) sumsq[0] = total;
+    coef = fminf(max_norm / (sqrtf(total) + 1e-6f), 1.f);
+  }
+  if (!live) return;
+  const float lr = d[0], wd = d[1], inv_bc1 = d[2], inv_sqrt_bc2 = d[3];
   const int64_t off = chunk_off[c];
   float4* p4 = reinterpret_cast<float4*>(param + off);
   const float4* g4 = reinterpret_cast<const float4*>(grad + off);
@@ -136,6 +140,8 @@
   if (chunk_amax) chunk_amax_store(chunk_amax, c, amx);
 }
 
+static int sumsq_parts(int nchunks) { return nchunks < SUMSQ_PARTS ? nchunks : SUMSQ_PARTS; }
+
 }
 
 using namespace rscotr;
@@ -148,23 +154,22 @@
   if (!grad || !chunk_seg || !chunk_off || !chunk_len || !seg_dyn || !sumsq)
     return fail(RSCOTR_E_ARG, "rscotr_grad_sumsq: null pointer");
   if (!aligned16(grad)) return fail(RSCOTR_E_ALIGN, "rscotr_grad_sumsq: grad must be 16-byte aligned");
-  const int nparts = nchunks < SUMSQ_PARTS ? nchunks : SUMSQ_PARTS;
+  const int nparts = sumsq_parts(nchunks);
   grad_sumsq_kernel<<<dim3(nparts), dim3(256), 0, (hipStream_t)stream>>>(
       grad, chunk_seg, chunk_off, chunk_len, seg_dyn, sumsq, nchunks);
-  grad_sumsq_final_kernel<<<1, 256, 0, (hipStream_t)stream>>>(sumsq, nparts);
   return check_launch("rscotr_grad_sumsq");
 }
 
 extern "C" int rscotr_adamw_clip_step_r(float* param, const float* grad, float* exp_avg, float* exp_avg_sq,
                                         const int32_t* chunk_seg, const int64_t* chunk_off,
                                         const int32_t* chunk_len, const float* seg_dyn, int nchunks,
-                                        const float* sumsq, float max_norm, float beta1, float beta2,
+                                        float* sumsq, float max_norm, float beta1, float beta2,
                                         float eps, uint32_t* seg_amax, int nseg, uint32_t* chunk_amax, void* stream);
 
 extern "C" int rscotr_adamw_clip_step(float* param, const float* grad, float* exp_avg, float* exp_avg_sq,
                                       const int32_t* chunk_seg, const int64_t* chunk_off,
                                       const int32_t* chunk_len, const float* seg_dyn, int nchunks,
-                                      const float* sumsq, float max_norm, float beta1, float beta2,
+                                      float* sumsq, float max_norm, float beta1, float beta2,
                                       float eps, void* stream) {
   return rscotr_adamw_clip_step_r(param, grad, exp_avg, exp_avg_sq, chunk_seg, chunk_off, chunk_len, seg_dyn, nchunks, sumsq,
                                   max_norm, beta1, beta2, eps, nullptr, 0, nullptr, stream);
@@ -185,7 +190,7 @@
 extern "C" int rscotr_adamw_clip_step_r(float* param, const float* grad, float* exp_avg, float* exp_avg_sq,
                                         const int32_t* chunk_seg, const int64_t* chunk_off,
                                         const int32_t* chunk_len, const float* seg_dyn, int nchunks,
-                                        const float* sumsq, float max_norm, float beta1, float beta2,
+                                        float* sumsq, float max_norm, float beta1, float beta2,
                                         float eps, uint32_t* seg_amax, int nseg, uint32_t* chunk_amax, void* stream) {
   if (nchunks < 0) return fail(RSCOTR_E_SHAPE, "rscotr_adamw_clip_step: negative chunk count");
   if (nchunks == 0) return RSCOTR_OK;
@@ -199,7 +204,7 @@
   if (ranges && !aligned16(chunk_amax)) return fail(RSCOTR_E_ALIGN, "rscotr_adamw_clip_step_r: chunk_amax must be 16-byte aligned");
   ProfScope prof(PROF_HBM, 0.0, (hipStream_t)stream, "rscotr::adamw_clip_kernel");
   adamw_clip_kernel<<<dim3(nchunks), dim3(256), 0, (hipStream_t)stream>>>(
-      param, grad, exp_avg, exp_avg_sq, chunk_seg, chunk_off, chunk_len, seg_dyn, sumsq, max_norm, beta1,
+      param, grad, exp_avg, exp_avg_sq, chunk_seg, chunk_off, chunk_len, seg_dyn, sumsq, sumsq_parts(nchunks), max_norm, beta1,
       beta2, eps, ranges ? chunk_amax : nullptr);
   if (ranges)
     seg_amax_reduce_kernel<<<dim3((nseg + 3) / 4), dim3(256), 0, (hipStream_t)stream>>>(chunk_seg, chunk_amax, seg_dyn, seg_amax, nseg, nchunks);
diff --git a/rscotr_amd/csrc/ranges.hip b/rscotr_amd/csrc/ranges.hip
--- a/rscotr_amd/csrc/ranges.hip
+++ b/rscotr_amd/csrc/ranges.hip
@@ -39,6 +39,30 @@
   amax_mark(amax_scan(X, rows, cols, ld, vec, (long)blockIdx.x * 256 + threadIdx.x, (long)gridDim.x * 256), sm, slot);
 }
 
+__global__ __launch_bounds__(256) void add_range_kernel(const float* __restrict__ a, const float* __restrict__ b,
+                                                        float* __restrict__ out, long n, int vec, unsigned* __restrict__ slot) {
+  __shared__ unsigned sm[4];
+  const long tid = (long)blockIdx.x * 256 + threadIdx.x, nth = (long)gridDim.x * 256;
+  unsigned m = 0u;
+  if (vec) {
+    const long n4 = n >> 2;
+    for (long i = tid; i < n4; i += nth) {
+      const float4 x = reinterpret_cast<const float4*>(a)[i], y = reinterpret_cast<const float4*>(b)[i];
+      const float4 s = make_float4(x.x + y.x, x.y + y.y, x.z + y.z, x.w + y.w);
+      reinterpret_cast<float4*>(out)[i] = s;
+      m = max(max(m, __float_as_uint(s.x) & 0x7fffffffu),
+              max(max(__float_as_uint(s.y) & 0x7fffffffu, __float_as_uint(s.z) & 0x7fffffffu), __float_as_uint(s.w) & 0x7fffffffu));
+    }
+  } else {
+    for (long i = tid; i < n; i += nth) {
+      const float s = a[i] + b[i];
+      out[i] = s;
+      m = max(m, __float_as_uint(s) & 0x7fffffffu);
+    }
+  }
+  amax_mark(m, sm, slot);
+}
+
 __global__ __launch_bounds__(256) void amax_group_kernel(const int64_t* __restrict__ table, int n) {
   __shared__ unsigned sm[4];
   int lo = 0, hi = n - 1;
@@ -65,6 +89,18 @@
   return rscotr::check_launch("rscotr_amax_group");
 }
 
+extern "C" int rscotr_add_range_f32(const float* a, const float* b, float* out, int64_t rows, int cols, uint32_t* slot,
+                                    void* stream) {
+  if (rows < 0 || cols < 0) return rscotr::fail(RSCOTR_E_SHAPE, "rscotr_add_range_f32: bad shape");
+  if (rows == 0 || cols == 0) return RSCOTR_OK;
+  if (!a || !b || !out || !slot) return rscotr::fail(RSCOTR_E_ARG, "rscotr_add_range_f32: null pointer");
+  const int vec = rscotr::aligned16(a) && rscotr::aligned16(b) && rscotr::aligned16(out) && cols % 4 == 0;
+  const long n = rows * (long)cols;
+  const unsigned grid = (unsigned)std::max<long>(1, std::min<long>(256, (n + 8191) / 8192));
+  rscotr::add_range_kernel<<<dim3(grid), 256, 0, (hipStream_t)stream>>>(a, b, out, n, vec, slot);
+  return rscotr::check_launch("rscotr_add_range_f32");
+}
+
 extern "C" int rscotr_amax_f32(const float* X, int64_t rows, int cols, int ld, uint32_t* slot, void* stream) {
   if (rows < 0 || cols < 0 || ld < cols) return rscotr::fail(RSCOTR_E_SHAPE, "rscotr_amax_f32: bad shape");
   if (rows == 0 || cols == 0) return RSCOTR_OK;
diff --git a/rscotr_amd/ops/deform.py b/rscotr_amd/ops/deform.py
--- a/rscotr_amd/ops/deform.py
+++ b/rscotr_amd/ops/deform.py
@@ -162,6 +162,16 @@
 
 
 
+def _add_ranged(a, b):
+    if not (RANGES.enabled and a.is_cuda and a.shape == b.shape and a.dtype == b.dtype == torch.float32
+            and a.is_contiguous() and b.is_contiguous() and a.dim() >= 1 and a.numel()):
+        return _f32c(torch.add(a, b))
+    out = torch.empty_like(a)
+    slot = RANGES.new_slot(a.device)
+    lib.call('rscotr_add_range_f32', a.data_ptr(), b.data_ptr(), out.data_ptr(), a.numel() // a.shape[-1], a.shape[-1], slot, _stream())
+    return RANGES.tag(out, slot)
+
+
 class _MSDAAttn(Function):
 
     @staticmethod
@@ -171,8 +181,9 @@
         H, D = heads, C // heads
         M = B * Nq
         x2 = RANGES.carry(x, _f32c(x).reshape(M, C))
-        q2 = x2 if q_pos is None else (_f32c(torch.add(x, q_pos)).reshape(M, C) if q_sum is None else
-                                       RANGES.carry(q_sum, _f32c(q_sum).reshape(M, C)))
+        if q_pos is not None and q_sum is None:
+            q_sum = _add_ranged(x, q_pos)
+        q2 = x2 if q_pos is None else RANGES.carry(q_sum, _f32c(q_sum).reshape(M, C))
         v_is_x = value_in is None or value_in is x
         id_is_x = identity is x
         val2 = x2 if v_is_x else RANGES.carry(value_in, _f32c(value_in).reshape(-1, C))
diff --git a/rscotr_amd/ops/norm.py b/rscotr_amd/ops/norm.py
--- a/rscotr_amd/ops/norm.py
+++ b/rscotr_amd/ops/norm.py
@@ -229,10 +229,9 @@
         dwb = None if direct else torch.zeros((2, C), dtype=torch.float32, device=x.device)
         dw_ptr = skw[1].data_ptr() if direct else dwb[0].data_ptr()
         db_ptr = (skb[1].data_ptr() if ctx.has_b else 0) if direct else dwb[1].data_ptr()
-        proj = torch.empty((B, ctx.groups, 2), dtype=torch.float32, device=x.device)
         nws = lib.rscotr_groupnorm_tokens_workspace(B, L, C, ctx.groups)
         lib.call('rscotr_groupnorm_tokens_bwd', dy.data_ptr(), x.data_ptr(), _ptr(w), stats.data_ptr(), dx.data_ptr(),
-                 dw_ptr, db_ptr, proj.data_ptr(), B, L, C, ctx.groups, dy.stride(0),
+                 dw_ptr, db_ptr, 0, B, L, C, ctx.groups, dy.stride(0),
                  _WS.get(nws, x.device).data_ptr(), nws, _stream())
         if direct:
             STATE.grad_sink.grad_written(skw[0])
```

After: 214.7, median of 6. No clear change (+0.5%).
